# CMB-BNU/PloidyFrost

Measured on AMD Instinct MI355X. Metric: unitigs/s through superbubble+SeqAlign (k=25, z=8), higher is better.
Workload: dtype u64

## Files before the change

ploidyfrost_amd/csrc/pf_bubble.hip:

```cpp
#include <hip/hip_runtime.h>

#include <algorithm>
#include <chrono>
#include <cmath>
#include <cstdio>
#include <cstdlib>
#include <cstring>
#include <string>
#include <vector>

#include "pf_align_dev.hpp"
#include "pf_bubble_launch.hpp"
#include "pf_ctx.hpp"
#include "pf_device_common.hpp"
#include "ploidyfrost_hip.h"

using namespace pf;

#define PF_HIP(call)                                                                         \
    do {                                                                                     \
        hipError_t e_ = (call);                                                              \
        if (e_ != hipSuccess) {                                                              \
            pf::CtxErr{ctx} = std::string(#call) + ": " + hipGetErrorString(e_);                   \
            return PF_ERR_HIP;                                                               \
// ... 534 lines not shown
            const MsaRef M = list[cur][c];
            const char *rows = arena[cur] + M.off;
            uint8_t *ci = M.len <= p.work_bytes ? nw_base : colinfo;
            const Metrics m = classify(rows, M.rows, M.len, ci, snp_pos, indel_pos, indel_len);
            int verdict = 0;
            uint64_t c_indel = 0, c_snp = 0, c_all = 0;
            const int total = m.snp + m.indel, btotal = best_snp + best_indel;
            if (total < btotal) verdict = 1;
            else if (total == btotal) {
                if (m.indel < best_indel) verdict = 1;
                else if (m.indel == best_indel) {
                    c_indel = spread_merged(indel_pos, m.n_indel_pos, nullptr, 0, Lref);
                    if (c_indel > (uint64_t)d_indel) verdict = 1;
                    else if (c_indel == (uint64_t)d_indel) {
                        c_snp = spread_merged(snp_pos, m.n_snp_pos, nullptr, 0, Lref);
                        if (c_snp > (uint64_t)d_snp) verdict = 1;
                        else if (c_snp == (uint64_t)d_snp) {
                            c_all = spread_merged(snp_pos, m.n_snp_pos, indel_pos, m.n_indel_pos, Lref);
                            if (c_all > (uint64_t)d_all) verdict = 1;
                            else if (c_all == (uint64_t)d_all) {
                                if (m.first_site > left || m.last_site > right) verdict = 1;
                                else if (m.first_site == left && m.last_site == right && best >= 0) {
                                    const MsaRef B = list[cur][best];
                                    const char *brows = arena[cur] + B.off;
                                    for (uint32_t r = 0; r < M.rows; ++r)
                                        if (str_greater(rows + (size_t)r * M.len, M.len, brows + (size_t)r * B.len, B.len)) {
                                            verdict = 2;
                                            break;
                                        }
                                    if (verdict == 2) { left = m.first_site; right = m.last_site; }
                                }
                            }
                        }
                    }
                }
            }
            if (verdict == 0) continue;
            if (verdict == 1) {
                const int f = m.any_site ? m.first_site : -1, l = m.any_site ? m.last_site : -1;
                left = left > f ? left : f;
                right = right > l ? right : l;
                c_all = spread_merged(snp_pos, m.n_snp_pos, indel_pos, m.n_indel_pos, Lref);
                c_snp = spread_merged(snp_pos, m.n_snp_pos, nullptr, 0, Lref);
                c_indel = spread_merged(indel_pos, m.n_indel_pos, nullptr, 0, Lref);
            }
            d_all = (int)c_all;
            d_snp = (int)c_snp;
            d_indel = (int)c_indel;
            best_snp = m.snp;
            best_indel = m.indel;
            best = (int)c;
        }
    }

    mark(5);
    pf_bubble_result res;
    memset(&res, 0, sizeof(res));
    if (best < 0) {
        if (lane == 0) o.res[job] = res;
        return 0;
    }
    const MsaRef B = list[cur][best];
    const char *rows = arena[cur] + B.off;
    if (B.len <= p.work_bytes) colinfo = nw_base;
    const Metrics m = classify(rows, B.rows, B.len, colinfo, snp_pos, indel_pos, indel_len);
    uint32_t n_sites = 0;
    for (uint32_t base = 0; base < B.len; base += WAVE) {
        const uint32_t j = base + lane;
        n_sites += (uint32_t)__popcll(__ballot(j < B.len && (colinfo[j] & 16)));
    }
    const unsigned long long t0 = bub_take(o, al, 0, (unsigned long long)B.rows * B.len, 4096);
    const unsigned long long s0 = bub_take(o, al, 1, n_sites, 64);
    const unsigned long long g0 = bub_take(o, al, 2, (unsigned long long)n_sites * B.rows, 256);
    const unsigned long long l0 = bub_take(o, al, 3, m.n_indel_len, 32);
    res.rows_off = t0;
    res.site_off = s0;
    res.group_off = g0;
    res.ilen_off = l0;
    res.n_rows = B.rows;
    res.n_cols = B.len;
    res.n_sites = n_sites;
    res.n_indel_len = m.n_indel_len;
    if (lane == 0) o.res[job] = res;
    if (t0 + (uint64_t)B.rows * B.len > o.text_cap || s0 + n_sites > o.site_cap || g0 + (uint64_t)n_sites * B.rows > o.group_cap ||
        l0 + m.n_indel_len > o.ilen_cap)
        return 0;
    for (uint32_t t = lane; t < B.rows * B.len; t += WAVE) o.text[t0 + t] = rows[t];
    for (uint32_t t = lane; t < m.n_indel_len; t += WAVE) o.ilen[l0 + t] = indel_len[t];
    uint32_t rank_base = 0;
    for (uint32_t base = 0; base < B.len; base += WAVE) {
        const uint32_t j = base + lane;
        const bool is_site = j < B.len && (colinfo[j] & 16);
        const unsigned long long mask = __ballot(is_site);
        if (is_site) {
            const uint32_t rk = rank_base + (uint32_t)__popcll(mask & ((1ull << lane) - 1));
            uint8_t *grp = o.groups + g0 + (uint64_t)rk * B.rows;
            uint8_t next = 0;
            for (uint32_t r = 0; r < B.rows; ++r) {
                const char c = rows[(size_t)r * B.len + j];
                uint32_t e = 0;
                while (e < r && rows[(size_t)e * B.len + j] != c) ++e;
                grp[r] = e < r ? grp[e] : ++next;
            }
            pf_bubble_site sr;
            sr.col = j;
            sr.is_indel = (colinfo[j] & 32) ? 1 : 0;
            sr.maxnum = next;
            sr.pad_ = 0;
            o.sites[s0 + rk] = sr;
        }
        rank_base += (uint32_t)__popcll(mask);
    }
    mark(6);
    return 0;
}

template <bool LDS>
__global__ __launch_bounds__(64, 3) void k_bubble(BubParams p, BubOut o) {
    extern __shared__ __attribute__((aligned(16))) uint8_t smem[];
    uint8_t *nw_base;
    if constexpr (LDS) nw_base = smem;
    else nw_base = p.work + (uint64_t)blockIdx.x * p.work_per_wave;
    uint8_t *scr = p.scratch + (uint64_t)blockIdx.x * p.scratch_per_wave;
    BubAlloc al;
    for (;;) {
        uint32_t q = 0;
        if (lane_id() == 0) q = atomicAdd(p.next, 1u);
        q = read_lane(q, 0);
        if (q >= p.n) break;
        const uint32_t job = p.idx[q];
        const unsigned long long c0 = p.task_clk ? wall_clock64() : 0;
        const int rc = bubble_task<LDS>(p, o, al, job, nw_base, scr);
        if (p.task_clk && lane_id() == 0) p.task_clk[job] = wall_clock64() - c0;
        if (rc != 0 && lane_id() == 0) {
            if (p.final_tier) {
                pf_bubble_result r;
                memset(&r, 0, sizeof(r));
                r.n_rows = 0xFFFFFFFFu;
                o.res[job] = r;
                if (p.bad) atomicAdd(p.bad, 1u);
            } else {
                const unsigned int x = atomicAdd(o.n_retry, 1u);
                o.retry[x] = job;
            }
        }
        aln_sync();
    }
}

}

namespace pf {

unsigned long long *bubble_pool_heads(pf_ctx *ctx, int lane) { return (unsigned long long *)ctx_ws(ctx, bub_ws(WS_BUB_SMALL, lane), 128); }

constexpr int kBubTrains = 3;
static int bubble_streams(pf_ctx *ctx, int lane) {
    if (ctx->bub_streams[lane][0]) return PF_OK;
    for (int c = 0; c < kBubTrains; ++c) {
        PF_HIP(lane_stream_create(&ctx->bub_streams[lane][c], lane));
        PF_HIP(hipEventCreateWithFlags(&ctx->bub_events[lane][c], hipEventDisableTiming));
    }
    PF_HIP(hipEventCreateWithFlags(&ctx->bub_events[lane][kBubLdsClasses], hipEventDisableTiming));
    return PF_OK;
}
static int bubble_func_attr(pf_ctx *ctx) {
    static const hipError_t once = hipFuncSetAttribute(reinterpret_cast<const void *>(&k_bubble<true>), hipFuncAttributeMaxDynamicSharedMemorySize, 64 * 1024);
    PF_HIP(once);
    return PF_OK;
}

int bubble_reserve(pf_ctx *ctx, uint32_t n_tasks, int lane) {
    const BubCaps std_caps{64 * 1024, 8 * 1024, 512, 16 * 1024, 128 * 1024, 256, 8 * 1024};
    const uint64_t per = (bub_scratch_bytes(std_caps) + 255) & ~255ull;
    if (!ctx_ws(ctx, bub_ws(WS_BUB_SMALL, lane), 128) || !ctx_ws(ctx, bub_ws(WS_BUB_RETRY, lane), (size_t)std::max<uint32_t>(n_tasks, 1) * 4) ||
        !ctx_ws(ctx, bub_ws(WS_BUB_SCRATCH, lane), per * (uint64_t)ctx->n_cu * 24))
        return PF_ERR_HIP;
    DevLoadTrace trace;
    { const int e = bubble_streams(ctx, lane); if (e != PF_OK) return e; }
    trace.mark("bubble: class streams");
    { const int e = bubble_func_attr(ctx); if (e != PF_OK) return e; }
    trace.mark("bubble: function attributes");
    uint8_t *small = (uint8_t *)ctx_ws(ctx, bub_ws(WS_BUB_SMALL, lane), 128);
    PF_HIP(hipMemsetAsync(small, 0, 128, ctx->bub_streams[lane][0]));
    PF_HIP(hipStreamSynchronize(ctx->bub_streams[lane][0]));
    BubParams p;
    memset(&p, 0, sizeof(p));
    BubOut o;
    memset(&o, 0, sizeof(o));
    p.next = reinterpret_cast<unsigned int *>(small + 64);
    for (int c = 0; c < kBubLdsClasses; ++c) k_bubble<true><<<1, 64, kBubClassBytes[c], ctx->bub_streams[lane][c % kBubTrains]>>>(p, o);
    PF_HIP(hipGetLastError());
    for (int c = 0; c < kBubTrains; ++c) PF_HIP(hipStreamSynchronize(ctx->bub_streams[lane][c]));
    trace.mark("bubble: an empty launch per class stream");
    return PF_OK;
}

int bubble_launch(pf_ctx *ctx, const BubbleLaunch &L, unsigned long long heads[4]) {
    const int lane = L.lane;
    hipStream_t st = L.stream ? L.stream : ctx->stream;
    size_t tl_at = (size_t)-1;
    auto tbegin = [&](int kernel, hipStream_t s) { (void)ctx_begin_at(ctx, kernel, s, &tl_at); };
    auto tend = [&](hipStream_t s) { ctx_end_at(ctx, tl_at, s); };
    uint8_t *small = (uint8_t *)ctx_ws(ctx, bub_ws(WS_BUB_SMALL, lane), 128);
    uint32_t *d_retry = (uint32_t *)ctx_ws(ctx, bub_ws(WS_BUB_RETRY, lane), (size_t)std::max<uint32_t>(L.n_tasks, 1) * 4);
    if (!small || !d_retry) return PF_ERR_HIP;
    if (L.keep_heads) PF_HIP(hipMemsetAsync(small + 32, 0, 96, st));
    else PF_HIP(hipMemsetAsync(small, 0, 128, st));
    BubOut o;
    o.res = L.out.res; o.text = L.out.otext; o.sites = L.out.osites; o.groups = L.out.ogroups; o.ilen = L.out.oilen;
    o.text_cap = L.out.text_cap; o.site_cap = L.out.site_cap; o.group_cap = L.out.group_cap; o.ilen_cap = L.out.ilen_cap;
    o.heads = reinterpret_cast<unsigned long long *>(small);
    o.n_retry = reinterpret_cast<unsigned int *>(small + 40);
    unsigned int *queue_heads = reinterpret_cast<unsigned int *>(small + 64);
    int n_launch = 0;
    o.retry = d_retry;

    BubParams p;
    memset(&p, 0, sizeof(p));
    p.text = L.text; p.paths = L.paths; p.tasks = L.tasks; p.M = L.match; p.D = L.mismatch; p.G = L.gap;
    p.integral = (L.match == std::floor(L.match) && L.mismatch == std::floor(L.mismatch) && L.gap == std::floor(L.gap) &&
                  std::fabs(L.match) < 1e6 && std::fabs(L.mismatch) < 1e6 && std::fabs(L.gap) < 1e6) ? 1 : 0;
    p.seq = ctx->d_seq; p.off = ctx->d_off; p.len = ctx->d_len; p.n_unitigs = ctx->N;
    const BubCaps std_caps{64 * 1024, 8 * 1024, 512, 16 * 1024, 128 * 1024, 256, 8 * 1024};
    constexpr bool class_streams = true;
    constexpr int kTrains = kBubTrains;
    int grids[kBubLdsClasses];
    int train_of[kBubLdsClasses];
    int order[kBubLdsClasses];
    int n_order = 0;
    const uint64_t wave_budget = (uint64_t)ctx->n_cu * 24;
    const uint64_t train_waves = wave_budget / kTrains;
    {
        double load[kTrains] = {0, 0, 0};
        for (int c = 0; c < kBubLdsClasses; ++c) {
            grids[c] = 0;
            train_of[c] = 0;
            if (L.n_cls[c]) order[n_order++] = c;
        }
        auto work_of = [&](int c) { return (double)L.n_cls[c] * (double)kBubClassBytes[c]; };
        std::sort(order, order + n_order, [&](int x, int y) { return work_of(x) > work_of(y) || (work_of(x) == work_of(y) && x > y); });
        for (int i = 0; i < n_order; ++i) {
            const int c = order[i];
            int tr = 0;
            for (int q = 1; q < kTrains; ++q)
                if (load[q] < load[tr]) tr = q;
            train_of[c] = tr;
            load[tr] += work_of(c);
            grids[c] = (int)std::min<uint64_t>(std::min<uint64_t>(L.n_cls[c], (uint64_t)ctx->n_cu * bubble_class_waves_per_cu(c)), class_streams ? train_waves : wave_budget);
        }
    }
    const uint64_t max_waves = wave_budget;
    p.caps = std_caps;
    p.scratch_per_wave = (bub_scratch_bytes(std_caps) + 255) & ~255ull;
    const bool trace_ws = getenv("PF_TRACE_ALIGN") != nullptr;
    const auto t_ws = std::chrono::steady_clock::now();
    uint8_t *const scratch0 = (uint8_t *)ctx_ws(ctx, bub_ws(WS_BUB_SCRATCH, lane), p.scratch_per_wave * max_waves);
    if (trace_ws)
        fprintf(stderr, "[bubble_launch] scratch for %llu wavefronts x %llu bytes = %.1f MB taken in %.2f ms\n", (unsigned long long)max_waves, (unsigned long long)p.scratch_per_wave,
                (double)(p.scratch_per_wave * max_waves) / 1e6, std::chrono::duration<double>(std::chrono::steady_clock::now() - t_ws).count() * 1e3);
    p.scratch = scratch0;
    if (!p.scratch) return PF_ERR_HIP;
    if (class_streams) { const int e = bubble_streams(ctx, lane); if (e != PF_OK) return e; }

    DevTmp<unsigned long long> clk_;
    unsigned long long *d_clk = nullptr;
    const bool want_clk = getenv("PF_BUBBLE_STATS") != nullptr;
    if (want_clk) {
        PF_HIP(clk_.alloc(((size_t)L.n_tasks + 16) * 8));
        d_clk = clk_.p;
        PF_HIP(hipMemsetAsync(d_clk, 0, ((size_t)L.n_tasks + 16) * 8, st));
        p.task_clk = d_clk;
        p.prof = d_clk + L.n_tasks;
    }
    { const int e = bubble_func_attr(ctx); if (e != PF_OK) return e; }
    uint32_t idx_off = 0;
    for (int c = 0; c < kBubLdsClasses; ++c) idx_off += L.n_cls[c];
    if (class_streams) PF_HIP(hipEventRecord(ctx->bub_events[lane][kBubLdsClasses], st));
    bool train_used[kTrains] = {false, false, false};
    for (int i = 0; i < n_order; ++i) {
        const int c = order[i];
        const uint32_t nc = L.n_cls[c];
        uint32_t first = 0;
        for (int q = 0; q < c; ++q) first += L.n_cls[q];
        p.idx = L.idx + first;
        p.n = nc;
        p.work_bytes = (uint32_t)kBubClassBytes[c];
        const int grid = grids[c];
        p.next = queue_heads + n_launch++;
        hipStream_t cst = st;
        if (class_streams) {
            const int tr = train_of[c];
            cst = ctx->bub_streams[lane][tr];
            if (!train_used[tr]) PF_HIP(hipStreamWaitEvent(cst, ctx->bub_events[lane][kBubLdsClasses], 0));
            train_used[tr] = true;
            p.scratch = scratch0 + (uint64_t)tr * train_waves * p.scratch_per_wave;
        }
        tbegin(PF_K_BUBBLE, cst);
        k_bubble<true><<<grid, 64, kBubClassBytes[c], cst>>>(p, o);
        tend(cst);
        ctx_units(ctx, PF_K_BUBBLE, nc);
    }
    if (class_streams)
        for (int tr = 0; tr < kTrains; ++tr) {
            if (!train_used[tr]) continue;
            PF_HIP(hipEventRecord(ctx->bub_events[lane][tr], ctx->bub_streams[lane][tr]));
            PF_HIP(hipStreamWaitEvent(st, ctx->bub_events[lane][tr], 0));
        }
    p.scratch = scratch0;
    if (L.n_cls[kBubLdsClasses]) {
        const uint32_t nc = L.n_cls[kBubLdsClasses];
        const int grid = (int)std::min<uint32_t>(nc, 256);
        const uint64_t per = (std::min<uint64_t>(L.max_need * 2, 1ull << 31) + 255) & ~255ull;
        uint8_t *work = (uint8_t *)ctx_ws(ctx, bub_ws(WS_BUB_WORK, lane), per * grid);
        if (!work) return PF_ERR_HIP;
        p.idx = L.idx + idx_off;
        p.n = nc;
        p.work = work;
        p.work_per_wave = per;
        p.work_bytes = (uint32_t)std::min<uint64_t>(per, 0xFFFFFFFFu);
        p.next = queue_heads + n_launch++;
        tbegin(PF_K_BUBBLE_BIG, st);
        k_bubble<false><<<grid, 64, 0, st>>>(p, o);
        tend(st);
        ctx_units(ctx, PF_K_BUBBLE_BIG, nc);
    }
    unsigned int n_retry = 0;
    PF_HIP(hipMemcpyAsync(&n_retry, o.n_retry, 4, hipMemcpyDeviceToHost, st));
    PF_HIP(hipStreamSynchronize(st));
    int status = PF_OK;
    DevTmp<uint8_t> big_scratch_, big_work_;
    DevTmp<unsigned int> bad_;
    if (n_retry) {
        const uint64_t need = std::max<uint64_t>(1 << 20, L.retry_need);
        const BubCaps big{2u << 20, 256 * 1024, 16 * 1024, 512 * 1024, 4u << 20, 8192, 256 * 1024};
        const int grid = (int)std::min<uint32_t>(n_retry, 8);
        const uint64_t per_s = (bub_scratch_bytes(big) + 255) & ~255ull;
        const uint64_t per_w = (std::min<uint64_t>(need, 0xFFFFFF00u) + 255) & ~255ull;
        PF_HIP(big_scratch_.alloc(per_s * grid));
        PF_HIP(big_work_.alloc(per_w * grid));
        PF_HIP(bad_.alloc(4));
        PF_HIP(hipMemsetAsync(bad_.p, 0, 4, st));
        uint32_t *d_q = (uint32_t *)ctx_ws(ctx, bub_ws(WS_BUB_IDX2, lane), (size_t)n_retry * 4);
        if (!d_q) return PF_ERR_HIP;
        PF_HIP(hipMemcpyAsync(d_q, d_retry, (size_t)n_retry * 4, hipMemcpyDeviceToDevice, st));
        p.idx = d_q; p.n = n_retry; p.caps = big; p.scratch = big_scratch_.p; p.scratch_per_wave = per_s;
        p.work = big_work_.p; p.work_per_wave = per_w; p.work_bytes = (uint32_t)per_w; p.final_tier = 1;
        p.bad = bad_.p;
        p.next = queue_heads + n_launch++;
        tbegin(PF_K_BUBBLE_BIG, st);
        k_bubble<false><<<grid, 64, 0, st>>>(p, o);
        tend(st);
        unsigned int bad = 0;
        PF_HIP(hipMemcpyAsync(&bad, bad_.p, 4, hipMemcpyDeviceToHost, st));
        PF_HIP(hipStreamSynchronize(st));
        if (bad) {
            pf::CtxErr{ctx} = "pf_align_bubbles: a bubble exceeds the largest scratch tier";
            status = PF_ERR_OVERFLOW;
        }
    }
    if (want_clk) {
        const uint32_t n_tasks = L.n_tasks;
        std::vector<unsigned long long> clk(n_tasks + 16);
        PF_HIP(hipMemcpy(clk.data(), d_clk, ((size_t)n_tasks + 16) * 8, hipMemcpyDeviceToHost));
        fprintf(stderr, "[pf_align_bubbles] traceback: %llu jobs on the one-path fast road, %llu through the depth-first walk: %llu steps, %llu complete paths (%llu ticks in their analysis and copy), %llu kept\n",
                clk[n_tasks + 13], clk[n_tasks + 12], clk[n_tasks + 8], clk[n_tasks + 9], clk[n_tasks + 11], clk[n_tasks + 10]);
        fprintf(stderr, "[pf_align_bubbles] ticks by phase: fill %llu traceback %llu | decode %llu round0(incl. NW) %llu rounds %llu choose %llu publish %llu\n",
                clk[n_tasks], clk[n_tasks + 1], clk[n_tasks + 2], clk[n_tasks + 3], clk[n_tasks + 4], clk[n_tasks + 5], clk[n_tasks + 6]);
        clk.resize(n_tasks);
        {
            uint32_t tot_q = 0;
            for (int c = 0; c <= kBubLdsClasses; ++c) tot_q += L.n_cls[c];
            std::vector<uint32_t> hq(tot_q);
            if (tot_q) PF_HIP(hipMemcpy(hq.data(), L.idx, (size_t)tot_q * 4, hipMemcpyDeviceToHost));
            uint32_t at = 0;
            for (int c = 0; c <= kBubLdsClasses; ++c) {
                unsigned long long sum = 0, mx = 0;
                for (uint32_t q = 0; q < L.n_cls[c]; ++q) { const unsigned long long t = hq[at + q] < n_tasks ? clk[hq[at + q]] : 0; sum += t; mx = std::max(mx, t); }
                at += L.n_cls[c];
                if (L.n_cls[c])
                    fprintf(stderr, "   class %d (%s): %u bubbles on %d wavefronts, %llu ticks (%.2f ms if spread evenly), longest %llu ticks\n", c,
                            c == kBubLdsClasses ? "global" : "LDS", L.n_cls[c], c < kBubLdsClasses ? grids[c] : 0, sum,
                            c < kBubLdsClasses && grids[c] ? (double)sum / grids[c] * 1e-5 : 0.0, mx);
            }
        }
        std::vector<unsigned long long> srt(clk);
        std::sort(srt.begin(), srt.end());
        unsigned long long tot = 0;
        for (auto c : srt) tot += c;
        fprintf(stderr, "[pf_align_bubbles] %u tasks: ticks(10ns) sum %llu  median %llu  p90 %llu  p99 %llu  p99.9 %llu  max %llu\n", n_tasks, tot,
                srt[n_tasks / 2], srt[(size_t)(n_tasks * 0.9)], srt[(size_t)(n_tasks * 0.99)], srt[(size_t)(n_tasks * 0.999)], srt[n_tasks - 1]);
        {
            std::vector<pf_bubble_task> ht(n_tasks);
            PF_HIP(hipMemcpy(ht.data(), L.tasks, (size_t)n_tasks * sizeof(pf_bubble_task), hipMemcpyDeviceToHost));
            unsigned long long tk[2][4] = {{0, 0, 0, 0}, {0, 0, 0, 0}}, nk[2][4] = {{0, 0, 0, 0}, {0, 0, 0, 0}};
            for (uint32_t t = 0; t < n_tasks; ++t) {
                if (!clk[t] || ht[t].n_paths < 2) continue;
                pf_bubble_path p0;
                if (hipMemcpy(&p0, L.paths + ht[t].path_first, sizeof(p0), hipMemcpyDeviceToHost) != hipSuccess) break;
                const int a = p0.ov == PF_NONE ? 1 : 0, b = ht[t].n_paths >= 5 ? 3 : (int)ht[t].n_paths - 2;
                tk[a][b] += clk[t];
                nk[a][b]++;
                if (t > 60000) break;
            }
            for (int a = 0; a < 2; ++a)
                fprintf(stderr, "   %s: 2 paths %llu tasks %llu ticks | 3: %llu / %llu | 4: %llu / %llu | 5+: %llu / %llu\n", a ? "branching" : "strict   ",
                        nk[a][0], tk[a][0], nk[a][1], tk[a][1], nk[a][2], tk[a][2], nk[a][3], tk[a][3]);
        }
        unsigned long long over[4] = {0, 0, 0, 0};
        for (auto c : srt) { over[0] += c > 10000; over[1] += c > 30000; over[2] += c > 100000; if (c > 30000) over[3] += c; }
        fprintf(stderr, "   tasks over 0.1 ms: %llu, over 0.3 ms: %llu (their sum %llu ticks), over 1 ms: %llu\n", over[0], over[1], over[3], over[2]);
        for (int top = 0; top < 8 && top < (int)n_tasks; ++top) {
            const uint32_t t = (uint32_t)(std::max_element(clk.begin(), clk.end()) - clk.begin());
            pf_bubble_task tk;
            PF_HIP(hipMemcpy(&tk, L.tasks + t, sizeof(tk), hipMemcpyDeviceToHost));
            std::vector<pf_bubble_path> pp(std::min<uint32_t>(tk.n_paths, 12));
            if (!pp.empty()) PF_HIP(hipMemcpy(pp.data(), L.paths + tk.path_first, pp.size() * sizeof(pf_bubble_path), hipMemcpyDeviceToHost));
            pf_bubble_result rr;
            PF_HIP(hipMemcpy(&rr, L.out.res + t, sizeof(rr), hipMemcpyDeviceToHost));
            fprintf(stderr, "   slowest: task %u ticks %llu paths %u -> rows %u cols %u sites %u; lens", t, clk[t], tk.n_paths, rr.n_rows, rr.n_cols, rr.n_sites);
            for (auto &x : pp) fprintf(stderr, " %u", x.len);
            fprintf(stderr, "\n");
            clk[t] = 0;
        }
    }
    PF_HIP(hipMemcpy(heads, o.heads, 32, hipMemcpyDeviceToHost));
    if (status == PF_OK && (heads[0] > L.out.text_cap || heads[1] > L.out.site_cap || heads[2] > L.out.group_cap || heads[3] > L.out.ilen_cap)) {
        pf::CtxErr{ctx} = "pf_align_bubbles: output pools too small";
        status = PF_ERR_OVERFLOW;
    }
    return status;
}

}

extern "C" int pf_align_bubbles(pf_ctx *ctx, const char *text, uint64_t text_len, const pf_bubble_path *paths, uint64_t n_paths,
                                const pf_bubble_task *tasks, uint32_t n_tasks, double match, double mismatch, double gap,
                                pf_bubble_result *results, char *out_text, uint64_t text_cap, pf_bubble_site *out_sites,
                                uint64_t site_cap, uint8_t *out_groups, uint64_t group_cap, uint32_t *out_ilen,
                                uint64_t ilen_cap, uint64_t used[4]) {
    if (!ctx || !used || (n_tasks && (!paths || !tasks || !results || !out_text || !out_sites || !out_groups || !out_ilen)))
        return PF_ERR_ARG;
    used[0] = used[1] = used[2] = used[3] = 0;
    if (n_tasks == 0) return PF_OK;
    if (!ctx->d_seq) { pf::CtxErr{ctx} = "pf_align_bubbles: no graph uploaded"; return PF_ERR_ARG; }
    PF_HIP(hipSetDevice(ctx->device));
    hipStream_t st = ctx->stream;
    auto is_dev = [](const void *p) {
        hipPointerAttribute_t at;
        bool d = p && hipPointerGetAttributes(&at, p) == hipSuccess && at.type == hipMemoryTypeDevice;
        (void)hipGetLastError();
        return d;
    };
    std::vector<pf_bubble_task> ht_own;
    std::vector<pf_bubble_path> hp_own;
    const pf_bubble_task *ht = tasks;
    const pf_bubble_path *hp = paths;
    if (is_dev(tasks)) {
        ht_own.resize(n_tasks);
        PF_HIP(hipMemcpy(ht_own.data(), tasks, (size_t)n_tasks * sizeof(pf_bubble_task), hipMemcpyDeviceToHost));
        ht = ht_own.data();
    }
    if (n_paths && is_dev(paths)) {
        hp_own.resize(n_paths);
        PF_HIP(hipMemcpy(hp_own.data(), paths, (size_t)n_paths * sizeof(pf_bubble_path), hipMemcpyDeviceToHost));
        hp = hp_own.data();
    }
    const std::vector<uint32_t> &hlen = ctx->h_len;
    std::vector<uint32_t> cls[kBubLdsClasses + 1];
    std::vector<char> heavy;
    heavy.reserve(n_tasks);
    uint64_t max_need = 0, retry_need = 0;
    for (uint32_t t = 0; t < n_tasks; ++t) {
        const pf_bubble_task &tk = ht[t];
        if (tk.n_paths < 2 || tk.n_paths > 65535 || tk.path_first + tk.n_paths > n_paths) {
            pf::CtxErr{ctx} = "pf_align_bubbles: a bubble needs 2..65535 paths inside the path array";
            return PF_ERR_ARG;
        }
        uint32_t l0 = 0, lmax = 0;
        uint64_t sum = 0;
        for (uint32_t i = 0; i < tk.n_paths; ++i) {
            const pf_bubble_path &pp = hp[tk.path_first + i];
            if (pp.ov != PF_NONE) {
                if ((pp.ov >> 1) >= ctx->N) { pf::CtxErr{ctx} = "pf_align_bubbles: path unitig out of range"; return PF_ERR_ARG; }
                if (pp.len != hlen[pp.ov >> 1]) { pf::CtxErr{ctx} = "pf_align_bubbles: path length differs from the unitig's"; return PF_ERR_ARG; }
            } else if (pp.text_off + pp.len > text_len) {
                pf::CtxErr{ctx} = "pf_align_bubbles: path outside the text buffer";
                return PF_ERR_ARG;
            }
            if (pp.len == 0 || pp.len > 60000) { pf::CtxErr{ctx} = "pf_align_bubbles: empty path or longer than 60000"; return PF_ERR_ARG; }
            if (i == 0) l0 = pp.len;
            lmax = std::max(lmax, pp.len);
            sum += pp.len;
        }
        const int c = bubble_class(l0, lmax);
        cls[c].push_back(t);
        heavy.push_back(tk.n_paths > 2 || lmax > 64);
        if (c == kBubLdsClasses) max_need = std::max(max_need, bubble_need(l0, lmax));
        retry_need = std::max(retry_need, job_bytes((uint32_t)std::min<uint64_t>(sum, 60000), lmax));
    }
    for (auto &v : cls)
        std::stable_partition(v.begin(), v.end(), [&](uint32_t t) { return heavy[t]; });
    const char *d_text = text;
    if (text_len && !is_dev(text)) {
        char *b = (char *)ctx_ws(ctx, WS_BUB_TEXT, text_len + 1);
        if (!b) return PF_ERR_HIP;
        PF_HIP(hipMemcpyAsync(b, text, text_len, hipMemcpyHostToDevice, st));
        d_text = b;
    }
    pf_bubble_path *d_paths = (pf_bubble_path *)ctx_ws(ctx, WS_BUB_PATHS, std::max<uint64_t>(n_paths, 1) * sizeof(pf_bubble_path));
    pf_bubble_task *d_tasks = (pf_bubble_task *)ctx_ws(ctx, WS_BUB_TASKS, (size_t)n_tasks * sizeof(pf_bubble_task));
    uint32_t *d_idx = (uint32_t *)ctx_ws(ctx, WS_BUB_IDX, (size_t)n_tasks * 4);
    if (!d_paths || !d_tasks || !d_idx) return PF_ERR_HIP;
    PF_HIP(hipMemcpyAsync(d_paths, hp, (size_t)n_paths * sizeof(pf_bubble_path), hipMemcpyHostToDevice, st));
    PF_HIP(hipMemcpyAsync(d_tasks, ht, (size_t)n_tasks * sizeof(pf_bubble_task), hipMemcpyHostToDevice, st));
    const bool dev_out = is_dev(results);
    BubbleLaunch L;
    if (dev_out) {
        L.out.res = results; L.out.otext = out_text; L.out.osites = out_sites; L.out.ogroups = out_groups; L.out.oilen = out_ilen;
    } else {
        L.out.res = (pf_bubble_result *)ctx_ws(ctx, WS_BUB_RES, (size_t)n_tasks * sizeof(pf_bubble_result));
        L.out.otext = (char *)ctx_ws(ctx, WS_BUB_OTEXT, std::max<uint64_t>(text_cap, 1));
        L.out.osites = (pf_bubble_site *)ctx_ws(ctx, WS_BUB_OSITES, std::max<uint64_t>(site_cap, 1) * sizeof(pf_bubble_site));
        L.out.ogroups = (uint8_t *)ctx_ws(ctx, WS_BUB_OGROUPS, std::max<uint64_t>(group_cap, 1));
        L.out.oilen = (uint32_t *)ctx_ws(ctx, WS_BUB_OILEN, std::max<uint64_t>(ilen_cap, 1) * 4);
        if (!L.out.res || !L.out.otext || !L.out.osites || !L.out.ogroups || !L.out.oilen) return PF_ERR_HIP;
    }
    L.out.text_cap = text_cap; L.out.site_cap = site_cap; L.out.group_cap = group_cap; L.out.ilen_cap = ilen_cap;
    L.text = d_text; L.paths = d_paths; L.tasks = d_tasks; L.n_tasks = n_tasks;
    L.match = match; L.mismatch = mismatch; L.gap = gap;
    uint32_t idx_off = 0;
    for (int c = 0; c <= kBubLdsClasses; ++c) {
        L.n_cls[c] = (uint32_t)cls[c].size();
        if (cls[c].empty()) continue;
        PF_HIP(hipMemcpyAsync(d_idx + idx_off, cls[c].data(), cls[c].size() * 4, hipMemcpyHostToDevice, st));
        idx_off += (uint32_t)cls[c].size();
    }
    L.idx = d_idx;
    L.max_need = max_need;
    L.retry_need = retry_need;
    unsigned long long heads[4] = {0, 0, 0, 0};
    int status = bubble_launch(ctx, L, heads);
    for (int x = 0; x < 4; ++x) used[x] = heads[x];
    if (!dev_out && status == PF_OK) {
        PF_HIP(hipMemcpyAsync(results, L.out.res, (size_t)n_tasks * sizeof(pf_bubble_result), hipMemcpyDeviceToHost, st));
        PF_HIP(hipMemcpyAsync(out_text, L.out.otext, (size_t)heads[0], hipMemcpyDeviceToHost, st));
        PF_HIP(hipMemcpyAsync(out_sites, L.out.osites, (size_t)heads[1] * sizeof(pf_bubble_site), hipMemcpyDeviceToHost, st));
        PF_HIP(hipMemcpyAsync(out_groups, L.out.ogroups, (size_t)heads[2], hipMemcpyDeviceToHost, st));
        PF_HIP(hipMemcpyAsync(out_ilen, L.out.oilen, (size_t)heads[3] * 4, hipMemcpyDeviceToHost, st));
        PF_HIP(hipStreamSynchronize(st));
    }
    return status;
}
```

ploidyfrost_amd/csrc/pf_bubble_launch.hpp:

```cpp
#pragma once
#include <hip/hip_runtime.h>
#include <stdint.h>

#include "pf_align_dev.hpp"
#include "ploidyfrost_hip.h"

struct pf_ctx;

namespace pf {

constexpr int kBubLdsClasses = 9;
constexpr uint64_t kBubClassBytes[kBubLdsClasses] = {3072, 4608, 6 * 1024, 8 * 1024, 10 * 1024, 12 * 1024, 20 * 1024, 32 * 1024, 64 * 1024};
constexpr int kBubMaxClasses = 12;
__host__ __device__ inline int bubble_class_waves_per_cu(int c) {
    const int fit = (int)((160 * 1024) / kBubClassBytes[c]);
    return fit > 24 ? 24 : fit;
}

__host__ __device__ inline uint64_t bubble_need(uint32_t l0, uint32_t lmax) {
    return job_bytes((l0 > lmax ? l0 : lmax) + 32, lmax);
}
__host__ __device__ inline int bubble_class(uint32_t l0, uint32_t lmax) {
    const uint64_t need = bubble_need(l0, lmax);
    for (int x = 0; x < kBubLdsClasses; ++x)
        if (need <= kBubClassBytes[x]) return x;
    return kBubLdsClasses;
}

struct RowPools {
    pf_bubble_result *res = nullptr;
    char *otext = nullptr;
    uint64_t text_cap = 0;
    pf_bubble_site *osites = nullptr;
    uint64_t site_cap = 0;
    uint8_t *ogroups = nullptr;
    uint64_t group_cap = 0;
    uint32_t *oilen = nullptr;
    uint64_t ilen_cap = 0;
    unsigned long long *heads = nullptr;
};

struct BubbleLaunch {
    const char *text = nullptr;
    const pf_bubble_path *paths = nullptr;
    const pf_bubble_task *tasks = nullptr;
    uint32_t n_tasks = 0;
    const uint32_t *idx = nullptr;
    uint32_t n_cls[kBubLdsClasses + 1] = {};
    uint64_t max_need = 0;
    uint64_t retry_need = 0;
    double match = 2, mismatch = -1, gap = -3;
    RowPools out;
    bool keep_heads = false;
    int lane = 0;
    hipStream_t stream = nullptr;
};

unsigned long long *bubble_pool_heads(pf_ctx *ctx, int lane = 0);

inline bool snp_shortcut_scores(double M, double D, double G) {
    if (!(M < 1e6 && M > -1e6 && D < 1e6 && D > -1e6 && G < 1e6 && G > -1e6)) return false;
    const bool integral = M == (double)(long long)M && D == (double)(long long)D && G == (double)(long long)G;
    return integral && M >= D && M + 1 >= 2 * (G + 1) && D - 2 * G - 2 > 0;
}

int bubble_launch(pf_ctx *ctx, const BubbleLaunch &L, unsigned long long heads[4]);
int bubble_reserve(pf_ctx *ctx, uint32_t n_tasks, int lane = 0);

}
```

ploidyfrost_amd/csrc/pf_call.hip:

```cpp
#include "pf_call_kernels.hpp"
#include "pf_scan.hpp"

using namespace pf;

#define PF_HIP(call)                                                                         \
    do {                                                                                     \
        hipError_t e_ = (call);                                                              \
        if (e_ != hipSuccess) {                                                              \
            pf::CtxErr{ctx} = std::string(#call) + ": " + hipGetErrorString(e_);                   \
            return PF_ERR_HIP;                                                               \
        }                                                                                    \
    } while (0)

#define PF_TRY(call) do { const int s_ = (call); if (s_ != PF_OK) return s_; } while (0)

using namespace pf_call;

struct Need { DevBuf *buf; size_t bytes; };
static int need(pf_ctx *ctx, const char *who, std::initializer_list<Need> list) {
    for (const Need &n : list)
        if (!n.buf->ensure(n.bytes)) { pf::CtxErr{ctx} = std::string(who) + ": out of device memory"; return PF_ERR_HIP; }
    return PF_OK;
}

// ... 214 lines not shown
        return PF_OK;
    }
    if (!ctx || !ctx->d_seq || !ctx->d_tab) { if (ctx) pf::CtxErr{ctx} = "pf_call_coverage: graph and count table first"; return PF_ERR_ARG; }
    PF_HIP(hipSetDevice(ctx->device));
    CallState *S = state_of(ctx);
    const size_t N = ctx->N;
    const int slots = ctx->tab_exact ? 2 : 1;
    if (!S->cov_sum.ensure(N * slots * 8) || !S->cov_min.ensure(N * slots * 4) || !S->cov_miss.ensure(N * slots)) {
        pf::CtxErr{ctx} = "pf_call_coverage: out of device memory";
        return PF_ERR_HIP;
    }
    int st;
    if (!ctx->tab_exact) {
        st = pf_unitig_cov(ctx, 0, (uint32_t)N, S->cov_sum.as<uint64_t>(), S->cov_min.as<uint32_t>(), S->cov_miss.as<uint8_t>());
    } else {
        st = pf_unitig_cov_exact(ctx, 0, (uint32_t)N, 0, S->cov_sum.as<uint64_t>(), S->cov_min.as<uint32_t>(), S->cov_miss.as<uint8_t>());
        if (st == PF_OK || st == PF_ERR_MISSING_KMER)
            st = pf_unitig_cov_exact(ctx, 0, (uint32_t)N, 1, S->cov_sum.as<uint64_t>() + N, S->cov_min.as<uint32_t>() + N, S->cov_miss.as<uint8_t>() + N);
    }
    if (st != PF_OK && st != PF_ERR_MISSING_KMER) return st;
    S->per_strand = ctx->tab_exact;
    S->have_cov = true;
    return PF_OK;
}

int pf_call_scan(pf_ctx *ctx, uint32_t lower, uint32_t upper, uint64_t *n_sides) {
    if (!ctx || !n_sides) return PF_ERR_ARG;
    CallState *S = ctx->call;
    if (!S || !S->have_state || !S->have_cov) { pf::CtxErr{ctx} = "pf_call_scan: pf_call_set_state and pf_call_coverage first"; return PF_ERR_ARG; }
    PF_HIP(hipSetDevice(ctx->device));
    hipStream_t st = ctx->stream;
    const uint32_t N = ctx->N;
    if (!S->side_cnt.ensure(((size_t)N + 1) * 4) || !S->side_base.ensure(((size_t)N + 1) * 4)) { pf::CtxErr{ctx} = "pf_call_scan: out of device memory"; return PF_ERR_HIP; }
    k_call_count_sides<<<(N + 1 + 255) / 256, 256, 0, st>>>(S->flags.as<uint8_t>(), N, S->side_cnt.as<uint32_t>());
    if (!S->scan_tmp.ensure(scan_scratch_bytes((uint64_t)N + 1))) { pf::CtxErr{ctx} = "pf_call_scan: out of device memory"; return PF_ERR_HIP; }
    PF_HIP(scan_exclusive_u32(S->side_cnt.as<uint32_t>(), S->side_base.as<uint32_t>(), (uint64_t)N + 1, S->scan_tmp.p, st));
    uint32_t total = 0;
    PF_HIP(hipMemcpyAsync(&total, S->side_base.as<uint32_t>() + N, 4, hipMemcpyDeviceToHost, st));
    PF_HIP(hipStreamSynchronize(st));
    S->n_sides = total;
    S->n_tasks = 0;
    S->low = lower;
    S->up = upper;
    *n_sides = total;
    if (total == 0) return PF_OK;
    if (!S->sides.ensure((size_t)total * sizeof(pf_call_side)) || !S->ctask.ensure((size_t)total * sizeof(CallTask)) ||
        !S->target.ensure((size_t)total * 4)) {
        pf::CtxErr{ctx} = "pf_call_scan: out of device memory";
        return PF_ERR_HIP;
    }
    ScanArgs a;
    a.flags = S->flags.as<uint8_t>(); a.plus = S->plus.as<uint32_t>(); a.minus = S->minus.as<uint32_t>();
    a.succ = ctx->d_succ; a.pred = ctx->d_pred; a.seq = ctx->d_seq; a.off = ctx->d_off; a.len = ctx->d_len; a.N = N; a.k = ctx->k;
    a.cov_sum = S->cov_sum.as<uint64_t>(); a.cov_min = S->cov_min.as<uint32_t>(); a.cov_miss = S->cov_miss.as<uint8_t>();
    a.per_strand = S->per_strand; a.low = lower; a.up = upper;
    a.side_base = S->side_base.as<uint32_t>(); a.sides = S->sides.as<pf_call_side>(); a.tasks = S->ctask.as<CallTask>();
    a.target = S->target.as<uint32_t>();
    a.n_colors = S->n_colors;
    a.ccov_sum = S->ccov_sum.as<uint64_t>(); a.ccov_min = S->ccov_min.as<uint32_t>(); a.ccov_max = S->ccov_max.as<uint32_t>(); a.ccov_miss = S->ccov_miss.as<uint8_t>();
    a.clow = S->col_low.as<uint32_t>(); a.cup = S->col_up.as<uint32_t>(); a.full = S->col_full.as<uint64_t>(); a.cwords = S->col_words; a.size_total = S->col_size.as<uint64_t>();
    ctx_begin(ctx, PF_K_CALL_SCAN);
    if (S->n_colors) k_call_sides<true><<<(N + 255) / 256, 256, 0, st>>>(a);
    else k_call_sides<false><<<(N + 255) / 256, 256, 0, st>>>(a);
    ctx_end(ctx);
    ctx_units(ctx, PF_K_CALL_SCAN, N);
    PF_HIP(hipGetLastError());
    return PF_OK;
}

int pf_call_resolve(pf_ctx *ctx, uint64_t *n_bubbles, uint32_t *err, uint32_t *err_unitig) {
    if (!ctx || !ctx->call || !n_bubbles || !err || !err_unitig) return PF_ERR_ARG;
    CallState *S = ctx->call;
    *n_bubbles = 0;
    *err = 0;
    *err_unitig = 0;
    S->n_tasks = 0;
    const uint64_t n = S->n_sides;
    if (n == 0) return PF_OK;
    PF_HIP(hipSetDevice(ctx->device));
    hipStream_t st = ctx->stream;
    if (!S->pending.ensure(n * 4) || !S->killed.ensure(n) || !S->rstate.ensure(n) || !S->rflag.ensure(n * 4) || !S->rsmall.ensure(64) ||
        !S->kept.ensure(n * 4)) {
        pf::CtxErr{ctx} = "pf_call_resolve: out of device memory";
        return PF_ERR_HIP;
    }
    PF_HIP(hipMemsetAsync(S->pending.p, 0, n * 4, st));
    PF_HIP(hipMemsetAsync(S->killed.p, 0, n, st));
    PF_HIP(hipMemsetAsync(S->rstate.p, 0, n, st));
    unsigned int *small = S->rsmall.as<unsigned int>();
    ResolveArgs a;
    a.sides = S->sides.as<pf_call_side>(); a.target = S->target.as<uint32_t>(); a.n = (uint32_t)n; a.pending = S->pending.as<int>();
    a.killed = S->killed.as<uint8_t>(); a.state = S->rstate.as<uint8_t>(); a.flag = S->rflag.as<uint32_t>();
    a.undecided = small; a.first_err = small + 1;
    const unsigned int init[3] = {0, 0xFFFFFFFFu, 0};
    PF_HIP(hipMemcpyAsync(small, init, 12, hipMemcpyHostToDevice, st));
    const unsigned grid = (unsigned)((n + 255) / 256);
    k_call_pending<<<grid, 256, 0, st>>>(a);
    for (uint64_t round = 0;; ++round) {
        if (round > n + 2) { pf::CtxErr{ctx} = "pf_call_resolve: the driver pass does not settle"; return PF_ERR_ARG; }
        k_call_resolve<<<grid, 256, 0, st>>>(a);
        PF_HIP(hipMemsetAsync(small, 0, 4, st));
        k_call_resolve<<<grid, 256, 0, st>>>(a);
        unsigned int h[2];
        PF_HIP(hipMemcpyAsync(h, small, 8, hipMemcpyDeviceToHost, st));
        PF_HIP(hipStreamSynchronize(st));
        if (h[1] != 0xFFFFFFFFu && h[0] == 0) {
            pf_call_side bad;
            PF_HIP(hipMemcpy(&bad, S->sides.as<pf_call_side>() + h[1], sizeof(bad), hipMemcpyDeviceToHost));
            *err = bad.err;
            *err_unitig = bad.err_unitig;
            return PF_OK;
        }
        if (h[0] == 0) break;
    }
    if (!S->scan_tmp.ensure(scan_scratch_bytes(n))) { pf::CtxErr{ctx} = "pf_call_resolve: out of device memory"; return PF_ERR_HIP; }
    PF_HIP(select_flagged_u32(S->rflag.as<uint32_t>(), S->kept.as<uint32_t>(), small + 2, nullptr, n, S->scan_tmp.p, st));
    unsigned int sel = 0;
    PF_HIP(hipMemcpyAsync(&sel, small + 2, 4, hipMemcpyDeviceToHost, st));
    PF_HIP(hipStreamSynchronize(st));
    S->n_tasks = sel;
    *n_bubbles = sel;
    return PF_OK;
}

int pf_call_sides(pf_ctx *ctx, pf_call_side *out, uint64_t cap) {
    if (!ctx || !ctx->call) return PF_ERR_ARG;
    CallState *S = ctx->call;
    if (cap < S->n_sides || (S->n_sides && !out)) return PF_ERR_OVERFLOW;
    if (S->n_sides == 0) return PF_OK;
    PF_HIP(hipSetDevice(ctx->device));
    PF_HIP(hipMemcpyAsync(out, S->sides.p, (size_t)S->n_sides * sizeof(pf_call_side), hipMemcpyDefault, ctx->stream));
    PF_HIP(hipStreamSynchronize(ctx->stream));
    return PF_OK;
}

int pf_call_select(pf_ctx *ctx, const uint32_t *side_index, uint64_t n_tasks) {
    if (!ctx || !ctx->call || (n_tasks && !side_index)) return PF_ERR_ARG;
    CallState *S = ctx->call;
    if (n_tasks > S->n_sides) { pf::CtxErr{ctx} = "pf_call_select: more bubbles than open sides"; return PF_ERR_ARG; }
    PF_HIP(hipSetDevice(ctx->device));
    if (!S->kept.ensure(std::max<size_t>(n_tasks, 1) * 4)) { pf::CtxErr{ctx} = "pf_call_select: out of device memory"; return PF_ERR_HIP; }
    if (n_tasks) PF_HIP(hipMemcpyAsync(S->kept.p, side_index, (size_t)n_tasks * 4, hipMemcpyDefault, ctx->stream));
    PF_HIP(hipStreamSynchronize(ctx->stream));
    S->n_tasks = n_tasks;
    return PF_OK;
}

}

namespace {

int ensure_batch_buffers(pf_ctx *ctx, const char *who, CallState::AlignWork &W, CallState::AlignOut &O, uint32_t nb) {
    const size_t list = (size_t)nb * 4;
    return need(ctx, who, {{&W.counters, sizeof(CallCounters)}, {&W.btask, (size_t)nb * sizeof(pf_bubble_task)}, {&W.queues, (size_t)NQ * list},
                           {&W.blist, list}, {&W.slist, list}, {&W.plist, list}, {&W.plist2, list}, {&W.klist, list}, {&W.klist_b, list}, {&W.has, list},
                           {&O.res, (size_t)nb * sizeof(pf_bubble_result)}, {&O.sv_off, (size_t)nb * 8}, {&O.vc, list}});
}

int ensure_wave_scratch(pf_ctx *ctx, const char *who, CallState::AlignWork &W, const CallGrids &g, uint32_t depth, bool stack_tier, bool pair_tier) {
    PF_TRY(need(ctx, who, {{&W.paths_scr, paths_per_wave(depth) * g.paths}}));
    if (stack_tier) PF_TRY(need(ctx, who, {{&W.stack_scr, stack_scratch_bytes() * g.stack}}));
    if (pair_tier) PF_TRY(need(ctx, who, {{&W.pair_scr, PairGeom<PAIR_MAX>::scratch_bytes * g.pair}}));
    return PF_OK;
}

int ensure_pools(pf_ctx *ctx, const char *who, CallState::AlignWork &W, CallState::AlignOut &O, uint32_t nb, const BatchPools &p) {
    PF_TRY(need(ctx, who, {{&W.bpath, p.path_entries(nb) * sizeof(pf_bubble_path)}, {&W.ptext, p.path_text}, {&O.otext, p.row_text},
                           {&O.osites, p.sites * sizeof(pf_bubble_site)}, {&O.ogroups, p.groups}, {&O.oilen, p.ilen * 4}}));
    if (p.walk) PF_TRY(need(ctx, who, {{&W.walk_pool, p.walk * 4}, {&W.walk_off, (size_t)nb * 8}}));
    return PF_OK;
}

int ensure_lane_streams(pf_ctx *ctx, CallState::AlignWork &W, int lane) {
    if (lane != 0 && !W.stream) { PF_HIP(lane_stream_create(&W.stream, lane)); W.own_stream = true; }
    if (!W.side_stream) {
        PF_HIP(lane_stream_create(&W.side_stream, lane));
        PF_HIP(hipEventCreateWithFlags(&W.ev_prep, hipEventDisableTiming));
        PF_HIP(hipEventCreateWithFlags(&W.ev_paths, hipEventDisableTiming));
    }
    return PF_OK;
}

int stats_begin(pf_ctx *ctx, DevTmp<unsigned long long> &prof, size_t words, hipStream_t st, unsigned long long **arg) {
    PF_HIP(prof.alloc(words * 8));
    PF_HIP(hipMemsetAsync(prof.p, 0, words * 8, st));
    *arg = prof.p;
    return PF_OK;
}
int print_pair_stats(pf_ctx *ctx, const DevTmp<unsigned long long> &prof) {
    unsigned long long h[8];
    PF_HIP(hipMemcpy(h, prof.p, 64, hipMemcpyDeviceToHost));
    fprintf(stderr, "[k_call_pair] %llu wavefront rounds; lane-0 ticks (10 ns): decode %llu fill %llu traceback %llu classify %llu publish %llu\n", h[5],
            h[0], h[1], h[2], h[3], h[4]);
    return PF_OK;
}
int print_sites_stats(pf_ctx *ctx, const DevTmp<unsigned long long> &prof, int grid, hipStream_t st) {
    PF_HIP(hipStreamSynchronize(st));
    std::vector<unsigned long long> h((size_t)grid * 6);
    PF_HIP(hipMemcpy(h.data(), prof.p, h.size() * 8, hipMemcpyDeviceToHost));
    unsigned long long sum[6] = {0, 0, 0, 0, 0, 0}, mx = 0;
    for (int w = 0; w < grid; ++w) {
        for (int x = 0; x < 6; ++x) sum[x] += h[(size_t)w * 6 + x];
        mx = std::max(mx, h[(size_t)w * 6]);
    }
    fprintf(stderr, "[k_call_sites] %d wavefronts, %llu bubbles; ticks (10 ns) per wavefront: total %.0f (max %llu) = pop + load %.0f, strings %.0f, ranks + probes %.0f, groups %.0f\n",
            grid, sum[5], (double)sum[0] / grid, mx, (double)sum[1] / grid, (double)sum[2] / grid, (double)sum[3] / grid, (double)sum[4] / grid);
    return PF_OK;
}

int env_int(const char *name, int otherwise) { const char *e = getenv(name); return e ? atoi(e) : otherwise; }

struct AlignTrace {
    const bool on = getenv("PF_TRACE_ALIGN") != nullptr;
    const std::chrono::steady_clock::time_point t_enter = std::chrono::steady_clock::now();
    void stage(const char *what) const {
        if (on) fprintf(stderr, "[pf_call_align]   %-34s %.2f ms\n", what, std::chrono::duration<double>(std::chrono::steady_clock::now() - t_enter).count() * 1e3);
    }
};

struct AlignCall {
    static constexpr const char *who = "pf_call_run";
    pf_ctx *const ctx; CallState *const S;
    CallState::AlignWork &W; CallState::AlignOut &O;
    const int lane; const uint64_t t0; const uint32_t nb;
    const double match, mismatch, gap;
    const AlignTrace trace;
    const bool snp_ok = snp_shortcut_scores(match, mismatch, gap);
    const bool pair_tier = std::fabs(match) < 1e5 && std::fabs(mismatch) < 1e5 && std::fabs(gap) < 1e5;
    const bool pair_integral = match == std::floor(match) && mismatch == std::floor(mismatch) && gap == std::floor(gap);
    const bool stack_tier = stack_scores(match, mismatch, gap);
    const int stack_ok = stack_tier ? std::max(1, std::min(3, env_int("PF_STACK_LEVEL", 1))) : 0;
    const int paths_force_scratch = env_int("PF_PATHS_SCRATCH", 0) ? 1 : 0;
    const CallGrids grids = call_grids(ctx->n_cu);
    const uint32_t depth;
    hipStream_t st = nullptr;
    CallCounters *d_cnt = nullptr;
    BatchRef batch = {};
    GraphSeq graph = {};
    CallLists lists = {};
    RowPools pools;
    BatchPools cap = {};
    PathArgs ph = {};
    PairArgs pr = {};
    int attempt = 0;
    CallCounters hc = {};
    unsigned long long heads[4] = {0, 0, 0, 0};
    uint64_t n_jobs = 0;
    uint32_t n_called = 0;
    size_t tl_at = (size_t)-1;

    AlignCall(pf_ctx *c, int lane_, uint64_t t0_, uint32_t nb_, uint32_t complex_size, double m, double d, double g)
        : ctx(c), S(c->call), W(c->call->work[lane_]), O(c->call->lane[lane_]), lane(lane_), t0(t0_), nb(nb_), match(m), mismatch(d), gap(g), depth(depth_cap(complex_size)) {}

    void tbegin(int kernel, hipStream_t s) { (void)ctx_begin_at(ctx, kernel, s, &tl_at); }
    void tend(hipStream_t s) { ctx_end_at(ctx, tl_at, s); }

    int prepare() {
        PF_TRY(ensure_lane_streams(ctx, W, lane));
        st = lane == 0 ? ctx->stream : W.stream;
        for (hipEvent_t e : O.read_ev) if (e) PF_HIP(hipStreamWaitEvent(st, e, 0));
        PF_TRY(ensure_batch_buffers(ctx, who, W, O, nb));
        PF_TRY(ensure_wave_scratch(ctx, who, W, grids, depth, stack_tier, pair_tier));
        if (W.mlist_cap < MANY_LIST_MIN) W.mlist_cap = MANY_LIST_MIN;
        PF_TRY(need(ctx, who, {{&W.mlist, (size_t)W.mlist_cap * 4}}));
        d_cnt = W.counters.as<CallCounters>();
        batch = BatchRef{S->ctask.as<CallTask>(), S->kept.as<uint32_t>(), t0, nb};
        graph = GraphSeq{ctx->d_seq, ctx->d_off, ctx->d_len};
        lists = CallLists{W.queues.as<uint32_t>(), W.blist.as<uint32_t>(), W.slist.as<uint32_t>(), W.plist.as<uint32_t>(), W.plist2.as<uint32_t>(), W.klist.as<uint32_t>(), W.klist_b.as<uint32_t>(), nb};
        trace.stage("lists and scratch");
        return PF_OK;
    }

    int size_pools() {
        LearntPools l;
        l.path_pool = S->path_pool; l.path_text = S->text_pool; l.row_text = S->otext_cap; l.sites = S->osites_cap; l.groups = S->ogroups_cap; l.ilen = S->oilen_cap;
        l.walk = W.walk_cap;
        cap = batch_pools(nb, grids, l, S->n_colors != 0);
        PF_TRY(ensure_pools(ctx, who, W, O, nb, cap));
        unsigned long long *d_heads = bubble_pool_heads(ctx, lane);
        if (!d_heads) return PF_ERR_HIP;
        pools = RowPools{O.res.as<pf_bubble_result>(), O.otext.as<char>(), cap.row_text, O.osites.as<pf_bubble_site>(), cap.sites, O.ogroups.as<uint8_t>(), cap.groups,
                         O.oilen.as<uint32_t>(), cap.ilen, d_heads};
        PF_HIP(hipMemsetAsync(d_cnt, 0, sizeof(CallCounters), st));
        PF_HIP(hipMemsetAsync(d_heads, 0, 32, st));
        return PF_OK;
    }

    int launch_tiers() {
        PrepArgs pa;
        pa.batch = batch; pa.len = graph.len; pa.btask = W.btask.as<pf_bubble_task>(); pa.bpath = W.bpath.as<pf_bubble_path>(); pa.res = pools.res;
        pa.lists = lists; pa.snp_ok = snp_ok ? 1 : 0; pa.pair_ok = pair_tier ? 1 : 0; pa.stack_ok = stack_ok; pa.cnt = d_cnt;
        tbegin(PF_K_CALL_PREP, st);
        k_call_prep<<<(nb + 255) / 256, 256, 0, st>>>(pa);
        tend(st);
        hipStream_t pst = W.side_stream;
        PF_HIP(hipEventRecord(W.ev_prep, st));
        PF_HIP(hipStreamWaitEvent(pst, W.ev_prep, 0));
        ph = PathArgs{};
        ph.batch = batch; ph.blist = lists.blist; ph.succ = ctx->d_succ; ph.graph = graph; ph.k = ctx->k; ph.depth_cap = depth;
        ph.scratch = W.paths_scr.as<uint8_t>(); ph.scratch_per_wave = paths_per_wave(depth); ph.force_scratch = paths_force_scratch;
        ph.max_paths = MAX_PATHS; ph.n_list = &d_cnt->n_branching; ph.mlist = W.mlist.as<uint32_t>(); ph.mlist_cap = W.mlist_cap;
        ph.walk_pool = S->n_colors ? W.walk_pool.as<uint32_t>() : nullptr; ph.walk_off = W.walk_off.as<uint64_t>(); ph.walk_cap = cap.walk;
        ph.btask = pa.btask; ph.bpath = pa.bpath; ph.path_cap = cap.path_pool; ph.text = W.ptext.as<char>(); ph.text_cap = cap.path_text;
        ph.queues = lists.queues; ph.klist = lists.klist_b; ph.stack_ok = stack_ok; ph.cnt = d_cnt;
        tbegin(PF_K_CALL_PATHS, pst);
        k_call_paths<false><<<grids.paths, 64, 0, pst>>>(ph);
        tend(pst);
        PF_HIP(hipEventRecord(W.ev_paths, pst));
        if (snp_ok) {
            SnpArgs sn;
            sn.batch = batch; sn.slist = lists.slist; sn.graph = graph; sn.out = pools; sn.lists = lists; sn.pair_ok = pa.pair_ok; sn.stack_ok = stack_ok; sn.cnt = d_cnt;
            tbegin(PF_K_CALL_SNP, st);
            k_call_snp<<<(nb + 255) / 256, 256, 0, st>>>(sn);
            tend(st);
        }
        StackArgs sk;
        if (stack_tier) {
            sk.list = lists.klist; sk.n_list = &d_cnt->n_stack; sk.scratch = W.stack_scr.as<uint8_t>(); sk.pair_ok = pa.pair_ok;
            sk.btask = pa.btask; sk.bpath = pa.bpath; sk.ptext = W.ptext.as<char>(); sk.graph = graph;
            sk.M = (int)match; sk.D = (int)mismatch; sk.G = (int)gap;
            sk.out = pools; sk.lists = lists; sk.cnt = d_cnt;
            tbegin(PF_K_CALL_STACK, st);
            k_call_stack<<<grids.stack, 64, 0, st>>>(sk);
            tend(st);
        }
        if (pair_tier) {
            pr = PairArgs{};
            pr.batch = batch; pr.graph = graph; pr.M = match; pr.D = mismatch; pr.G = gap; pr.Mi = (int)match; pr.Di = (int)mismatch; pr.Gi = (int)gap;
            pr.list = lists.plist; pr.n_list = &d_cnt->n_pair; pr.n_done = &d_cnt->n_pair_done;
            pr.scratch = W.pair_scr.as<uint8_t>(); pr.out = pools; pr.lists = lists; pr.cnt = d_cnt;
            static const bool pair_stats = getenv("PF_PAIR_STATS") != nullptr;
            DevTmp<unsigned long long> prof;
            if (pair_stats) PF_TRY(stats_begin(ctx, prof, 8, st, &pr.prof));
            tbegin(PF_K_CALL_PAIR, st);
            if (pair_integral) k_call_pair<PAIR_MAX, true><<<grids.pair, 64, 0, st>>>(pr);
            else k_call_pair<PAIR_MAX, false><<<grids.pair, 64, 0, st>>>(pr);
            tend(st);
            if (pair_stats) PF_TRY(print_pair_stats(ctx, prof));
            pr.prof = nullptr;
        }
        PF_HIP(hipStreamWaitEvent(st, W.ev_paths, 0));
        if (stack_tier) {
            sk.list = lists.klist_b; sk.n_list = &d_cnt->n_stack_b; sk.pair_ok = 0;
            tbegin(PF_K_CALL_STACK, st);
            k_call_stack<<<grids.stack, 64, 0, st>>>(sk);
            tend(st);
        }
        return PF_OK;
    }

    int read_counters() {
        PF_HIP(hipGetLastError());
        PF_HIP(hipMemcpyAsync(&hc, d_cnt, sizeof(hc), hipMemcpyDeviceToHost, st));
        PF_HIP(hipStreamSynchronize(st));
        return PF_OK;
    }

    int launch_pair_tier2() {
        if (!pair_tier || !hc.n_pair2) return PF_OK;
        PairArgs p2 = pr;
        p2.list = lists.plist2; p2.n_list = &d_cnt->n_pair2; p2.n_done = &d_cnt->n_pair2_done;
        const uint32_t tier2_min = (uint32_t)env_int("PF_PAIR2_MIN", 0);
        if (hc.n_pair2 < (tier2_min ? tier2_min : pair2_min(ctx->n_cu))) {
            k_call_pair2_reroute<<<(hc.n_pair2 + 255) / 256, 256, 0, st>>>(p2);
        } else {
            const int g2 = call_pair2_grid(hc.n_pair2, grids);
            PF_TRY(need(ctx, who, {{&W.pair_scr2, PairGeom<PAIR_MAX2>::scratch_bytes * g2}}));
            p2.scratch = W.pair_scr2.as<uint8_t>();
            tbegin(PF_K_CALL_PAIR, st);
            if (pair_integral) k_call_pair<PAIR_MAX2, true><<<g2, 64, 0, st>>>(p2);
            else k_call_pair<PAIR_MAX2, false><<<g2, 64, 0, st>>>(p2);
            tend(st);
        }
        return read_counters();
    }

    void note_units() const {
        ctx_units(ctx, PF_K_CALL_PREP, nb);
        if (snp_ok) ctx_units(ctx, PF_K_CALL_SNP, hc.n_snp);
        if (pair_tier) ctx_units(ctx, PF_K_CALL_PAIR, hc.n_pair + hc.n_pair2);
        if (stack_tier) ctx_units(ctx, PF_K_CALL_STACK, hc.n_stack + hc.n_stack_b);
        ctx_units(ctx, PF_K_CALL_PATHS, hc.n_branching);
        if (trace.on) fprintf(stderr, "[pf_call_align] bubbles of more than 255 walks: %u, err %u\n", hc.n_many, hc.err);
    }

    int launch_paths_big(bool *retry) {
        if (!hc.n_many || (hc.err & ERR_WALK)) return PF_OK;
        if (hc.n_many > W.mlist_cap) {
            W.mlist_cap = grown_many(hc.n_many);
            *retry = true;
            return need(ctx, who, {{&W.mlist, (size_t)W.mlist_cap * 4}});
        }
        const int big_grid = paths_big_grid(hc.n_many);
        const uint64_t big_per_wave = paths_big_per_wave(depth, PATHS_BIG);
        PF_TRY(need(ctx, who, {{&W.paths_big_scr, big_per_wave * big_grid}}));
        PathArgs pb = ph;
        pb.blist = W.mlist.as<uint32_t>(); pb.n_list = &d_cnt->n_many; pb.max_paths = PATHS_BIG; pb.mlist = nullptr; pb.mlist_cap = 0;
        pb.scratch = W.paths_big_scr.as<uint8_t>(); pb.scratch_per_wave = big_per_wave;
        tbegin(PF_K_CALL_PATHS, st);
        k_call_paths<true><<<big_grid, 64, 0, st>>>(pb);
        tend(st);
        return read_counters();
    }

    int accept_walks(bool *retry) {
        if (hc.err & ERR_WALK) {
            char where[96];
            snprintf(where, sizeof where, " (superbubble from unitig %u%c to unitig %u%c)", (hc.err_entrance >> 1) + 1, (hc.err_entrance & 1) ? '-' : '+',
                     (hc.err_exit >> 1) + 1, (hc.err_exit & 1) ? '-' : '+');
            pf::CtxErr{ctx} = std::string(hc.err & ERR_MANY_PATHS ? "pf_call_run: a bubble has more than 65535 paths" : "pf_call_run: a bubble is deeper than the complex size allows") + where;
            return PF_ERR_ARG;
        }
        amax(S->otext_cap, cap.row_text); amax(S->osites_cap, cap.sites);
        amax(S->ogroups_cap, cap.groups); amax(S->oilen_cap, cap.ilen);
        amax(S->path_pool, cap.path_pool);
        amax(S->text_pool, cap.path_text);
        const uint64_t rows_need = row_text_need(hc.text_head, hc.n_branching, nb);
        if (trace.on)
            fprintf(stderr, "[pf_call_align] attempt %d: %u bubbles, path pool %llu of %llu, path text %llu of %llu, rows text cap %llu (needs %llu)\n", attempt, nb,
                    (unsigned long long)hc.path_head, (unsigned long long)cap.path_pool, (unsigned long long)hc.text_head, (unsigned long long)cap.path_text,
                    (unsigned long long)cap.row_text, (unsigned long long)rows_need);
        if (hc.path_head > cap.path_pool || hc.text_head > cap.path_text || hc.walk_head > cap.walk) {
            amax(S->path_pool, grown(hc.path_head, 1024));
            amax(S->text_pool, grown(hc.text_head, 4096));
            if (S->n_colors) W.walk_cap = std::max<uint64_t>(W.walk_cap, grown(hc.walk_head, 1024));
            *retry = true;
            return PF_OK;
        }
        if (S->n_colors) W.walk_cap = std::max(W.walk_cap, cap.walk);
        if (cap.row_text < rows_need) {
            amax(S->otext_cap, rows_need + rows_need / 16 + 4096);
            *retry = true;
        }
        return PF_OK;
    }

    int run_bubble(bool *retry) {
        n_jobs = 0;
        for (int x = 0; x < NQ; ++x) n_jobs += hc.q_n[x];
        PF_TRY(need(ctx, who, {{&W.scan_tmp2, std::max<size_t>((size_t)n_jobs, 1) * 4}}));
        uint32_t *d_idx = W.scan_tmp2.as<uint32_t>();
        size_t at = 0;
        for (int x = 0; x < NQ; ++x) {
            if (!hc.q_n[x]) continue;
            PF_HIP(hipMemcpyAsync(d_idx + at, W.queues.as<uint32_t>() + (size_t)x * nb, (size_t)hc.q_n[x] * 4, hipMemcpyDeviceToDevice, st));
            at += hc.q_n[x];
        }
        BubbleLaunch BL;
        BL.text = W.ptext.as<char>(); BL.paths = W.bpath.as<pf_bubble_path>(); BL.tasks = W.btask.as<pf_bubble_task>();
        BL.n_tasks = nb; BL.idx = d_idx;
        for (int c = 0; c <= kBubLdsClasses; ++c) BL.n_cls[c] = hc.q_n[2 * c] + hc.q_n[2 * c + 1];
        BL.max_need = hc.max_need; BL.retry_need = hc.retry_need;
        BL.match = match; BL.mismatch = mismatch; BL.gap = gap;
        BL.out = pools;
        BL.keep_heads = true;
        BL.lane = lane; BL.stream = st;
        trace.stage("K-BUBBLE launching");
        const int bst = bubble_launch(ctx, BL, heads);
        trace.stage("K-BUBBLE done");
        if (trace.on)
            fprintf(stderr, "[pf_call_align] attempt %d: K-BUBBLE status %d, pools text %llu of %llu, sites %llu of %llu, groups %llu of %llu, indel lengths %llu of %llu\n", attempt, bst,
                    heads[0], (unsigned long long)cap.row_text, heads[1], (unsigned long long)cap.sites, heads[2], (unsigned long long)cap.groups, heads[3], (unsigned long long)cap.ilen);
        if (bst == PF_ERR_OVERFLOW && (heads[0] > cap.row_text || heads[1] > cap.sites || heads[2] > cap.groups || heads[3] > cap.ilen)) {
            amax(S->otext_cap, heads[0] + heads[0] / 8);
            amax(S->osites_cap, heads[1] + heads[1] / 8);
            amax(S->ogroups_cap, heads[2] + heads[2] / 8);
            amax(S->oilen_cap, heads[3] + heads[3] / 8);
            *retry = true;
            return PF_OK;
        }
        return bst;
    }

    int number_called() {
        k_call_has<<<(nb + 255) / 256, 256, 0, st>>>(O.res.as<pf_bubble_result>(), nb, W.has.as<uint32_t>());
        PF_TRY(need(ctx, who, {{&W.scan_tmp, scan_scratch_bytes(nb)}}));
        PF_HIP(scan_inclusive_u32(W.has.as<uint32_t>(), O.vc.as<uint32_t>(), nb, W.scan_tmp.p, st));
        PF_HIP(hipMemcpyAsync(&n_called, O.vc.as<uint32_t>() + (nb - 1), 4, hipMemcpyDeviceToHost, st));
        return PF_OK;
    }

    SiteArgs site_args(uint32_t ks, uint64_t rows_cap, uint64_t per_wave, uint64_t sv_cap) const {
        SiteArgs sa;
        sa.batch = batch; sa.blist = lists.blist; sa.res = pools.res; sa.otext = pools.otext; sa.osites = pools.osites; sa.ogroups = pools.ogroups;
        sa.k = ctx->k; sa.tab = ctx->d_tab; sa.mask = ctx->tab_cap - 1; sa.one_strand = ctx->tab_one_strand; sa.tab_exact = ctx->tab_exact;
        sa.low = S->low; sa.up = S->up; sa.ks = ks; sa.rows_cap = (uint32_t)rows_cap;
        sa.scratch = W.sites_scr.as<uint8_t>(); sa.scratch_per_wave = per_wave; sa.sv_off = O.sv_off.as<uint64_t>();
        sa.sv = O.sv.as<double>(); sa.sv_cap = sv_cap; sa.cnt = d_cnt; sa.prof = nullptr;
        sa.n_colors = S->n_colors;
        sa.ctab = CTab{ctx->d_ctab, ctx->ctab_cap - 1, ctx->ctab_line_bytes}; sa.c_one_strand = ctx->ctab_one_strand; sa.unread = ctx->d_unread;
        sa.clow = S->col_low.as<uint32_t>(); sa.cup = S->col_up.as<uint32_t>(); sa.full = S->col_full.as<uint64_t>(); sa.cwords = S->col_words;
        sa.part_first = S->part_first.as<uint32_t>(); sa.part_colour = S->part_colour.as<uint32_t>(); sa.part_word = S->part_word.as<uint64_t>();
        sa.part_bits = S->part_bits.as<uint64_t>(); sa.walk_pool = W.walk_pool.as<uint32_t>(); sa.walk_off = W.walk_off.as<uint64_t>();
        sa.graph = graph;
        return sa;
    }

    int launch_sites(SiteArgs &sa, int grid) {
        static const bool sites_stats = getenv("PF_SITES_STATS") != nullptr;
        DevTmp<unsigned long long> prof;
        if (sites_stats) PF_TRY(stats_begin(ctx, prof, (size_t)grid * 6, st, &sa.prof));
        PF_HIP(hipMemsetAsync(&d_cnt->sites_next, 0, 4, st));
        PF_HIP(hipMemsetAsync(&d_cnt->sv_head, 0, 8, st));
        PF_HIP(hipMemsetAsync(&d_cnt->site_strings, 0, 8, st));
        tbegin(PF_K_CALL_SITES, st);
        if (sa.n_colors) k_call_sites<true><<<grid, 64, 0, st>>>(sa);
        else k_call_sites<false><<<grid, 64, 0, st>>>(sa);
        tend(st);
        ctx_units(ctx, PF_K_CALL_SITES, hc.n_branching);
        if (sites_stats) { PF_HIP(hipGetLastError()); PF_TRY(print_sites_stats(ctx, prof, grid, st)); }
        return read_counters();
    }

    int run_sites() {
        uint32_t KS = std::max<uint32_t>(first_site_string(ctx->k), S->sites_ks.load());
        const uint32_t C = S->n_colors;
        const uint64_t rows_cap = sites_rows_cap(hc.max_rows);
        for (int sv_attempt = 0, ks_attempt = 0;;) {
            const uint64_t per_wave = sites_per_wave(rows_cap, KS, C, S->col_words);
            const int grid = call_sites_grid(hc.n_branching, grids, per_wave);
            const uint64_t sv_cap = site_values_cap(C, hc.n_branching, grid, S->sv_pool);
            PF_TRY(need(ctx, who, {{&W.sites_scr, per_wave * grid}, {&O.sv, sv_cap * 8}}));
            SiteArgs sa = site_args(KS, rows_cap, per_wave, sv_cap);
            PF_TRY(launch_sites(sa, grid));
            if (hc.err & ERR_SITE_LONG) {
                if (++ks_attempt > 3 || hc.ks_need <= KS) { pf::CtxErr{ctx} = "pf_call_run: the room for a site string does not converge"; return PF_ERR_OVERFLOW; }
                KS = grown_site_string(hc.ks_need);
                amax(S->sites_ks, KS);
                hc.err = 0; hc.ks_need = 0;
                PF_HIP(hipMemsetAsync(&d_cnt->err, 0, 4, st));
                PF_HIP(hipMemsetAsync(&d_cnt->ks_need, 0, 4, st));
                continue;
            }
            if (hc.err & ERR_MISSING_KMER) { pf::CtxErr{ctx} = "CDBG::readCov(): a kmer of a site string can not found ."; return PF_ERR_MISSING_KMER; }
            if (hc.err & ERR_SITE_ROW) { pf::CtxErr{ctx} = "CDBG::PloidyEstimation(): a site string runs past the end of an aligned row (the reference terminates here: std::out_of_range from substr, src/CDBG.cpp:1478-1590)"; return PF_ERR_ARG; }
            if (hc.err & ERR_SITE_UNITIG) { pf::CtxErr{ctx} = "CCDBG::PloidyEstimation(): a site string does not start on a unitig of its bubble"; return PF_ERR_ARG; }
            if (hc.sv_head > sv_cap) {
                if (sv_attempt++ >= 2) { pf::CtxErr{ctx} = "pf_call_run: site value pool does not converge"; return PF_ERR_OVERFLOW; }
                amax(S->sv_pool, grown(hc.sv_head, 1024));
                continue;
            }
            amax(S->sv_pool, sv_cap);
            return PF_OK;
        }
    }
};

}

extern "C" {

int pf_call_align_lane(pf_ctx *ctx, int lane, uint64_t t0, uint64_t t1, uint32_t complex_size, double match, double mismatch, double gap,
                       pf_call_result *out) {
    if (!ctx || !out || lane < 0 || lane >= PF_CALL_LANES) return PF_ERR_ARG;
    CallState *S = ctx->call;
    if (!S || t0 > t1 || t1 > S->n_tasks) { pf::CtxErr{ctx} = "pf_call_align: range outside the selection"; return PF_ERR_ARG; }
    memset(out, 0, sizeof(*out));
    CallState::AlignOut &O = S->lane[lane];
    O.nb = 0;
    O.t0 = t0;
    O.cur = pf_call_result{};
    if (t1 == t0) return PF_OK;
    if (t1 - t0 > (1u << 24)) { pf::CtxErr{ctx} = "pf_call_align: at most 2^24 bubbles per batch"; return PF_ERR_ARG; }
    PF_HIP(hipSetDevice(ctx->device));
    AlignCall A(ctx, lane, t0, (uint32_t)(t1 - t0), complex_size, match, mismatch, gap);
    PF_TRY(A.prepare());
    for (A.attempt = 0;; ++A.attempt) {
        if (A.attempt > 5) { pf::CtxErr{ctx} = "pf_call_align: pools do not converge"; return PF_ERR_OVERFLOW; }
        bool retry = false;
        PF_TRY(A.size_pools());
        PF_TRY(A.launch_tiers());
        PF_TRY(A.read_counters());
        A.trace.stage("K-PREP .. K-STACK done");
        PF_TRY(A.launch_pair_tier2());
        A.note_units();
        PF_TRY(A.launch_paths_big(&retry));
        if (!retry) PF_TRY(A.accept_walks(&retry));
        if (!retry) PF_TRY(A.run_bubble(&retry));
        if (!retry) break;
    }
    const CallCounters &hc = A.hc;
    out->n_branching = hc.n_branching;
    out->align_jobs = A.n_jobs + hc.n_snp_done + hc.n_pair_done + hc.n_pair2_done + hc.n_stack_done;
    out->snp_jobs = hc.n_snp_done; out->pair_jobs = hc.n_pair_done + hc.n_pair2_done; out->wave_jobs = A.n_jobs; out->stack_jobs = hc.n_stack_done;
    PF_TRY(A.number_called());
    if (hc.n_branching) {
        PF_TRY(A.run_sites());
    } else {
        PF_TRY(need(ctx, A.who, {{&O.sv, 16}}));
        PF_HIP(hipStreamSynchronize(A.st));
    }
    out->site_strings = hc.site_strings;
    A.trace.stage("K-SITES done");
    out->n_called = A.n_called;
    O.nb = A.nb;
    O.cur = *out;
    for (int x = 0; x < 4; ++x) O.used[x] = A.heads[x];
    O.used[4] = hc.n_branching ? hc.sv_head : 0;
    return PF_OK;
}

int pf_call_peek(pf_ctx *ctx, int lane, pf_call_bubble *bubbles, pf_bubble_result *results, uint64_t *sv_off, uint64_t bubble_cap, char *text,
                 pf_bubble_site *sites, uint8_t *groups, uint32_t *ilen, double *sv, const uint64_t cap[5], uint64_t used[6]) {
    if (!ctx || lane < 0 || lane >= PF_CALL_LANES || !used) return PF_ERR_ARG;
    CallState *S = ctx->call;
    if (!S) { pf::CtxErr{ctx} = "pf_call_peek: pf_call_align first"; return PF_ERR_ARG; }
    if (S->n_colors) { pf::CtxErr{ctx} = "pf_call_peek: the single-sample path's view (a colored site holds one value per colour and group)"; return PF_ERR_ARG; }
    const CallState::AlignOut &O = S->lane[lane];
    used[0] = O.nb;
    for (int x = 0; x < 5; ++x) used[x + 1] = O.used[x];
    if (!O.nb) return PF_OK;
    if (!bubbles && !results && !text && !sites && !groups && !ilen && !sv && !sv_off) return PF_OK;
    if (bubble_cap < O.nb || !cap) return PF_ERR_ARG;
    for (int x = 0; x < 5; ++x)
        if (cap[x] < O.used[x]) return PF_ERR_ARG;
    PF_HIP(hipSetDevice(ctx->device));
    if (bubbles) {
        std::vector<uint32_t> kept(O.nb);
        PF_HIP(hipMemcpy(kept.data(), S->kept.as<uint32_t>() + O.t0, (size_t)O.nb * 4, hipMemcpyDeviceToHost));
        std::vector<CallTask> ct(S->n_sides);
        if (S->n_sides) PF_HIP(hipMemcpy(ct.data(), S->ctask.p, (size_t)S->n_sides * sizeof(CallTask), hipMemcpyDeviceToHost));
        for (uint32_t j = 0; j < O.nb; ++j) {
            const CallTask &t = ct[kept[j]];
            pf_call_bubble &b = bubbles[j];
            b.entrance_ov = t.entrance_ov; b.exit_ov = t.exit_ov; b.strict = t.strict; b.n_inner = t.n_inner;
            for (int x = 0; x < 4; ++x) { b.inner[x] = t.inner[x]; b.cov[x] = t.cov[x]; }
            b.core_mean = t.core_mean; b.cov_sum = t.cov_sum;
        }
    }
    if (results) PF_HIP(hipMemcpy(results, O.res.p, (size_t)O.nb * sizeof(pf_bubble_result), hipMemcpyDeviceToHost));
    if (sv_off) PF_HIP(hipMemcpy(sv_off, O.sv_off.p, (size_t)O.nb * 8, hipMemcpyDeviceToHost));
    if (text && O.used[0]) PF_HIP(hipMemcpy(text, O.otext.p, O.used[0], hipMemcpyDeviceToHost));
    if (sites && O.used[1]) PF_HIP(hipMemcpy(sites, O.osites.p, O.used[1] * sizeof(pf_bubble_site), hipMemcpyDeviceToHost));
    if (groups && O.used[2]) PF_HIP(hipMemcpy(groups, O.ogroups.p, O.used[2], hipMemcpyDeviceToHost));
    if (ilen && O.used[3]) PF_HIP(hipMemcpy(ilen, O.oilen.p, O.used[3] * 4, hipMemcpyDeviceToHost));
    if (sv && O.used[4]) PF_HIP(hipMemcpy(sv, O.sv.p, O.used[4] * 8, hipMemcpyDeviceToHost));
    return PF_OK;
}

int pf_call_reserve_lanes(pf_ctx *ctx, uint64_t nb64, uint32_t complex_size, int n_lanes) {
    if (!ctx || nb64 == 0 || n_lanes < 1 || n_lanes > PF_CALL_LANES) return PF_ERR_ARG;
    CallState *S = state_of(ctx);
    PF_HIP(hipSetDevice(ctx->device));
    const uint32_t nb = (uint32_t)std::min<uint64_t>(nb64, 1u << 24);
    const char *who = "pf_call_reserve";
    const CallGrids grids = call_grids(ctx->n_cu);
    DevLoadTrace trace;
    for (int lane = 0; lane < n_lanes; ++lane) {
        CallState::AlignWork &W = S->work[lane];
        CallState::AlignOut &O = S->lane[lane];
        PF_TRY(ensure_batch_buffers(ctx, who, W, O, nb));
        PF_TRY(ensure_wave_scratch(ctx, who, W, grids, depth_cap(complex_size), true, true));
        PF_TRY(ensure_pools(ctx, who, W, O, nb, batch_pools(nb, grids, LearntPools{}, false)));
        PF_TRY(need(ctx, who, {{&W.scan_tmp2, reserve_job_index_bytes(nb)}, {&W.sites_scr, sites_per_wave(256, first_site_string(31), 0, 1) * grids.sites},
                               {&O.sv, reserve_site_values(nb, grids) * 8}}));
        trace.mark("reserve: a lane's buffers");
        PF_TRY(ensure_lane_streams(ctx, W, lane));
        trace.mark("reserve: a lane's streams and events");
        PF_TRY(bubble_reserve(ctx, nb, lane));
        trace.mark("reserve: K-BUBBLE's workspaces and first launches");
    }
    return PF_OK;
}

int pf_call_reserve(pf_ctx *ctx, uint64_t nb64, uint32_t complex_size) { return pf_call_reserve_lanes(ctx, nb64, complex_size, 2); }

int pf_call_align(pf_ctx *ctx, uint64_t t0, uint64_t t1, uint32_t complex_size, double match, double mismatch, double gap,
                  pf_call_result *out) {
    return pf_call_align_lane(ctx, 0, t0, t1, complex_size, match, mismatch, gap, out);
}

static int text_work_of(pf_ctx *ctx, pf::CallState *S, int which, uint32_t nb) {
    pf::CallState::TextWork &T = S->text[which];
    if (!T.stream) {
        int least = 0, greatest = 0;
        PF_HIP(hipDeviceGetStreamPriorityRange(&least, &greatest));
        PF_HIP(hipStreamCreateWithPriority(&T.stream, hipStreamNonBlocking, greatest));
    }
    return need(ctx, "pf_call_text", {{&T.sizes, (size_t)N_INT * (nb + 1) * 4}, {&T.offs, ((size_t)N_INT * (nb + 1) + 1) * 8}, {&T.totals, 16 * 8},
                                      {&T.tcounters, sizeof(CallCounters)}, {&T.tscan, scan_scratch_bytes((uint64_t)N_INT * (nb + 1))}});
}

int pf_call_reserve_text(pf_ctx *ctx, uint64_t piece_bubbles) {
    if (!ctx || piece_bubbles == 0) return PF_ERR_ARG;
    pf::CallState *S = state_of(ctx);
    PF_HIP(hipSetDevice(ctx->device));
    const uint32_t nb = (uint32_t)std::min<uint64_t>(piece_bubbles, 1u << 24);
    for (int which = 0; which < 2; ++which) { const int ts = text_work_of(ctx, S, which, nb); if (ts != PF_OK) return ts; }
    for (int slab = 0; slab < PF_CALL_SLABS; ++slab) PF_TRY(need(ctx, "pf_call_text", {{&S->out[slab], (11ull * 31 + 40) * nb}}));
    for (int which = 0; which < 2; ++which) {
        pf::CallState::TextWork &T = S->text[which];
        FmtArgs fa;
        memset(&fa, 0, sizeof(fa));
        fa.sizes = T.sizes.as<uint32_t>(); fa.offs = T.offs.as<uint64_t>(); fa.cnt = T.tcounters.as<CallCounters>();
        if (S->n_colors) { k_call_format<false, true><<<1, FMT_BLOCK, 0, T.stream>>>(fa); k_call_format<true, true><<<1, FMT_BLOCK, 0, T.stream>>>(fa); }
        else { k_call_format<false, false><<<1, FMT_BLOCK, 0, T.stream>>>(fa); k_call_format<true, false><<<1, FMT_BLOCK, 0, T.stream>>>(fa); }
        PF_HIP(hipGetLastError());
        PF_HIP(hipStreamSynchronize(T.stream));
    }
    return PF_OK;
}

static int call_text_impl(pf_ctx *ctx, int lane, int slab, uint64_t first, uint64_t count, uint64_t var_count_base, pf_call_result *out, bool sizes_only) {
    if (!ctx || !out || slab < 0 || slab >= PF_CALL_SLABS || lane < 0 || lane >= PF_CALL_LANES) return PF_ERR_ARG;
    CallState *S = ctx->call;
    if (!S) return PF_ERR_ARG;
    CallState::AlignOut &O = S->lane[lane];
    if (first + count > O.nb) { pf::CtxErr{ctx} = "pf_call_text_range: range outside the aligned batch"; return PF_ERR_ARG; }
    if (S->n_colors && S->mt_format) { pf::CtxErr{ctx} = "pf_call_text_range: the -t > 1 format is the single-sample path's"; return PF_ERR_ARG; }
    if (!sizes_only)
        for (int s = 0; s < N_STREAMS; ++s) S->out_len[slab][s] = 0;
    *out = O.cur;
    out->n_called = 0;
    if (count == 0) return PF_OK;
    PF_HIP(hipSetDevice(ctx->device));
    const bool trace_stages = getenv("PF_TRACE_ALIGN") != nullptr;
    const auto t_enter = std::chrono::steady_clock::now();
    auto ta = [&](const char *what) {
        if (trace_stages) fprintf(stderr, "[pf_call_text]    %-34s %.2f ms\n", what, std::chrono::duration<double>(std::chrono::steady_clock::now() - t_enter).count() * 1e3);
    };
    const uint32_t nb = (uint32_t)count;
    const int which = sizes_only ? 0 : (slab & 1);
    { const int ts = text_work_of(ctx, S, which, nb); if (ts != PF_OK) return ts; }
    CallState::TextWork &T = S->text[which];
    hipStream_t st = T.stream;
    const uint64_t t0 = O.t0;
    uint32_t vc_edge[2] = {0, 0};
    PF_HIP(hipMemcpyAsync(&vc_edge[1], O.vc.as<uint32_t>() + (first + count - 1), 4, hipMemcpyDeviceToHost, st));
    if (first) PF_HIP(hipMemcpyAsync(&vc_edge[0], O.vc.as<uint32_t>() + (first - 1), 4, hipMemcpyDeviceToHost, st));
    CallCounters *d_cnt = T.tcounters.as<CallCounters>();
    CallCounters hc;
    const size_t n_sizes = (size_t)N_INT * (nb + 1);
    ta("stream and size tables");
    PF_HIP(hipMemsetAsync(&d_cnt->allele[0], 0, 6 * 8, st));
    FmtArgs fa;
    fa.ct = S->ctask.as<CallTask>(); fa.kept = S->kept.as<uint32_t>(); fa.t0 = t0; fa.j0 = (uint32_t)first; fa.nb = nb;
    fa.res = O.res.as<pf_bubble_result>();
    fa.otext = O.otext.as<char>(); fa.osites = O.osites.as<pf_bubble_site>(); fa.ogroups = O.ogroups.as<uint8_t>();
    fa.oilen = O.oilen.as<uint32_t>(); fa.sv_off = O.sv_off.as<uint64_t>(); fa.sv = O.sv.as<double>(); fa.vc = O.vc.as<uint32_t>();
    fa.vc_base = var_count_base; fa.mt = S->mt_format ? 1 : 0; fa.len = ctx->d_len; fa.sizes = T.sizes.as<uint32_t>(); fa.offs = T.offs.as<uint64_t>(); fa.cnt = d_cnt;
    for (int s = 0; s < N_INT; ++s) fa.out[s] = nullptr;
    fa.packed = S->pack_alignseq ? 1 : 0;
    size_t at = 0;
    ctx_begin_at(ctx, PF_K_CALL_FORMAT, st, &at);
    fa.n_colors = S->n_colors; fa.N = ctx->N; fa.k = ctx->k; fa.full = S->col_full.as<uint64_t>(); fa.cwords = S->col_words; fa.ccov_sum = S->ccov_sum.as<uint64_t>();
    if (S->n_colors) k_call_format<false, true><<<(nb + 1 + FMT_BLOCK - 1) / FMT_BLOCK, FMT_BLOCK, 0, st>>>(fa);
    else k_call_format<false, false><<<(nb + 1 + FMT_BLOCK - 1) / FMT_BLOCK, FMT_BLOCK, 0, st>>>(fa);
    ctx_end_at(ctx, at, st);
    PF_HIP(scan_exclusive_u32_u64(T.sizes.as<uint32_t>(), T.offs.as<uint64_t>(), n_sizes, T.tscan.p, st));
    k_call_totals<<<1, 64, 0, st>>>(T.offs.as<uint64_t>(), T.sizes.as<uint32_t>(), nb, T.totals.as<uint64_t>());
    uint64_t totals[N_INT + 1] = {};
    PF_HIP(hipMemcpyAsync(totals, T.totals.p, N_INT * 8, hipMemcpyDeviceToHost, st));
    PF_HIP(hipMemcpyAsync(&hc, d_cnt, sizeof(hc), hipMemcpyDeviceToHost, st));
    PF_HIP(hipStreamSynchronize(st));
    out->n_called = vc_edge[1] - vc_edge[0];
    const uint64_t packed_len = (fa.packed && totals[PF_OUT_ALIGNSEQ]) ? alnpack_index_bytes(nb) + totals[S_PACK] : 0;
    auto slab_len = [&](int s) { return (s == PF_OUT_ALIGNSEQ && fa.packed) ? packed_len : totals[s]; };
    out->alignseq_packed_len = packed_len;
    uint64_t all = 0;
    for (int s = 0; s < N_STREAMS; ++s) all += slab_len(s);
    if (sizes_only) {
        for (int s = 0; s < N_STREAMS; ++s) out->text_len[s] = totals[s];
        for (int x = 0; x < 4; ++x) out->allele[x] = hc.allele[x];
        out->core_cov = hc.core_cov;
        out->core_num = hc.core_num;
        return PF_OK;
    }
    ta("sizes counted");
    PF_TRY(need(ctx, "pf_call_text", {{&S->out[slab], std::max<uint64_t>(all, 16)}}));
    ta("slab taken");
    all = 0;
    for (int s = 0; s < N_STREAMS; ++s) {
        fa.out[s] = S->out[slab].as<char>() + all;
        S->out_off[slab][s] = all;
        S->out_len[slab][s] = slab_len(s);
        out->text_len[s] = totals[s];
        all += slab_len(s);
    }
    if (fa.packed) { fa.out[S_PACK] = fa.out[PF_OUT_ALIGNSEQ]; fa.out[PF_OUT_ALIGNSEQ] = nullptr; }
    if (S->model.read_ev[slab]) PF_HIP(hipStreamWaitEvent(st, S->model.read_ev[slab], 0));
    ctx_begin_at(ctx, PF_K_CALL_FORMAT, st, &at);
    if (S->n_colors) k_call_format<true, true><<<(nb + FMT_BLOCK - 1) / FMT_BLOCK, FMT_BLOCK, 0, st>>>(fa);
    else k_call_format<true, false><<<(nb + FMT_BLOCK - 1) / FMT_BLOCK, FMT_BLOCK, 0, st>>>(fa);
    ctx_end_at(ctx, at, st);
    ctx_units(ctx, PF_K_CALL_FORMAT, nb);
    PF_HIP(hipGetLastError());
    S->fetch_base[slab] = S->out[slab].as<char>();
    S->nib[slab] = false;
    out->numeric_packed = 0;
    for (int s = 0; s < N_STREAMS; ++s) { S->txt_off[slab][s] = S->out_off[slab][s]; S->txt_len[slab][s] = S->out_len[slab][s]; }
    if (S->pack_numeric) {
        uint64_t foff[N_STREAMS], flen[N_STREAMS], fall = 0;
        for (int s = 0; s < N_STREAMS; ++s) {
            flen[s] = s == PF_OUT_ALIGNSEQ ? ((slab_len(s) + 15) & ~15ull) : PF_NUMERIC_PACKED_LEN(totals[s]);
            foff[s] = fall;
            fall += flen[s];
        }
        PF_TRY(need(ctx, "pf_call_text", {{&S->outp[slab], fall + 16}}));
        char *pb = S->outp[slab].as<char>();
        PF_HIP(hipMemsetAsync(pb + fall, 0, 16, st));
        if (slab_len(PF_OUT_ALIGNSEQ))
            PF_HIP(hipMemcpyAsync(pb + foff[PF_OUT_ALIGNSEQ], S->out[slab].as<char>() + S->txt_off[slab][PF_OUT_ALIGNSEQ], (size_t)slab_len(PF_OUT_ALIGNSEQ), hipMemcpyDeviceToDevice, st));
        NibArgs na;
        int x = 0;
        uint64_t units = 0;
        for (int s = 0; s < N_STREAMS; ++s) {
            if (s == PF_OUT_ALIGNSEQ) continue;
// ... 154 lines not shown
```

ploidyfrost_amd/csrc/pf_call_kernels.hpp:

```cpp
#pragma once

#include <hip/hip_runtime.h>

#include <algorithm>
#include <atomic>
#include <chrono>
#include <cmath>
#include <cstddef>
#include <cstdio>
#include <cstdlib>
#include <cstring>
#include <string>
#include <vector>

#include "pf_bubble_launch.hpp"
#include "pf_alnpack.hpp"
#include "pf_call_dev.hpp"
#include "pf_call_plan.hpp"
#include "pf_colored_dev.hpp"
#include "pf_cov_stream.hpp"
#include "pf_ctx.hpp"
#include "pf_device_common.hpp"
#include "pf_filter_rows.hpp"
#include "pf_format_dev.hpp"
#include "pf_pair_dev.hpp"
#include "pf_stack_dev.hpp"
#include "ploidyfrost_hip.h"

using namespace pf;

namespace pf_call {

constexpr uint8_t B_PLUS = 0x01, B_MINUS = 0x02, B_STRICT_M = 0x08, B_STRICT_P = 0x10, B_COMPLEX_M = 0x20, B_COMPLEX_P = 0x40;
constexpr int N_STREAMS = PF_CALL_STREAMS;
constexpr int N_INT = N_STREAMS + 1;
constexpr int S_PACK = N_STREAMS;
constexpr int NQ = 2 * (kBubLdsClasses + 1);
constexpr int KEY_BRANCHING = NQ, KEY_SNP = NQ + 1, KEY_PAIR = NQ + 2, KEY_PAIR2 = NQ + 3, KEY_STACK = NQ + 4, KEY_NONE = NQ + 5;

struct DevBuf {
    void *p = nullptr;
    size_t cap = 0;
    template <typename T>
    T *as() const { return reinterpret_cast<T *>(p); }
    bool ensure(size_t bytes) {
        if (bytes <= cap && p) return true;
        if (p) (void)hipFree(p);
        p = nullptr;
        cap = 0;
        const size_t want = bytes + bytes / 4 + 256;
        if (hipMalloc(&p, want) != hipSuccess) { (void)hipGetLastError(); p = nullptr; return false; }
        cap = want;
        return true;
    }
    void release() {
        if (p) (void)hipFree(p);
        p = nullptr;
        cap = 0;
    }
};

template <typename T, typename V>
inline void amax(std::atomic<T> &a, V v) {
    T cur = a.load(std::memory_order_relaxed);
    while (cur < (T)v && !a.compare_exchange_weak(cur, (T)v, std::memory_order_relaxed)) {}
}

enum CallErr : unsigned int {
    ERR_MANY_PATHS = 1u,
    ERR_MISSING_KMER = 2u,
    ERR_SITE_ROW = 4u,
    ERR_PATH_POOL = 8u,
    ERR_SITE_LONG = 16u,
    ERR_TOO_DEEP = 32u,
    ERR_SITE_UNITIG = 64u,
    ERR_WALK = ERR_MANY_PATHS | ERR_TOO_DEEP,
};

struct CallCounters {
    unsigned int q_n[NQ];
    unsigned int n_branching;
    unsigned int n_snp, n_snp_done;
    unsigned int n_pair, n_pair_done;
    unsigned int n_pair2, n_pair2_done;
    unsigned int n_stack, n_stack_b, n_stack_done;
    unsigned int paths_next, sites_next;
    unsigned int n_many, max_rows;
    unsigned int ks_need;
    unsigned int err;
    unsigned int err_entrance, err_exit;
    unsigned long long path_head, text_head, sv_head, walk_head;
    unsigned long long max_need, retry_need;
    unsigned long long allele[4], core_cov, core_num, n_called, site_strings;
};

static_assert(offsetof(CallCounters, core_cov) == offsetof(CallCounters, allele) + 32 && offsetof(CallCounters, core_num) == offsetof(CallCounters, allele) + 40, "allele[4], core_cov, core_num are contiguous");

}

namespace pf {
using namespace pf_call;

struct CallState {
    DevBuf flags, plus, minus;
    bool have_state = false;
    DevBuf cov_sum, cov_min, cov_miss;
    bool have_cov = false, per_strand = false;
    uint32_t n_colors = 0, col_words = 1;
    DevBuf col_low, col_up, col_full, col_size, part_first, part_colour, part_word, part_bits;
    DevBuf ccov_sum, ccov_min, ccov_max, ccov_miss;
    std::atomic<uint32_t> sites_ks{0};
    bool pack_alignseq = false;
    bool pack_numeric = false;
    DevBuf side_cnt, side_base, sides, ctask, scan_tmp, target, pending, killed, rstate, rflag, rsmall;
    uint64_t n_sides = 0;
    uint32_t low = 0, up = 0;
    DevBuf kept;
    DevBuf sb_cnt, sb_base, sb_sizes, sb_offs, sb_out;
    uint64_t sb_len = 0;
    uint64_t n_tasks = 0;
    struct AlignOut {
        DevBuf res, otext, osites, ogroups, oilen, sv_off, sv, vc;
        uint64_t t0 = 0;
        uint32_t nb = 0;
        pf_call_result cur = {};
        uint64_t used[5] = {};
        hipEvent_t read_ev[2] = {nullptr, nullptr};
    } lane[PF_CALL_LANES];
    struct AlignWork {
        DevBuf counters, btask, bpath, ptext, queues, blist, slist, plist, plist2, klist, klist_b, stack_scr, pair_scr, pair_scr2, has, scan_tmp, scan_tmp2, paths_scr, sites_scr;
        DevBuf mlist, paths_big_scr;
        uint32_t mlist_cap = 0;
        DevBuf walk_off, walk_pool;
        uint64_t walk_cap = 0;
        hipStream_t stream = nullptr;
        bool own_stream = false;
        hipStream_t side_stream = nullptr;
        hipEvent_t ev_prep = nullptr, ev_paths = nullptr;
    } work[PF_CALL_LANES];
    struct TextWork {
        DevBuf sizes, offs, totals, tcounters, tscan;
        hipStream_t stream = nullptr;
    } text[2];
    std::atomic<uint64_t> path_pool{0}, text_pool{0}, sv_pool{0};
    std::atomic<uint64_t> otext_cap{0}, osites_cap{0}, ogroups_cap{0}, oilen_cap{0};
    DevBuf out[PF_CALL_SLABS];
    uint64_t out_len[PF_CALL_SLABS][N_STREAMS] = {}, out_off[PF_CALL_SLABS][N_STREAMS] = {};
    DevBuf outp[PF_CALL_SLABS];
    const char *fetch_base[PF_CALL_SLABS] = {};
    bool nib[PF_CALL_SLABS] = {};
    uint64_t txt_len[PF_CALL_SLABS][N_STREAMS] = {}, txt_off[PF_CALL_SLABS][N_STREAMS] = {};
    hipStream_t copy_stream = nullptr;
    hipEvent_t fetch_ev[2] = {nullptr, nullptr};
    hipEvent_t text_ev[PF_CALL_SLABS] = {};
    bool mt_format = false;
    std::atomic<uint64_t> fetched_bytes{0};
    struct ModelWork {
        bool active = false;
        int source = 0;
        double q = 0;
        hipStream_t stream = nullptr;
        DevBuf state, flags, ends, nvals, voff, n_rows, scan;
        DevBuf vals[14];
        uint64_t bound[14] = {};
        bool filter = false, taken = false;
        pf::FilterRule rule = {};
        DevBuf cflag, coff, upload, tokens;
        bool each = false, each_done = false;
        DevBuf keys[14], tkeys, ctok;
        uint64_t pooled_n = 0;
        uint32_t color_count = 0;
        uint8_t color_kept[1024] = {};
        hipEvent_t read_ev[PF_CALL_SLABS] = {};
    } model;
    void release_all() {
        for (DevBuf *b : {&model.state, &model.flags, &model.ends, &model.nvals, &model.voff, &model.n_rows, &model.scan, &model.cflag, &model.coff, &model.upload, &model.tokens, &model.tkeys, &model.ctok}) b->release();
        for (DevBuf &b : model.vals) b.release();
        for (DevBuf &b : model.keys) b.release();
        model.each_done = false;
        if (model.stream) { (void)hipStreamDestroy(model.stream); model.stream = nullptr; }
        for (hipEvent_t &e : model.read_ev)
            if (e) { (void)hipEventDestroy(e); e = nullptr; }
        model.active = false;
        DevBuf *all[] = {&col_low, &col_up, &col_full, &col_size, &part_first, &part_colour, &part_word, &part_bits, &ccov_sum, &ccov_min, &ccov_max, &ccov_miss,
                         &flags, &plus, &minus, &cov_sum, &cov_min, &cov_miss, &side_cnt, &side_base, &sides, &ctask, &scan_tmp, &target, &pending, &killed, &rstate, &rflag, &rsmall, &kept, &sb_cnt, &sb_base, &sb_sizes, &sb_offs, &sb_out,
                         };
        for (DevBuf *b : all) b->release();
        for (TextWork &t : text) {
            for (DevBuf *b : {&t.sizes, &t.offs, &t.totals, &t.tcounters, &t.tscan}) b->release();
            if (t.stream) { (void)hipStreamDestroy(t.stream); t.stream = nullptr; }
        }
        for (AlignOut &o : lane) {
            for (DevBuf *b : {&o.res, &o.otext, &o.osites, &o.ogroups, &o.oilen, &o.sv_off, &o.sv, &o.vc}) b->release();
            for (hipEvent_t &e : o.read_ev) if (e) { (void)hipEventDestroy(e); e = nullptr; }
        }
        for (AlignWork &w : work) {
            for (DevBuf *b : {&w.counters, &w.btask, &w.bpath, &w.ptext, &w.queues, &w.blist, &w.slist, &w.plist, &w.plist2, &w.klist, &w.klist_b, &w.stack_scr,
                              &w.pair_scr, &w.pair_scr2, &w.has, &w.scan_tmp, &w.scan_tmp2, &w.paths_scr, &w.sites_scr, &w.mlist, &w.paths_big_scr, &w.walk_off, &w.walk_pool})
                b->release();
            if (w.own_stream && w.stream) (void)hipStreamDestroy(w.stream);
            w.stream = nullptr; w.own_stream = false;
            if (w.side_stream) { (void)hipStreamDestroy(w.side_stream); w.side_stream = nullptr; }
            if (w.ev_prep) { (void)hipEventDestroy(w.ev_prep); w.ev_prep = nullptr; }
            if (w.ev_paths) { (void)hipEventDestroy(w.ev_paths); w.ev_paths = nullptr; }
        }
        for (DevBuf &b : out) b.release();
        for (DevBuf &b : outp) b.release();
        if (copy_stream) { (void)hipStreamDestroy(copy_stream); copy_stream = nullptr; }
        for (hipEvent_t &e : fetch_ev)
            if (e) { (void)hipEventDestroy(e); e = nullptr; }
        for (hipEvent_t &e : text_ev)
            if (e) { (void)hipEventDestroy(e); e = nullptr; }
    }
};
}

namespace pf_call {

__device__ inline bool colour_in(const uint64_t *__restrict__ full, uint32_t words, uint32_t u, uint32_t c) {
    return (full[(size_t)u * words + (c >> 6)] >> (c & 63)) & 1;
}

inline CallState *state_of(pf_ctx *ctx) {
    if (!ctx->call) {
        ctx->call = new CallState();
        if (hipStreamCreateWithFlags(&ctx->call->copy_stream, hipStreamNonBlocking) != hipSuccess) { (void)hipGetLastError(); ctx->call->copy_stream = nullptr; }
    }
    return ctx->call;
}

struct ScanArgs {
    const uint8_t *flags;
    const uint32_t *plus, *minus, *succ, *pred;
    const uint64_t *seq, *off;
    const uint32_t *len;
    uint32_t N;
    int k;
    const uint64_t *cov_sum;
    const uint32_t *cov_min;
    const uint8_t *cov_miss;
    int per_strand;
    uint32_t low, up;
    const uint32_t *side_base;
    pf_call_side *sides;
    CallTask *tasks;
    uint32_t *target;
    uint32_t n_colors;
    const uint64_t *ccov_sum;
    const uint32_t *ccov_min, *ccov_max;
    const uint8_t *ccov_miss;
    const uint32_t *clow, *cup;
    const uint64_t *full, *size_total;
    uint32_t cwords;
};

struct ResolveArgs {
    const pf_call_side *sides;
    const uint32_t *target;
    uint32_t n;
    int *pending;
    uint8_t *killed;
    uint8_t *state;
    uint32_t *flag;
    unsigned int *undecided;
    unsigned int *first_err;
};

struct CallLists {
    uint32_t *queues;
    uint32_t *blist, *slist, *plist, *plist2, *klist, *klist_b;
    uint32_t nb;
};
__device__ inline void wave_append(int key, uint32_t val, const CallLists &L, CallCounters *cnt) {
    unsigned long long todo = __ballot(key != KEY_NONE);
    while (todo) {
        const int x = __shfl(key, __ffsll((long long)todo) - 1, WAVE);
        const unsigned long long m = __ballot(key == x);
        todo &= ~m;
        const int leader = __ffsll((long long)m) - 1;
        uint32_t base = 0;
        uint32_t c_off = (uint32_t)offsetof(CallCounters, n_stack);
        c_off = x == KEY_PAIR2 ? (uint32_t)offsetof(CallCounters, n_pair2) : c_off;
        c_off = x == KEY_PAIR ? (uint32_t)offsetof(CallCounters, n_pair) : c_off;
        c_off = x == KEY_SNP ? (uint32_t)offsetof(CallCounters, n_snp) : c_off;
        c_off = x == KEY_BRANCHING ? (uint32_t)offsetof(CallCounters, n_branching) : c_off;
        c_off = x < NQ ? (uint32_t)offsetof(CallCounters, q_n) + 4u * (uint32_t)x : c_off;
        if (lane_id() == leader)
            base = atomicAdd(reinterpret_cast<unsigned int *>(reinterpret_cast<char *>(cnt) + c_off), (unsigned int)__popcll(m));
        base = __shfl(base, leader, WAVE);
        if (key == x) {
            const uint32_t at = base + (uint32_t)__popcll(m & ((1ull << lane_id()) - 1));
            if (x < NQ) L.queues[(size_t)x * L.nb + at] = val;
            else if (x == KEY_BRANCHING) L.blist[at] = val;
            else if (x == KEY_SNP) L.slist[at] = val;
            else if (x == KEY_PAIR) L.plist[at] = val;
            else if (x == KEY_PAIR2) L.plist2[at] = val;
            else L.klist[at] = val;
        }
    }
}

constexpr int N_KEYS = NQ + 5;
__device__ inline void block_append(int key, uint32_t val, const CallLists &L, CallCounters *cnt) {
    __shared__ uint32_t s_n[4][N_KEYS];
    __shared__ uint32_t s_base[N_KEYS];
    const int lane = lane_id(), wv = (int)(threadIdx.x >> 6);
    if (lane < N_KEYS) s_n[wv][lane] = 0;
    __builtin_amdgcn_fence(__ATOMIC_SEQ_CST, "workgroup");
    __builtin_amdgcn_wave_barrier();
    uint32_t rank = 0;
    unsigned long long todo = __ballot(key != KEY_NONE);
    while (todo) {
        const int x = __shfl(key, __ffsll((long long)todo) - 1, WAVE);
        const unsigned long long m = __ballot(key == x);
        todo &= ~m;
        if (key == x) rank = (uint32_t)__popcll(m & ((1ull << lane) - 1));
        if (lane == __ffsll((long long)m) - 1) s_n[wv][x] = (uint32_t)__popcll(m);
    }
    __syncthreads();
    if (threadIdx.x < (unsigned)N_KEYS) {
        const int x = (int)threadIdx.x;
        const uint32_t total = s_n[0][x] + s_n[1][x] + s_n[2][x] + s_n[3][x];
        uint32_t base = 0;
        if (total) {
            uint32_t c_off = (uint32_t)offsetof(CallCounters, n_stack);
            c_off = x == KEY_PAIR2 ? (uint32_t)offsetof(CallCounters, n_pair2) : c_off;
            c_off = x == KEY_PAIR ? (uint32_t)offsetof(CallCounters, n_pair) : c_off;
            c_off = x == KEY_SNP ? (uint32_t)offsetof(CallCounters, n_snp) : c_off;
            c_off = x == KEY_BRANCHING ? (uint32_t)offsetof(CallCounters, n_branching) : c_off;
            c_off = x < NQ ? (uint32_t)offsetof(CallCounters, q_n) + 4u * (uint32_t)x : c_off;
            base = atomicAdd(reinterpret_cast<unsigned int *>(reinterpret_cast<char *>(cnt) + c_off), total);
        }
        s_base[x] = base;
    }
    __syncthreads();
    if (key != KEY_NONE) {
        uint32_t at = s_base[key] + rank;
        for (int w = 0; w < wv; ++w) at += s_n[w][key];
        if (key < NQ) L.queues[(size_t)key * L.nb + at] = val;
        else if (key == KEY_BRANCHING) L.blist[at] = val;
        else if (key == KEY_SNP) L.slist[at] = val;
        else if (key == KEY_PAIR) L.plist[at] = val;
        else if (key == KEY_PAIR2) L.plist2[at] = val;
        else L.klist[at] = val;
    }
    __syncthreads();
}

struct BatchRef { const CallTask *ct; const uint32_t *kept; uint64_t t0; uint32_t nb; };
struct GraphSeq { const uint64_t *seq, *off; const uint32_t *len; };

struct PrepArgs {
    BatchRef batch;
    const uint32_t *len;
    pf_bubble_task *btask;
    pf_bubble_path *bpath;
    pf_bubble_result *res;
// ... 188 lines not shown
```

ploidyfrost_amd/csrc/pf_ctx.hpp:

```cpp
#pragma once
#include <hip/hip_runtime.h>
#include <stdint.h>

#include <mutex>
#include <string>
#include <vector>

#include "pf_device_common.hpp"
#include "ploidyfrost_hip.h"

namespace pf {
template <typename T>
struct DevTmp {
    T *p = nullptr;
    DevTmp() = default;
    DevTmp(const DevTmp &) = delete;
    DevTmp &operator=(const DevTmp &) = delete;
    ~DevTmp() { if (p) (void)hipFree(p); }
    hipError_t alloc(size_t bytes) { return hipMalloc(reinterpret_cast<void **>(&p), bytes ? bytes : 1); }
};

struct TimedLaunch {
    int kernel;
    hipEvent_t a, b;
    bool closed;
};
struct CallState;

inline bool is_device_ptr(const void *p) {
    hipPointerAttribute_t at;
    const bool dev = p && hipPointerGetAttributes(&at, p) == hipSuccess && at.type == hipMemoryTypeDevice;
    (void)hipGetLastError();
    return dev;
}
}

struct pf_ctx {
    int device = 0;
    int n_cu = 256;
    std::string name;
    std::string err;
    hipStream_t own_stream = nullptr, stream = nullptr;

    uint64_t *d_seq = nullptr;
    uint64_t *d_off = nullptr;
    uint32_t *d_len = nullptr;
    uint32_t N = 0;
    int k = 0;
    uint64_t n_words = 0, n_kmers = 0;
    uint64_t *d_kpre = nullptr;
    uint32_t *d_kwin = nullptr;
    uint64_t n_kwin = 0;
    uint32_t *d_succ = nullptr, *d_pred = nullptr;
    uint32_t *d_pred16 = nullptr;
    bool has_adj = false;
    uint32_t *d_cand = nullptr;
    std::vector<uint32_t> h_cand;
    std::vector<uint32_t> h_len;

    pf::CountLine *d_tab = nullptr;
    uint64_t tab_cap = 0, tab_n = 0;
    hipStream_t join_stream = nullptr;
    hipEvent_t join_done = nullptr;
    bool join_inflight = false;
    hipEvent_t join_c_done = nullptr;
    bool join_c_inflight = false;
    int tab_k = 0;
    bool tab_one_strand = false;
    bool tab_exact = false;
    uint64_t tab_max_count = 0;

    uint32_t *d_gcov = nullptr;
    uint64_t *d_khead = nullptr;
    uint32_t *d_krow = nullptr;
    uint64_t n_krow = 0;
    bool gcov_valid = false;

    uint8_t *d_ctab = nullptr;
    uint64_t ctab_cap = 0;
    uint32_t ctab_line_bytes = 128, n_colors = 0;
    bool ctab_one_strand = false;
    uint64_t ctab_unread = 0;
    uint8_t *d_unread = nullptr;
    uint64_t ctab_max_count = 0;
    uint32_t *d_gcov_c = nullptr;
    uint64_t gcov_c_stride = 0;
    bool gcov_c_valid = false;

    uint64_t *d_cov_sum = nullptr;
    uint32_t *d_cov_min = nullptr;
    uint8_t *d_cov_miss = nullptr;
    uint32_t cov_cap = 0;

    uint64_t gmm_n = 0;
    bool gmm_loaded = false;

    pf::CallState *call = nullptr;
    hipStream_t bub_streams[PF_CALL_LANES][12] = {};
    hipEvent_t bub_events[PF_CALL_LANES][13] = {};

    void *cc = nullptr;
    void *gfa = nullptr;
    void *count = nullptr;
    void *comm = nullptr;
    const void *cc_rec = nullptr;
    const uint32_t *cc_pool = nullptr;
    const pf_bfs_record *bfs_last_rec = nullptr;
    const uint32_t *bfs_last_pool = nullptr;
    uint64_t bfs_last_n = 0, bfs_last_pool_len = 0;
    uint64_t bfs_call_id = 0;
    uint64_t bfs_res_pool_cap = 0;
    hipStream_t copy_stream = nullptr;
    struct {
        bool active = false;
        pf_bfs_record *records = nullptr;
        uint64_t c0 = 0;
        std::vector<uint32_t> deferred;
    } bfs_pending;

    unsigned int bfs_live_n = 0;
    unsigned long long *h_live = nullptr;
    uint64_t live_cap = 0;

    std::vector<std::pair<void *, size_t>> ws;

    bool timing = false;
    uint64_t timing_mask = ~0ull;
    std::vector<hipEvent_t> event_pool;
    std::vector<pf::TimedLaunch> launches;
    size_t side_launch = (size_t)-1;
    size_t main_launch = (size_t)-1;
    std::mutex launch_mu;
    uint64_t units[PF_K_COUNT_] = {};
};

namespace pf {
struct CtxErr {
    pf_ctx *c;
    void operator=(std::string s) const {
        std::lock_guard<std::mutex> lk(c->launch_mu);
        c->err = std::move(s);
    }
};
struct Kc4Args;
int launch_cov_stream(pf_ctx *ctx, Kc4Args a, uint32_t n_colors, bool wide, bool colored);
int ctx_begin(pf_ctx *ctx, int kernel);
void ctx_end(pf_ctx *ctx);
int ctx_begin_on(pf_ctx *ctx, int kernel, hipStream_t stream);
void ctx_end_on(pf_ctx *ctx, hipStream_t stream);
int ctx_begin_at(pf_ctx *ctx, int kernel, hipStream_t stream, size_t *at);
void ctx_end_at(pf_ctx *ctx, size_t at, hipStream_t stream);
inline void ctx_units(pf_ctx *ctx, int kernel, uint64_t n) { if (ctx->timing) __atomic_fetch_add(&ctx->units[kernel], n, __ATOMIC_RELAXED); }
int ctx_grid(const pf_ctx *ctx, uint64_t work_items, int block, int per_cu);
int join_graph_counts(pf_ctx *ctx);
int join_graph_counts_begin(pf_ctx *ctx);
int join_finish(pf_ctx *ctx);
int join_graph_counts_colored_begin(pf_ctx *ctx);
int join_colored_finish(pf_ctx *ctx);
hipStream_t join_stream(pf_ctx *ctx);
int join_graph_counts_colored(pf_ctx *ctx);
void *ctx_ws(pf_ctx *ctx, int slot, size_t bytes);
hipError_t lane_stream_create(hipStream_t *s, int lane);
struct DevLoadTrace {
    bool on = getenv("PF_TRACE_LOAD") != nullptr;
    std::chrono::steady_clock::time_point t = std::chrono::steady_clock::now();
    void mark(const char *what) {
        if (!on) return;
        const auto now = std::chrono::steady_clock::now();
        fprintf(stderr, "[load]   . %-42s %.3fs\n", what, std::chrono::duration<double>(now - t).count());
        t = now;
    }
};
void call_state_create(pf_ctx *ctx);
void call_destroy(pf_ctx *ctx);
void cc_destroy(pf_ctx *ctx);
void gfa_destroy(pf_ctx *ctx);
void comm_destroy(pf_ctx *ctx);
void count_destroy(pf_ctx *ctx);
void call_invalidate(pf_ctx *ctx);
int call_state_arrays(pf_ctx *ctx, uint8_t **flags, uint32_t **plus, uint32_t **minus);
void call_state_resident(pf_ctx *ctx);
enum WsSlot {
    WS_ALN_TEXT = 0, WS_ALN_JOBS, WS_ALN_SMALL, WS_ALN_RETRY, WS_ALN_IDX, WS_ALN_OFIRST, WS_ALN_OCOUNT, WS_ALN_OHITS, WS_ALN_OTEXT,
    WS_ALN_OGAPS, WS_ALN_STTEXT, WS_ALN_STGAPS, WS_ALN_STHITS, WS_ALN_WORK, WS_BFS_REC, WS_BFS_POOL, WS_BFS_SMALL, WS_BFS_DEF, WS_BFS_WLIST,
    WS_BFS_RES_REC, WS_BFS_RES_POOL,
    WS_STR_TEXT, WS_STR_OFF, WS_STR_SUM, WS_STR_OK, WS_STR_MISS,
    WS_BUB_TEXT, WS_BUB_PATHS, WS_BUB_TASKS, WS_BUB_SMALL, WS_BUB_RETRY, WS_BUB_IDX, WS_BUB_RES, WS_BUB_OTEXT, WS_BUB_OSITES,
    WS_BUB_OGROUPS, WS_BUB_OILEN, WS_BUB_SCRATCH, WS_BUB_WORK, WS_BUB_IDX2, WS_CCOV_SUM, WS_CCOV_MIN, WS_CCOV_MAX, WS_CCOV_MISS, WS_GMM_X, WS_GMM_STATE, WS_GMM_PART,
    WS_JOIN_REST, WS_JOIN_REST_N,
    WS_DENSITY,
    WS_MASK_TEXT, WS_MASK_OUT, WS_MASK_BITS, WS_MASK_TABLE, WS_MASK_INDEX,
    WS_BUB_LANES,
    WS_COUNT_ = WS_BUB_LANES + 5 * (PF_CALL_LANES - 1)
};
inline int bub_ws(int slot, int lane) {
    if (lane == 0) return slot;
    const int j = slot == WS_BUB_SMALL ? 0 : slot == WS_BUB_RETRY ? 1 : slot == WS_BUB_SCRATCH ? 2 : slot == WS_BUB_WORK ? 3 : 4;
    return WS_BUB_LANES + 5 * (lane - 1) + j;
}
}
```

ploidyfrost_amd/csrc/pf_device.hip:

```cpp
#include <hip/hip_runtime.h>
#include <sys/mman.h>

#include <algorithm>
#include <cstdio>
#include <cstring>
#include <string>
#include <type_traits>
#include <vector>

#include "pf_cov_stream.hpp"
#include "pf_ctx.hpp"
#include "pf_device_common.hpp"
#include "pf_scan.hpp"
#include "ploidyfrost_hip.h"

using namespace pf;

static std::string g_create_err;

#define PF_HIP(call)                                                                         \
    do {                                                                                     \
        hipError_t e_ = (call);                                                              \
        if (e_ != hipSuccess) {                                                              \
            pf::CtxErr{ctx} = std::string(#call) + ": " + hipGetErrorString(e_);                   \
// ... 570 lines not shown
    if (!rest || !rest_n) { pf::CtxErr{ctx} = "no room for K-COV-JOIN's hand-over list"; return PF_ERR_HIP; }
    if (!ctx->join_done) PF_HIP(hipEventCreateWithFlags(&ctx->join_done, hipEventDisableTiming));
    const hipStream_t st = join_stream(ctx);
    size_t at = 0;
    (void)ctx_begin_at(ctx, PF_K_COV_JOIN, st, &at);
#define PF_JOIN_LAUNCH(KK) k_cov_join<KK><<<blocks, 256, 0, st>>>(ctx->d_tab, ctx->tab_cap - 1, ctx->k, ctx->d_seq, ctx->d_off, ctx->d_kpre, ctx->d_khead, \
        ctx->d_krow, ctx->tab_one_strand, ctx->n_kmers, ctx->d_gcov, rest, rest_n, rest_cap, JOIN_ROWS_PER_WAVE)
    if (ctx->k == 25) PF_JOIN_LAUNCH(25);
    else if (ctx->k == 31) PF_JOIN_LAUNCH(31);
    else PF_JOIN_LAUNCH(0);
#undef PF_JOIN_LAUNCH
    ctx_end_at(ctx, at, st);
    (void)ctx_begin_at(ctx, PF_K_COV_JOIN_REST, st, &at);
    k_cov_join_rest<<<blocks, 256, 0, st>>>(ctx->d_tab, ctx->tab_cap - 1, ctx->k, ctx->tab_one_strand, rest, rest_n, rest_cap, ctx->d_gcov, ctx->d_seq, ctx->d_off,
                                            ctx->d_kpre, ctx->d_khead, ctx->d_krow, ctx->n_kmers, JOIN_ROWS_PER_WAVE);
    ctx_end_at(ctx, at, st);
    PF_HIP(hipGetLastError());
    PF_HIP(hipEventRecord(ctx->join_done, st));
    ctx->join_inflight = true;
    return PF_OK;
}

int join_finish(pf_ctx *ctx) {
    if (!ctx->join_inflight) return PF_OK;
    ctx->join_inflight = false;
    PF_HIP(hipSetDevice(ctx->device));
    PF_HIP(hipEventSynchronize(ctx->join_done));
    ctx->gcov_valid = true;
    return PF_OK;
}

int join_graph_counts(pf_ctx *ctx) {
    const int rc = join_graph_counts_begin(ctx);
    return rc ? rc : join_finish(ctx);
}
}

template <typename T>
static int stage_in(pf_ctx *ctx, const T *src, size_t n, T **dev, bool *owned) {
    *owned = false;
    if (n == 0) { *dev = nullptr; return PF_OK; }
    if (is_device_ptr(src)) {
        *dev = const_cast<T *>(src);
        return PF_OK;
    }
    PF_HIP(hipMalloc(dev, n * sizeof(T)));
    *owned = true;
    PF_HIP(hipMemcpyAsync(*dev, src, n * sizeof(T), hipMemcpyDefault, ctx->stream));
    return PF_OK;
}


extern "C" {

const char *pf_kernel_name(int kernel) { return (kernel >= 0 && kernel < PF_K_COUNT_) ? kKernelNames[kernel] : "?"; }

const char *pf_last_error(const pf_ctx *ctx) {
    if (!ctx) return g_create_err.c_str();
    static thread_local std::string mine;
    {
        std::lock_guard<std::mutex> lk(const_cast<pf_ctx *>(ctx)->launch_mu);
        mine = ctx->err;
    }
    return mine.c_str();
}

int pf_warmup(int device) {
    if (hipSetDevice(device) != hipSuccess) { (void)hipGetLastError(); return PF_ERR_NO_DEVICE; }
    if (hipFree(nullptr) != hipSuccess) { (void)hipGetLastError(); return PF_ERR_HIP; }
    return PF_OK;
}

int pf_create(int device, pf_ctx **out) {
    if (!out) return PF_ERR_ARG;
    *out = nullptr;
    int n = 0;
    if (hipGetDeviceCount(&n) != hipSuccess || n <= 0) {
        g_create_err = "no HIP device visible: the PloidyFrost device layer has no CPU fallback";
        return PF_ERR_NO_DEVICE;
    }
    if (device < 0 || device >= n) { g_create_err = "device index out of range"; return PF_ERR_ARG; }
    hipDeviceProp_t prop;
    if (hipSetDevice(device) != hipSuccess || hipGetDeviceProperties(&prop, device) != hipSuccess) {
        g_create_err = "hipSetDevice / hipGetDeviceProperties failed";
        return PF_ERR_HIP;
    }
    if (std::string(prop.gcnArchName).rfind("gfx950", 0) != 0) {
        g_create_err = std::string("device is ") + prop.gcnArchName + ", this library is built for gfx950 only";
        return PF_ERR_NO_DEVICE;
    }
    pf_ctx *ctx = new pf_ctx();
    ctx->device = device;
    ctx->n_cu = prop.multiProcessorCount;
    ctx->name = prop.name;
    if (hipStreamCreateWithFlags(&ctx->own_stream, hipStreamNonBlocking) != hipSuccess) {
        g_create_err = "hipStreamCreate failed";
        delete ctx;
        return PF_ERR_HIP;
    }
    ctx->stream = ctx->own_stream;
    ctx->ws.resize(WS_COUNT_, {nullptr, 0});
    call_state_create(ctx);
    *out = ctx;
    return PF_OK;
}

static void free_graph(pf_ctx *ctx) {
    call_invalidate(ctx);
    hipFree(ctx->d_seq); hipFree(ctx->d_off); hipFree(ctx->d_len); hipFree(ctx->d_succ); hipFree(ctx->d_pred);
    hipFree(ctx->d_cand);
    hipFree(ctx->d_pred16);
    hipFree(ctx->d_kpre);
    hipFree(ctx->d_kwin);
    hipFree(ctx->d_gcov); hipFree(ctx->d_khead); hipFree(ctx->d_krow); hipFree(ctx->d_gcov_c);
    ctx->d_gcov = nullptr;
    ctx->d_gcov_c = nullptr;
    ctx->gcov_c_valid = false;
    ctx->d_khead = nullptr;
    ctx->d_krow = nullptr;
    ctx->gcov_valid = false;
    ctx->d_kpre = nullptr;
    ctx->d_kwin = nullptr;
    ctx->d_pred16 = nullptr;
    ctx->d_seq = ctx->d_off = nullptr;
    ctx->d_len = ctx->d_succ = ctx->d_pred = ctx->d_cand = nullptr;
    ctx->h_cand.clear();
    ctx->has_adj = false;
}

void pf_destroy(pf_ctx *ctx) {
    if (!ctx) return;
    hipSetDevice(ctx->device);
    hipStreamSynchronize(ctx->stream);
    if (ctx->join_stream) { hipStreamSynchronize(ctx->join_stream); hipStreamDestroy(ctx->join_stream); }
    if (ctx->join_done) hipEventDestroy(ctx->join_done);
    if (ctx->join_c_done) hipEventDestroy(ctx->join_c_done);
    for (auto &tl : ctx->launches) { hipEventDestroy(tl.a); hipEventDestroy(tl.b); }
    for (auto &e : ctx->event_pool) hipEventDestroy(e);
    call_destroy(ctx);
    cc_destroy(ctx);
    gfa_destroy(ctx);
    comm_destroy(ctx);
    count_destroy(ctx);
    free_graph(ctx);
    hipFree(ctx->d_tab);
    hipFree(ctx->d_ctab);
    hipFree(ctx->d_unread);
    hipFree(ctx->d_cov_sum); hipFree(ctx->d_cov_min); hipFree(ctx->d_cov_miss);
    for (auto &w : ctx->ws) hipFree(w.first);
    if (ctx->h_live) hipHostFree(ctx->h_live);
    if (ctx->copy_stream) { hipStreamSynchronize(ctx->copy_stream); hipStreamDestroy(ctx->copy_stream); }
    for (auto &lane : ctx->bub_streams) for (auto &s : lane) if (s) hipStreamDestroy(s);
    for (auto &lane : ctx->bub_events) for (auto &e : lane) if (e) hipEventDestroy(e);
    hipStreamDestroy(ctx->own_stream);
    delete ctx;
}

int pf_set_stream(pf_ctx *ctx, void *s) {
    if (!ctx) return PF_ERR_ARG;
    ctx->stream = s ? (hipStream_t)s : ctx->own_stream;
    return PF_OK;
}

int pf_synchronize(pf_ctx *ctx) {
    if (!ctx) return PF_ERR_ARG;
    PF_HIP(hipStreamSynchronize(ctx->stream));
    return PF_OK;
}

int pf_enable_timing(pf_ctx *ctx, int on) {
    if (!ctx) return PF_ERR_ARG;
    ctx->timing = on != 0;
    return PF_OK;
}

int pf_timing_select(pf_ctx *ctx, uint64_t kernel_mask) {
    if (!ctx) return PF_ERR_ARG;
    ctx->timing_mask = kernel_mask;
    return PF_OK;
}

int pf_reset_timing(pf_ctx *ctx) {
    if (!ctx) return PF_ERR_ARG;
    PF_HIP(hipSetDevice(ctx->device));
    PF_HIP(hipDeviceSynchronize());
    std::lock_guard<std::mutex> lk(ctx->launch_mu);
    for (auto &tl : ctx->launches) { ctx->event_pool.push_back(tl.a); ctx->event_pool.push_back(tl.b); }
    ctx->launches.clear();
    memset(ctx->units, 0, sizeof(ctx->units));
    return PF_OK;
}

int pf_kernel_units(pf_ctx *ctx, int kernel, uint64_t *units) {
    if (!ctx || kernel < 0 || kernel >= PF_K_COUNT_ || !units) return PF_ERR_ARG;
    *units = ctx->units[kernel];
    return PF_OK;
}

int pf_kernel_time(pf_ctx *ctx, int kernel, double *total_ms, uint64_t *launches) {
    if (!ctx || kernel < 0 || kernel >= PF_K_COUNT_) return PF_ERR_ARG;
    PF_HIP(hipStreamSynchronize(ctx->stream));
    double tot = 0;
    uint64_t n = 0;
    for (auto &tl : ctx->launches) {
        if (tl.kernel != kernel || !tl.closed) continue;
        float ms = 0;
        PF_HIP(hipEventElapsedTime(&ms, tl.a, tl.b));
        tot += ms;
        n++;
    }
    if (total_ms) *total_ms = tot;
    if (launches) *launches = n;
    return PF_OK;
}

static int busy_union(pf_ctx *ctx, uint64_t kernel_mask, double *busy_ms, double *span_ms) {
    if (!ctx) return PF_ERR_ARG;
    PF_HIP(hipSetDevice(ctx->device));
    PF_HIP(hipDeviceSynchronize());
    std::vector<std::pair<float, float>> iv;
    size_t unread = 0;
    {
        std::lock_guard<std::mutex> lk(ctx->launch_mu);
        iv.reserve(ctx->launches.size());
        for (auto &tl : ctx->launches) {
            float a = 0, b = 0;
            if (!((kernel_mask >> tl.kernel) & 1ull)) continue;
            if (!tl.closed) { ++unread; continue; }
            if (hipEventElapsedTime(&a, ctx->launches[0].a, tl.a) != hipSuccess || hipEventElapsedTime(&b, ctx->launches[0].a, tl.b) != hipSuccess) {
                (void)hipGetLastError();
                ++unread;
                continue;
            }
            if (b > a) iv.emplace_back(a, b);
        }
    }
    std::sort(iv.begin(), iv.end());
    double busy = 0, lo = 0, hi = 0;
    bool open = false;
    for (auto &x : iv) {
        if (!open) { lo = x.first; hi = x.second; open = true; }
        else if (x.first <= hi) hi = std::max<double>(hi, x.second);
        else { busy += hi - lo; lo = x.first; hi = x.second; }
    }
    if (open) busy += hi - lo;
    if (busy_ms) *busy_ms = busy;
    if (span_ms) {
        float mx = 0;
        for (auto &x : iv) mx = std::max(mx, x.second);
        *span_ms = iv.empty() ? 0.0 : (double)mx - (double)iv.front().first;
    }
    if (unread) {
        pf::CtxErr{ctx} = "pf_device_busy: " + std::to_string(unread) + " launch intervals could not be read (busy_ms leaves them out)";
        return PF_ERR_HIP;
    }
    return PF_OK;
}

int pf_device_busy(pf_ctx *ctx, double *busy_ms, double *span_ms) { return busy_union(ctx, ~0ull, busy_ms, span_ms); }
int pf_kernel_busy(pf_ctx *ctx, uint64_t kernel_mask, double *busy_ms) { return busy_union(ctx, kernel_mask, busy_ms, nullptr); }

namespace {
std::mutex g_host_mu;
std::vector<std::pair<void *, size_t>> g_host_maps;
}
int pf_host_alloc(pf_ctx *ctx, size_t bytes, void **out) {
    if (!ctx || !out) return PF_ERR_ARG;
    PF_HIP(hipSetDevice(ctx->device));
    const size_t page = 1u << 21;
    const size_t size = ((bytes ? bytes : 1) + page - 1) & ~(page - 1);
    void *p = mmap(nullptr, size, PROT_READ | PROT_WRITE, MAP_PRIVATE | MAP_ANONYMOUS | MAP_POPULATE, -1, 0);
    if (p != MAP_FAILED) {
        if (hipHostRegister(p, size, hipHostRegisterDefault) == hipSuccess) {
            std::lock_guard<std::mutex> lk(g_host_mu);
            g_host_maps.emplace_back(p, size);
            *out = p;
            return PF_OK;
        }
        (void)hipGetLastError();
        munmap(p, size);
    }
    PF_HIP(hipHostMalloc(out, bytes ? bytes : 1, hipHostMallocNonCoherent));
    return PF_OK;
}

int pf_fetch(pf_ctx *ctx, void *dst_host, const void *src_dev, uint64_t bytes) {
    if (!ctx || (bytes && (!dst_host || !src_dev))) return PF_ERR_ARG;
    PF_HIP(hipSetDevice(ctx->device));
    if (bytes) PF_HIP(hipMemcpy(dst_host, src_dev, bytes, hipMemcpyDeviceToHost));
    return PF_OK;
}

void pf_host_free(pf_ctx *ctx, void *p) {
    (void)ctx;
    if (!p) return;
    size_t size = 0;
    {
        std::lock_guard<std::mutex> lk(g_host_mu);
        for (size_t i = 0; i < g_host_maps.size(); ++i)
            if (g_host_maps[i].first == p) { size = g_host_maps[i].second; g_host_maps.erase(g_host_maps.begin() + (long)i); break; }
    }
    if (size) { (void)hipHostUnregister(p); munmap(p, size); }
    else hipHostFree(p);
}

int pf_device_name(pf_ctx *ctx, char *buf, size_t cap) {
// ... 431 lines not shown
```

Before: 244.7 million.

## Split bubble launch into enqueue/collect and overlap two bubble calls per lane

Splits bubble_launch into bubble_enqueue and bubble_collect so the alignment driver can queue a second bubble batch (slot 1) while the first is still running. It adds per-slot retry, work and index buffers plus pinned host retry counters, so the host does not block on a pageable copy. The global-memory big-bubble kernel now runs on the least-loaded train stream instead of after all trains on the caller stream. The cost is more workspace, more complex error/drain handling, and a risk of contention between overlapped batches.

Result: slower. 237.0 million (-3.2%).

```diff
diff --git a/ploidyfrost_amd/csrc/pf_bubble.hip b/ploidyfrost_amd/csrc/pf_bubble.hip
--- a/ploidyfrost_amd/csrc/pf_bubble.hip
+++ b/ploidyfrost_amd/csrc/pf_bubble.hip
@@ -710,7 +710,8 @@
 
 namespace pf {
 
-unsigned long long *bubble_pool_heads(pf_ctx *ctx, int lane) { return (unsigned long long *)ctx_ws(ctx, bub_ws(WS_BUB_SMALL, lane), 128); }
+constexpr size_t kBubSmallBytes = 256;
+unsigned long long *bubble_pool_heads(pf_ctx *ctx, int lane) { return (unsigned long long *)ctx_ws(ctx, bub_ws(WS_BUB_SMALL, lane), kBubSmallBytes); }
 
 constexpr int kBubTrains = 3;
 static int bubble_streams(pf_ctx *ctx, int lane) {
@@ -720,6 +721,7 @@
         PF_HIP(hipEventCreateWithFlags(&ctx->bub_events[lane][c], hipEventDisableTiming));
     }
     PF_HIP(hipEventCreateWithFlags(&ctx->bub_events[lane][kBubLdsClasses], hipEventDisableTiming));
+    if (!ctx->bub_h_retry[lane]) PF_HIP(hipHostMalloc((void **)&ctx->bub_h_retry[lane], 64, hipHostMallocDefault));
     return PF_OK;
 }
 static int bubble_func_attr(pf_ctx *ctx) {
@@ -731,7 +733,8 @@
 int bubble_reserve(pf_ctx *ctx, uint32_t n_tasks, int lane) {
     const BubCaps std_caps{64 * 1024, 8 * 1024, 512, 16 * 1024, 128 * 1024, 256, 8 * 1024};
     const uint64_t per = (bub_scratch_bytes(std_caps) + 255) & ~255ull;
-    if (!ctx_ws(ctx, bub_ws(WS_BUB_SMALL, lane), 128) || !ctx_ws(ctx, bub_ws(WS_BUB_RETRY, lane), (size_t)std::max<uint32_t>(n_tasks, 1) * 4) ||
+    if (!ctx_ws(ctx, bub_ws(WS_BUB_SMALL, lane), kBubSmallBytes) || !ctx_ws(ctx, bub_ws(WS_BUB_RETRY, lane), (size_t)std::max<uint32_t>(n_tasks, 1) * 4) ||
+        !ctx_ws(ctx, bub_ws(WS_BUB_RETRY, lane, 1), (size_t)std::max<uint32_t>(n_tasks, 1) * 4) ||
         !ctx_ws(ctx, bub_ws(WS_BUB_SCRATCH, lane), per * (uint64_t)ctx->n_cu * 24))
         return PF_ERR_HIP;
     DevLoadTrace trace;
@@ -739,8 +742,8 @@
     trace.mark("bubble: class streams");
     { const int e = bubble_func_attr(ctx); if (e != PF_OK) return e; }
     trace.mark("bubble: function attributes");
-    uint8_t *small = (uint8_t *)ctx_ws(ctx, bub_ws(WS_BUB_SMALL, lane), 128);
-    PF_HIP(hipMemsetAsync(small, 0, 128, ctx->bub_streams[lane][0]));
+    uint8_t *small = (uint8_t *)ctx_ws(ctx, bub_ws(WS_BUB_SMALL, lane), kBubSmallBytes);
+    PF_HIP(hipMemsetAsync(small, 0, kBubSmallBytes, ctx->bub_streams[lane][0]));
     PF_HIP(hipStreamSynchronize(ctx->bub_streams[lane][0]));
     BubParams p;
     memset(&p, 0, sizeof(p));
@@ -754,43 +757,63 @@
     return PF_OK;
 }
 
-int bubble_launch(pf_ctx *ctx, const BubbleLaunch &L, unsigned long long heads[4]) {
+struct BubSetup {
+    BubParams p;
+    BubOut o;
+    uint8_t *tail;
+    unsigned int *queue_heads;
+};
+static const BubCaps kStdCaps{64 * 1024, 8 * 1024, 512, 16 * 1024, 128 * 1024, 256, 8 * 1024};
+
+static int bubble_setup(pf_ctx *ctx, const BubbleLaunch &L, BubSetup &B) {
+    uint8_t *small = (uint8_t *)ctx_ws(ctx, bub_ws(WS_BUB_SMALL, L.lane), kBubSmallBytes);
+    uint32_t *d_retry = (uint32_t *)ctx_ws(ctx, bub_ws(WS_BUB_RETRY, L.lane, L.slot), (size_t)std::max<uint32_t>(L.n_tasks, 1) * 4);
+    if (!small || !d_retry) return PF_ERR_HIP;
+    B.tail = small + 128 * (size_t)L.slot;
+    BubOut &o = B.o;
+    o.res = L.out.res; o.text = L.out.otext; o.sites = L.out.osites; o.groups = L.out.ogroups; o.ilen = L.out.oilen;
+    o.text_cap = L.out.text_cap; o.site_cap = L.out.site_cap; o.group_cap = L.out.group_cap; o.ilen_cap = L.out.ilen_cap;
+    o.heads = reinterpret_cast<unsigned long long *>(small);
+    o.n_retry = reinterpret_cast<unsigned int *>(B.tail + 40);
+    B.queue_heads = reinterpret_cast<unsigned int *>(B.tail + 64);
+    o.retry = d_retry;
+    BubParams &p = B.p;
+    memset(&p, 0, sizeof(p));
+    p.text = L.text; p.paths = L.paths; p.tasks = L.tasks; p.M = L.match; p.D = L.mismatch; p.G = L.gap;
+    p.integral = (L.match == std::floor(L.match) && L.mismatch == std::floor(L.mismatch) && L.gap == std::floor(L.gap) &&
+                  std::fabs(L.match) < 1e6 && std::fabs(L.mismatch) < 1e6 && std::fabs(L.gap) < 1e6) ? 1 : 0;
+    p.seq = ctx->d_seq; p.off = ctx->d_off; p.len = ctx->d_len; p.n_unitigs = ctx->N;
+    p.caps = kStdCaps;
+    p.scratch_per_wave = (bub_scratch_bytes(kStdCaps) + 255) & ~255ull;
+    return PF_OK;
+}
+
+int bubble_enqueue(pf_ctx *ctx, const BubbleLaunch &L, BubblePending &P) {
+    P = BubblePending{};
+    P.L = L;
+    if (L.slot < 0 || L.slot > 1 || (L.slot == 1 && !L.keep_heads)) return PF_ERR_ARG;
     const int lane = L.lane;
     hipStream_t st = L.stream ? L.stream : ctx->stream;
     size_t tl_at = (size_t)-1;
     auto tbegin = [&](int kernel, hipStream_t s) { (void)ctx_begin_at(ctx, kernel, s, &tl_at); };
     auto tend = [&](hipStream_t s) { ctx_end_at(ctx, tl_at, s); };
-    uint8_t *small = (uint8_t *)ctx_ws(ctx, bub_ws(WS_BUB_SMALL, lane), 128);
-    uint32_t *d_retry = (uint32_t *)ctx_ws(ctx, bub_ws(WS_BUB_RETRY, lane), (size_t)std::max<uint32_t>(L.n_tasks, 1) * 4);
-    if (!small || !d_retry) return PF_ERR_HIP;
-    if (L.keep_heads) PF_HIP(hipMemsetAsync(small + 32, 0, 96, st));
-    else PF_HIP(hipMemsetAsync(small, 0, 128, st));
-    BubOut o;
-    o.res = L.out.res; o.text = L.out.otext; o.sites = L.out.osites; o.groups = L.out.ogroups; o.ilen = L.out.oilen;
-    o.text_cap = L.out.text_cap; o.site_cap = L.out.site_cap; o.group_cap = L.out.group_cap; o.ilen_cap = L.out.ilen_cap;
-    o.heads = reinterpret_cast<unsigned long long *>(small);
-    o.n_retry = reinterpret_cast<unsigned int *>(small + 40);
-    unsigned int *queue_heads = reinterpret_cast<unsigned int *>(small + 64);
-    int n_launch = 0;
-    o.retry = d_retry;
-
-    BubParams p;
-    memset(&p, 0, sizeof(p));
-    p.text = L.text; p.paths = L.paths; p.tasks = L.tasks; p.M = L.match; p.D = L.mismatch; p.G = L.gap;
-    p.integral = (L.match == std::floor(L.match) && L.mismatch == std::floor(L.mismatch) && L.gap == std::floor(L.gap) &&
-                  std::fabs(L.match) < 1e6 && std::fabs(L.mismatch) < 1e6 && std::fabs(L.gap) < 1e6) ? 1 : 0;
-    p.seq = ctx->d_seq; p.off = ctx->d_off; p.len = ctx->d_len; p.n_unitigs = ctx->N;
-    const BubCaps std_caps{64 * 1024, 8 * 1024, 512, 16 * 1024, 128 * 1024, 256, 8 * 1024};
-    constexpr bool class_streams = true;
+    BubSetup B;
+    { const int e = bubble_setup(ctx, L, B); if (e != PF_OK) return e; }
+    if (L.slot == 0 && !L.keep_heads) PF_HIP(hipMemsetAsync(B.tail, 0, 128, st));
+    else PF_HIP(hipMemsetAsync(B.tail + 32, 0, 96, st));
+    BubParams &p = B.p;
+    BubOut &o = B.o;
+    unsigned int *queue_heads = B.queue_heads;
+    int &n_launch = P.n_launch;
     constexpr int kTrains = kBubTrains;
-    int grids[kBubLdsClasses];
+    int *grids = P.grids;
     int train_of[kBubLdsClasses];
     int order[kBubLdsClasses];
     int n_order = 0;
     const uint64_t wave_budget = (uint64_t)ctx->n_cu * 24;
     const uint64_t train_waves = wave_budget / kTrains;
+    double load[kTrains] = {0, 0, 0};
     {
-        double load[kTrains] = {0, 0, 0};
         for (int c = 0; c < kBubLdsClasses; ++c) {
             grids[c] = 0;
             train_of[c] = 0;
@@ -805,12 +828,10 @@
                 if (load[q] < load[tr]) tr = q;
             train_of[c] = tr;
             load[tr] += work_of(c);
-            grids[c] = (int)std::min<uint64_t>(std::min<uint64_t>(L.n_cls[c], (uint64_t)ctx->n_cu * bubble_class_waves_per_cu(c)), class_streams ? train_waves : wave_budget);
+            grids[c] = (int)std::min<uint64_t>(std::min<uint64_t>(L.n_cls[c], (uint64_t)ctx->n_cu * bubble_class_waves_per_cu(c)), train_waves);
         }
     }
     const uint64_t max_waves = wave_budget;
-    p.caps = std_caps;
-    p.scratch_per_wave = (bub_scratch_bytes(std_caps) + 255) & ~255ull;
     const bool trace_ws = getenv("PF_TRACE_ALIGN") != nullptr;
     const auto t_ws = std::chrono::steady_clock::now();
     uint8_t *const scratch0 = (uint8_t *)ctx_ws(ctx, bub_ws(WS_BUB_SCRATCH, lane), p.scratch_per_wave * max_waves);
@@ -819,23 +840,26 @@
                 (double)(p.scratch_per_wave * max_waves) / 1e6, std::chrono::duration<double>(std::chrono::steady_clock::now() - t_ws).count() * 1e3);
     p.scratch = scratch0;
     if (!p.scratch) return PF_ERR_HIP;
-    if (class_streams) { const int e = bubble_streams(ctx, lane); if (e != PF_OK) return e; }
-
-    DevTmp<unsigned long long> clk_;
-    unsigned long long *d_clk = nullptr;
+    { const int e = bubble_streams(ctx, lane); if (e != PF_OK) return e; }
+
     const bool want_clk = getenv("PF_BUBBLE_STATS") != nullptr;
     if (want_clk) {
-        PF_HIP(clk_.alloc(((size_t)L.n_tasks + 16) * 8));
-        d_clk = clk_.p;
-        PF_HIP(hipMemsetAsync(d_clk, 0, ((size_t)L.n_tasks + 16) * 8, st));
-        p.task_clk = d_clk;
-        p.prof = d_clk + L.n_tasks;
+        PF_HIP(hipMalloc(&P.d_clk, ((size_t)L.n_tasks + 16) * 8));
+        PF_HIP(hipMemsetAsync(P.d_clk, 0, ((size_t)L.n_tasks + 16) * 8, st));
+        p.task_clk = P.d_clk;
+        p.prof = P.d_clk + L.n_tasks;
     }
     { const int e = bubble_func_attr(ctx); if (e != PF_OK) return e; }
     uint32_t idx_off = 0;
     for (int c = 0; c < kBubLdsClasses; ++c) idx_off += L.n_cls[c];
-    if (class_streams) PF_HIP(hipEventRecord(ctx->bub_events[lane][kBubLdsClasses], st));
+    PF_HIP(hipEventRecord(ctx->bub_events[lane][kBubLdsClasses], st));
     bool train_used[kTrains] = {false, false, false};
+    auto train_stream = [&](int tr) -> hipStream_t {
+        hipStream_t cst = ctx->bub_streams[lane][tr];
+        if (!train_used[tr] && hipStreamWaitEvent(cst, ctx->bub_events[lane][kBubLdsClasses], 0) != hipSuccess) return nullptr;
+        train_used[tr] = true;
+        return cst;
+    };
     for (int i = 0; i < n_order; ++i) {
         const int c = order[i];
         const uint32_t nc = L.n_cls[c];
@@ -846,46 +870,67 @@
         p.work_bytes = (uint32_t)kBubClassBytes[c];
         const int grid = grids[c];
         p.next = queue_heads + n_launch++;
-        hipStream_t cst = st;
-        if (class_streams) {
-            const int tr = train_of[c];
-            cst = ctx->bub_streams[lane][tr];
-            if (!train_used[tr]) PF_HIP(hipStreamWaitEvent(cst, ctx->bub_events[lane][kBubLdsClasses], 0));
-            train_used[tr] = true;
-            p.scratch = scratch0 + (uint64_t)tr * train_waves * p.scratch_per_wave;
-        }
+        const int tr = train_of[c];
+        hipStream_t cst = train_stream(tr);
+        if (!cst) { pf::CtxErr{ctx} = "bubble_enqueue: a train stream could not wait for its caller"; return PF_ERR_HIP; }
+        p.scratch = scratch0 + (uint64_t)tr * train_waves * p.scratch_per_wave;
         tbegin(PF_K_BUBBLE, cst);
         k_bubble<true><<<grid, 64, kBubClassBytes[c], cst>>>(p, o);
         tend(cst);
         ctx_units(ctx, PF_K_BUBBLE, nc);
     }
-    if (class_streams)
-        for (int tr = 0; tr < kTrains; ++tr) {
-            if (!train_used[tr]) continue;
-            PF_HIP(hipEventRecord(ctx->bub_events[lane][tr], ctx->bub_streams[lane][tr]));
-            PF_HIP(hipStreamWaitEvent(st, ctx->bub_events[lane][tr], 0));
-        }
-    p.scratch = scratch0;
     if (L.n_cls[kBubLdsClasses]) {
         const uint32_t nc = L.n_cls[kBubLdsClasses];
-        const int grid = (int)std::min<uint32_t>(nc, 256);
+        const int grid = (int)std::min<uint64_t>(std::min<uint32_t>(nc, 256), std::max<uint64_t>(train_waves, 1));
         const uint64_t per = (std::min<uint64_t>(L.max_need * 2, 1ull << 31) + 255) & ~255ull;
-        uint8_t *work = (uint8_t *)ctx_ws(ctx, bub_ws(WS_BUB_WORK, lane), per * grid);
+        uint8_t *work = (uint8_t *)ctx_ws(ctx, bub_ws(WS_BUB_WORK, lane, L.slot), per * grid);
         if (!work) return PF_ERR_HIP;
+        int tr = 0;
+        for (int q = 1; q < kTrains; ++q)
+            if (load[q] < load[tr]) tr = q;
+        hipStream_t cst = train_stream(tr);
+        if (!cst) { pf::CtxErr{ctx} = "bubble_enqueue: a train stream could not wait for its caller"; return PF_ERR_HIP; }
+        p.scratch = scratch0 + (uint64_t)tr * train_waves * p.scratch_per_wave;
         p.idx = L.idx + idx_off;
         p.n = nc;
         p.work = work;
         p.work_per_wave = per;
         p.work_bytes = (uint32_t)std::min<uint64_t>(per, 0xFFFFFFFFu);
         p.next = queue_heads + n_launch++;
-        tbegin(PF_K_BUBBLE_BIG, st);
-        k_bubble<false><<<grid, 64, 0, st>>>(p, o);
-        tend(st);
+        tbegin(PF_K_BUBBLE_BIG, cst);
+        k_bubble<false><<<grid, 64, 0, cst>>>(p, o);
+        tend(cst);
         ctx_units(ctx, PF_K_BUBBLE_BIG, nc);
     }
-    unsigned int n_retry = 0;
-    PF_HIP(hipMemcpyAsync(&n_retry, o.n_retry, 4, hipMemcpyDeviceToHost, st));
+    for (int tr = 0; tr < kTrains; ++tr) {
+        if (!train_used[tr]) continue;
+        PF_HIP(hipEventRecord(ctx->bub_events[lane][tr], ctx->bub_streams[lane][tr]));
+        PF_HIP(hipStreamWaitEvent(st, ctx->bub_events[lane][tr], 0));
+    }
+    PF_HIP(hipGetLastError());
+    PF_HIP(hipMemcpyAsync(ctx->bub_h_retry[lane] + L.slot, o.n_retry, 4, hipMemcpyDeviceToHost, st));
+    P.enqueued = true;
+    return PF_OK;
+}
+
+int bubble_collect(pf_ctx *ctx, BubblePending &P, unsigned long long heads[4]) {
+    if (!P.enqueued) return PF_ERR_ARG;
+    P.enqueued = false;
+    const BubbleLaunch &L = P.L;
+    const int lane = L.lane;
+    hipStream_t st = L.stream ? L.stream : ctx->stream;
+    size_t tl_at = (size_t)-1;
+    auto tbegin = [&](int kernel, hipStream_t s) { (void)ctx_begin_at(ctx, kernel, s, &tl_at); };
+    auto tend = [&](hipStream_t s) { ctx_end_at(ctx, tl_at, s); };
+    BubSetup B;
+    { const int e = bubble_setup(ctx, L, B); if (e != PF_OK) return e; }
+    BubParams &p = B.p;
+    BubOut &o = B.o;
+    unsigned long long *const d_clk = P.d_clk;
+    struct ClkFree { unsigned long long *&q; ~ClkFree() { if (q) { (void)hipFree(q); q = nullptr; } } } clk_free{P.d_clk};
+    if (d_clk) { p.task_clk = d_clk; p.prof = d_clk + L.n_tasks; }
     PF_HIP(hipStreamSynchronize(st));
+    const unsigned int n_retry = P.n_retry = ctx->bub_h_retry[lane][L.slot];
     int status = PF_OK;
     DevTmp<uint8_t> big_scratch_, big_work_;
     DevTmp<unsigned int> bad_;
@@ -899,13 +944,13 @@
         PF_HIP(big_work_.alloc(per_w * grid));
         PF_HIP(bad_.alloc(4));
         PF_HIP(hipMemsetAsync(bad_.p, 0, 4, st));
-        uint32_t *d_q = (uint32_t *)ctx_ws(ctx, bub_ws(WS_BUB_IDX2, lane), (size_t)n_retry * 4);
+        uint32_t *d_q = (uint32_t *)ctx_ws(ctx, bub_ws(WS_BUB_IDX2, lane, L.slot), (size_t)n_retry * 4);
         if (!d_q) return PF_ERR_HIP;
-        PF_HIP(hipMemcpyAsync(d_q, d_retry, (size_t)n_retry * 4, hipMemcpyDeviceToDevice, st));
+        PF_HIP(hipMemcpyAsync(d_q, o.retry, (size_t)n_retry * 4, hipMemcpyDeviceToDevice, st));
         p.idx = d_q; p.n = n_retry; p.caps = big; p.scratch = big_scratch_.p; p.scratch_per_wave = per_s;
         p.work = big_work_.p; p.work_per_wave = per_w; p.work_bytes = (uint32_t)per_w; p.final_tier = 1;
         p.bad = bad_.p;
-        p.next = queue_heads + n_launch++;
+        p.next = B.queue_heads + P.n_launch++;
         tbegin(PF_K_BUBBLE_BIG, st);
         k_bubble<false><<<grid, 64, 0, st>>>(p, o);
         tend(st);
@@ -917,7 +962,7 @@
             status = PF_ERR_OVERFLOW;
         }
     }
-    if (want_clk) {
+    if (d_clk) {
         const uint32_t n_tasks = L.n_tasks;
         std::vector<unsigned long long> clk(n_tasks + 16);
         PF_HIP(hipMemcpy(clk.data(), d_clk, ((size_t)n_tasks + 16) * 8, hipMemcpyDeviceToHost));
@@ -938,8 +983,8 @@
                 at += L.n_cls[c];
                 if (L.n_cls[c])
                     fprintf(stderr, "   class %d (%s): %u bubbles on %d wavefronts, %llu ticks (%.2f ms if spread evenly), longest %llu ticks\n", c,
-                            c == kBubLdsClasses ? "global" : "LDS", L.n_cls[c], c < kBubLdsClasses ? grids[c] : 0, sum,
-                            c < kBubLdsClasses && grids[c] ? (double)sum / grids[c] * 1e-5 : 0.0, mx);
+                            c == kBubLdsClasses ? "global" : "LDS", L.n_cls[c], c < kBubLdsClasses ? P.grids[c] : 0, sum,
+                            c < kBubLdsClasses && P.grids[c] ? (double)sum / P.grids[c] * 1e-5 : 0.0, mx);
             }
         }
         std::vector<unsigned long long> srt(clk);
@@ -982,12 +1027,29 @@
             clk[t] = 0;
         }
     }
-    PF_HIP(hipMemcpy(heads, o.heads, 32, hipMemcpyDeviceToHost));
+    PF_HIP(hipMemcpyAsync(heads, o.heads, 32, hipMemcpyDeviceToHost, st));
+    PF_HIP(hipStreamSynchronize(st));
     if (status == PF_OK && (heads[0] > L.out.text_cap || heads[1] > L.out.site_cap || heads[2] > L.out.group_cap || heads[3] > L.out.ilen_cap)) {
         pf::CtxErr{ctx} = "pf_align_bubbles: output pools too small";
         status = PF_ERR_OVERFLOW;
     }
     return status;
+}
+
+int bubble_launch(pf_ctx *ctx, const BubbleLaunch &L, unsigned long long heads[4]) {
+    BubblePending P;
+    const int e = bubble_enqueue(ctx, L, P);
+    if (e != PF_OK) {
+        if (P.d_clk) { (void)hipFree(P.d_clk); P.d_clk = nullptr; }
+        return e;
+    }
+    return bubble_collect(ctx, P, heads);
+}
+
+int bubble_drain(pf_ctx *ctx, int lane) {
+    for (int c = 0; c < kBubTrains; ++c)
+        if (ctx->bub_streams[lane][c]) PF_HIP(hipStreamSynchronize(ctx->bub_streams[lane][c]));
+    return PF_OK;
 }
 
 }
diff --git a/ploidyfrost_amd/csrc/pf_bubble_launch.hpp b/ploidyfrost_amd/csrc/pf_bubble_launch.hpp
--- a/ploidyfrost_amd/csrc/pf_bubble_launch.hpp
+++ b/ploidyfrost_amd/csrc/pf_bubble_launch.hpp
@@ -54,6 +54,16 @@
     bool keep_heads = false;
     int lane = 0;
     hipStream_t stream = nullptr;
+    int slot = 0;
+};
+
+struct BubblePending {
+    BubbleLaunch L;
+    int n_launch = 0;
+    int grids[kBubLdsClasses] = {};
+    unsigned long long *d_clk = nullptr;
+    unsigned int n_retry = 0;
+    bool enqueued = false;
 };
 
 unsigned long long *bubble_pool_heads(pf_ctx *ctx, int lane = 0);
@@ -64,7 +74,10 @@
     return integral && M >= D && M + 1 >= 2 * (G + 1) && D - 2 * G - 2 > 0;
 }
 
+int bubble_enqueue(pf_ctx *ctx, const BubbleLaunch &L, BubblePending &P);
+int bubble_collect(pf_ctx *ctx, BubblePending &P, unsigned long long heads[4]);
 int bubble_launch(pf_ctx *ctx, const BubbleLaunch &L, unsigned long long heads[4]);
+int bubble_drain(pf_ctx *ctx, int lane);
 int bubble_reserve(pf_ctx *ctx, uint32_t n_tasks, int lane = 0);
 
 }
diff --git a/ploidyfrost_amd/csrc/pf_call.hip b/ploidyfrost_amd/csrc/pf_call.hip
--- a/ploidyfrost_amd/csrc/pf_call.hip
+++ b/ploidyfrost_amd/csrc/pf_call.hip
@@ -390,14 +390,14 @@
 
 int ensure_batch_buffers(pf_ctx *ctx, const char *who, CallState::AlignWork &W, CallState::AlignOut &O, uint32_t nb) {
     const size_t list = (size_t)nb * 4;
-    return need(ctx, who, {{&W.counters, sizeof(CallCounters)}, {&W.btask, (size_t)nb * sizeof(pf_bubble_task)}, {&W.queues, (size_t)NQ * list},
+    return need(ctx, who, {{&W.counters, 2 * sizeof(CallCounters)}, {&W.btask, (size_t)nb * sizeof(pf_bubble_task)}, {&W.queues, 2 * (size_t)NQ * list},
                            {&W.blist, list}, {&W.slist, list}, {&W.plist, list}, {&W.plist2, list}, {&W.klist, list}, {&W.klist_b, list}, {&W.has, list},
                            {&O.res, (size_t)nb * sizeof(pf_bubble_result)}, {&O.sv_off, (size_t)nb * 8}, {&O.vc, list}});
 }
 
 int ensure_wave_scratch(pf_ctx *ctx, const char *who, CallState::AlignWork &W, const CallGrids &g, uint32_t depth, bool stack_tier, bool pair_tier) {
     PF_TRY(need(ctx, who, {{&W.paths_scr, paths_per_wave(depth) * g.paths}}));
-    if (stack_tier) PF_TRY(need(ctx, who, {{&W.stack_scr, stack_scratch_bytes() * g.stack}}));
+    if (stack_tier) PF_TRY(need(ctx, who, {{&W.stack_scr, stack_scratch_bytes() * g.stack}, {&W.stack_scr_b, stack_scratch_bytes() * g.stack}}));
     if (pair_tier) PF_TRY(need(ctx, who, {{&W.pair_scr, PairGeom<PAIR_MAX>::scratch_bytes * g.pair}}));
     return PF_OK;
 }
@@ -415,6 +415,7 @@
         PF_HIP(lane_stream_create(&W.side_stream, lane));
         PF_HIP(hipEventCreateWithFlags(&W.ev_prep, hipEventDisableTiming));
         PF_HIP(hipEventCreateWithFlags(&W.ev_paths, hipEventDisableTiming));
+        PF_HIP(hipEventCreateWithFlags(&W.ev_snp, hipEventDisableTiming));
     }
     return PF_OK;
 }
@@ -469,10 +470,15 @@
     const bool stack_tier = stack_scores(match, mismatch, gap);
     const int stack_ok = stack_tier ? std::max(1, std::min(3, env_int("PF_STACK_LEVEL", 1))) : 0;
     const int paths_force_scratch = env_int("PF_PATHS_SCRATCH", 0) ? 1 : 0;
+    const bool split = chains_split();
+    const uint32_t pools_divide = (uint32_t)std::max(1, env_int("PF_FIRST_POOLS_DIVIDE", 1));
     const CallGrids grids = call_grids(ctx->n_cu);
     const uint32_t depth;
     hipStream_t st = nullptr;
+    hipStream_t pst = nullptr;
     CallCounters *d_cnt = nullptr;
+    CallCounters *d_cnt_b = nullptr;
+    uint32_t *queues_b = nullptr;
     BatchRef batch = {};
     GraphSeq graph = {};
     CallLists lists = {};
@@ -482,14 +488,19 @@
     PairArgs pr = {};
     int attempt = 0;
     CallCounters hc = {};
+    CallCounters hb = {};
     unsigned long long heads[4] = {0, 0, 0, 0};
     uint64_t n_jobs = 0;
+    BubblePending pend_strict, pend_branch;
+    struct SitePlan { uint32_t ks = 0; uint64_t rows_cap = 0, per_wave = 0, sv_cap = 0; int grid = 0; } site_plan;
+    bool sites_enqueued = false;
     uint32_t n_called = 0;
     size_t tl_at = (size_t)-1;
 
     AlignCall(pf_ctx *c, int lane_, uint64_t t0_, uint32_t nb_, uint32_t complex_size, double m, double d, double g)
         : ctx(c), S(c->call), W(c->call->work[lane_]), O(c->call->lane[lane_]), lane(lane_), t0(t0_), nb(nb_), match(m), mismatch(d), gap(g), depth(depth_cap(complex_size)) {}
 
+    static bool chains_split() { const char *e = getenv("PF_CALL_CHAINS"); return e && strcmp(e, "split") == 0; }
     void tbegin(int kernel, hipStream_t s) { (void)ctx_begin_at(ctx, kernel, s, &tl_at); }
     void tend(hipStream_t s) { ctx_end_at(ctx, tl_at, s); }
 
@@ -502,6 +513,10 @@
         if (W.mlist_cap < MANY_LIST_MIN) W.mlist_cap = MANY_LIST_MIN;
         PF_TRY(need(ctx, who, {{&W.mlist, (size_t)W.mlist_cap * 4}}));
         d_cnt = W.counters.as<CallCounters>();
+        d_cnt_b = split ? d_cnt + 1 : d_cnt;
+        queues_b = W.queues.as<uint32_t>() + (split ? (size_t)NQ * nb : 0);
+        pst = W.side_stream;
+        if (split) PF_TRY(need(ctx, who, {{&W.scan_tmp2, (size_t)nb * 4}}));
         batch = BatchRef{S->ctask.as<CallTask>(), S->kept.as<uint32_t>(), t0, nb};
         graph = GraphSeq{ctx->d_seq, ctx->d_off, ctx->d_len};
         lists = CallLists{W.queues.as<uint32_t>(), W.blist.as<uint32_t>(), W.slist.as<uint32_t>(), W.plist.as<uint32_t>(), W.plist2.as<uint32_t>(), W.klist.as<uint32_t>(), W.klist_b.as<uint32_t>(), nb};
@@ -514,12 +529,20 @@
         l.path_pool = S->path_pool; l.path_text = S->text_pool; l.row_text = S->otext_cap; l.sites = S->osites_cap; l.groups = S->ogroups_cap; l.ilen = S->oilen_cap;
         l.walk = W.walk_cap;
         cap = batch_pools(nb, grids, l, S->n_colors != 0);
+        if (pools_divide > 1) {
+            cap.path_text = std::max<uint64_t>(l.path_text, cap.path_text / pools_divide);
+            cap.row_text = std::max<uint64_t>(l.row_text, cap.row_text / pools_divide);
+            cap.sites = std::max<uint64_t>(l.sites, cap.sites / pools_divide);
+            cap.groups = std::max<uint64_t>(l.groups, cap.groups / pools_divide);
+            cap.ilen = std::max<uint64_t>(l.ilen, cap.ilen / pools_divide);
+        }
         PF_TRY(ensure_pools(ctx, who, W, O, nb, cap));
         unsigned long long *d_heads = bubble_pool_heads(ctx, lane);
         if (!d_heads) return PF_ERR_HIP;
         pools = RowPools{O.res.as<pf_bubble_result>(), O.otext.as<char>(), cap.row_text, O.osites.as<pf_bubble_site>(), cap.sites, O.ogroups.as<uint8_t>(), cap.groups,
                          O.oilen.as<uint32_t>(), cap.ilen, d_heads};
-        PF_HIP(hipMemsetAsync(d_cnt, 0, sizeof(CallCounters), st));
+        PF_HIP(hipMemsetAsync(d_cnt, 0, 2 * sizeof(CallCounters), st));
+        sites_enqueued = false;
         PF_HIP(hipMemsetAsync(d_heads, 0, 32, st));
         return PF_OK;
     }
@@ -531,7 +554,6 @@
         tbegin(PF_K_CALL_PREP, st);
         k_call_prep<<<(nb + 255) / 256, 256, 0, st>>>(pa);
         tend(st);
-        hipStream_t pst = W.side_stream;
         PF_HIP(hipEventRecord(W.ev_prep, st));
         PF_HIP(hipStreamWaitEvent(pst, W.ev_prep, 0));
         ph = PathArgs{};
@@ -540,17 +562,35 @@
         ph.max_paths = MAX_PATHS; ph.n_list = &d_cnt->n_branching; ph.mlist = W.mlist.as<uint32_t>(); ph.mlist_cap = W.mlist_cap;
         ph.walk_pool = S->n_colors ? W.walk_pool.as<uint32_t>() : nullptr; ph.walk_off = W.walk_off.as<uint64_t>(); ph.walk_cap = cap.walk;
         ph.btask = pa.btask; ph.bpath = pa.bpath; ph.path_cap = cap.path_pool; ph.text = W.ptext.as<char>(); ph.text_cap = cap.path_text;
-        ph.queues = lists.queues; ph.klist = lists.klist_b; ph.stack_ok = stack_ok; ph.cnt = d_cnt;
+        ph.queues = queues_b; ph.klist = lists.klist_b; ph.stack_ok = stack_ok; ph.cnt = d_cnt_b;
         tbegin(PF_K_CALL_PATHS, pst);
         k_call_paths<false><<<grids.paths, 64, 0, pst>>>(ph);
         tend(pst);
-        PF_HIP(hipEventRecord(W.ev_paths, pst));
+        StackArgs skb;
+        if (stack_tier) {
+            skb.list = lists.klist_b; skb.n_list = &d_cnt_b->n_stack_b; skb.scratch = W.stack_scr_b.as<uint8_t>(); skb.pair_ok = 0;
+            skb.btask = pa.btask; skb.bpath = pa.bpath; skb.ptext = W.ptext.as<char>(); skb.graph = graph;
+            skb.M = (int)match; skb.D = (int)mismatch; skb.G = (int)gap;
+            skb.out = pools; skb.lists = lists; skb.lists.queues = queues_b; skb.cnt = d_cnt_b;
+        }
+        if (!split) PF_HIP(hipEventRecord(W.ev_paths, pst));
         if (snp_ok) {
             SnpArgs sn;
             sn.batch = batch; sn.slist = lists.slist; sn.graph = graph; sn.out = pools; sn.lists = lists; sn.pair_ok = pa.pair_ok; sn.stack_ok = stack_ok; sn.cnt = d_cnt;
             tbegin(PF_K_CALL_SNP, st);
             k_call_snp<<<(nb + 255) / 256, 256, 0, st>>>(sn);
             tend(st);
+        }
+        if (split) {
+            if (snp_ok) {
+                PF_HIP(hipEventRecord(W.ev_snp, st));
+                PF_HIP(hipStreamWaitEvent(pst, W.ev_snp, 0));
+            }
+            if (stack_tier) {
+                tbegin(PF_K_CALL_STACK, pst);
+                k_call_stack<<<grids.stack, 64, 0, pst>>>(skb);
+                tend(pst);
+            }
         }
         StackArgs sk;
         if (stack_tier) {
@@ -577,11 +617,11 @@
             if (pair_stats) PF_TRY(print_pair_stats(ctx, prof));
             pr.prof = nullptr;
         }
+        if (split) return PF_OK;
         PF_HIP(hipStreamWaitEvent(st, W.ev_paths, 0));
         if (stack_tier) {
-            sk.list = lists.klist_b; sk.n_list = &d_cnt->n_stack_b; sk.pair_ok = 0;
             tbegin(PF_K_CALL_STACK, st);
-            k_call_stack<<<grids.stack, 64, 0, st>>>(sk);
+            k_call_stack<<<grids.stack, 64, 0, st>>>(skb);
             tend(st);
         }
         return PF_OK;
@@ -591,7 +631,25 @@
         PF_HIP(hipGetLastError());
         PF_HIP(hipMemcpyAsync(&hc, d_cnt, sizeof(hc), hipMemcpyDeviceToHost, st));
         PF_HIP(hipStreamSynchronize(st));
+        if (!split) hb = hc;
         return PF_OK;
+    }
+    int read_branch_counters() {
+        PF_HIP(hipGetLastError());
+        unsigned int n_branching = 0;
+        PF_HIP(hipMemcpyAsync(&hb, d_cnt_b, sizeof(hb), hipMemcpyDeviceToHost, pst));
+        PF_HIP(hipMemcpyAsync(&n_branching, &d_cnt->n_branching, 4, hipMemcpyDeviceToHost, pst));
+        PF_HIP(hipStreamSynchronize(pst));
+        hb.n_branching = n_branching;
+        return PF_OK;
+    }
+    void drain() {
+        (void)hipStreamSynchronize(st);
+        (void)hipStreamSynchronize(pst);
+        (void)bubble_drain(ctx, lane);
+        if (pend_strict.d_clk) { (void)hipFree(pend_strict.d_clk); pend_strict.d_clk = nullptr; }
+        if (pend_branch.d_clk) { (void)hipFree(pend_branch.d_clk); pend_branch.d_clk = nullptr; }
+        pend_strict.enqueued = pend_branch.enqueued = false;
     }
 
     int launch_pair_tier2() {
@@ -617,51 +675,52 @@
         ctx_units(ctx, PF_K_CALL_PREP, nb);
         if (snp_ok) ctx_units(ctx, PF_K_CALL_SNP, hc.n_snp);
         if (pair_tier) ctx_units(ctx, PF_K_CALL_PAIR, hc.n_pair + hc.n_pair2);
-        if (stack_tier) ctx_units(ctx, PF_K_CALL_STACK, hc.n_stack + hc.n_stack_b);
-        ctx_units(ctx, PF_K_CALL_PATHS, hc.n_branching);
-        if (trace.on) fprintf(stderr, "[pf_call_align] bubbles of more than 255 walks: %u, err %u\n", hc.n_many, hc.err);
+        if (stack_tier) ctx_units(ctx, PF_K_CALL_STACK, hc.n_stack + hb.n_stack_b);
+        ctx_units(ctx, PF_K_CALL_PATHS, hb.n_branching);
+        if (trace.on) fprintf(stderr, "[pf_call_align] bubbles of more than 255 walks: %u, err %u\n", hb.n_many, hb.err);
     }
 
     int launch_paths_big(bool *retry) {
-        if (!hc.n_many || (hc.err & ERR_WALK)) return PF_OK;
-        if (hc.n_many > W.mlist_cap) {
-            W.mlist_cap = grown_many(hc.n_many);
+        if (!hb.n_many || (hb.err & ERR_WALK)) return PF_OK;
+        if (hb.n_many > W.mlist_cap) {
+            W.mlist_cap = grown_many(hb.n_many);
             *retry = true;
             return need(ctx, who, {{&W.mlist, (size_t)W.mlist_cap * 4}});
         }
-        const int big_grid = paths_big_grid(hc.n_many);
+        const int big_grid = paths_big_grid(hb.n_many);
         const uint64_t big_per_wave = paths_big_per_wave(depth, PATHS_BIG);
         PF_TRY(need(ctx, who, {{&W.paths_big_scr, big_per_wave * big_grid}}));
         PathArgs pb = ph;
-        pb.blist = W.mlist.as<uint32_t>(); pb.n_list = &d_cnt->n_many; pb.max_paths = PATHS_BIG; pb.mlist = nullptr; pb.mlist_cap = 0;
+        pb.blist = W.mlist.as<uint32_t>(); pb.n_list = &d_cnt_b->n_many; pb.max_paths = PATHS_BIG; pb.mlist = nullptr; pb.mlist_cap = 0;
         pb.scratch = W.paths_big_scr.as<uint8_t>(); pb.scratch_per_wave = big_per_wave;
-        tbegin(PF_K_CALL_PATHS, st);
-        k_call_paths<true><<<big_grid, 64, 0, st>>>(pb);
-        tend(st);
-        return read_counters();
+        hipStream_t bst = split ? pst : st;
+        tbegin(PF_K_CALL_PATHS, bst);
+        k_call_paths<true><<<big_grid, 64, 0, bst>>>(pb);
+        tend(bst);
+        return split ? read_branch_counters() : read_counters();
     }
 
     int accept_walks(bool *retry) {
-        if (hc.err & ERR_WALK) {
+        if (hb.err & ERR_WALK) {
             char where[96];
-            snprintf(where, sizeof where, " (superbubble from unitig %u%c to unitig %u%c)", (hc.err_entrance >> 1) + 1, (hc.err_entrance & 1) ? '-' : '+',
-                     (hc.err_exit >> 1) + 1, (hc.err_exit & 1) ? '-' : '+');
-            pf::CtxErr{ctx} = std::string(hc.err & ERR_MANY_PATHS ? "pf_call_run: a bubble has more than 65535 paths" : "pf_call_run: a bubble is deeper than the complex size allows") + where;
+            snprintf(where, sizeof where, " (superbubble from unitig %u%c to unitig %u%c)", (hb.err_entrance >> 1) + 1, (hb.err_entrance & 1) ? '-' : '+',
+                     (hb.err_exit >> 1) + 1, (hb.err_exit & 1) ? '-' : '+');
+            pf::CtxErr{ctx} = std::string(hb.err & ERR_MANY_PATHS ? "pf_call_run: a bubble has more than 65535 paths" : "pf_call_run: a bubble is deeper than the complex size allows") + where;
             return PF_ERR_ARG;
         }
         amax(S->otext_cap, cap.row_text); amax(S->osites_cap, cap.sites);
         amax(S->ogroups_cap, cap.groups); amax(S->oilen_cap, cap.ilen);
         amax(S->path_pool, cap.path_pool);
         amax(S->text_pool, cap.path_text);
-        const uint64_t rows_need = row_text_need(hc.text_head, hc.n_branching, nb);
+        const uint64_t rows_need = row_text_need(hb.text_head, hb.n_branching, nb);
         if (trace.on)
             fprintf(stderr, "[pf_call_align] attempt %d: %u bubbles, path pool %llu of %llu, path text %llu of %llu, rows text cap %llu (needs %llu)\n", attempt, nb,
-                    (unsigned long long)hc.path_head, (unsigned long long)cap.path_pool, (unsigned long long)hc.text_head, (unsigned long long)cap.path_text,
+                    (unsigned long long)hb.path_head, (unsigned long long)cap.path_pool, (unsigned long long)hb.text_head, (unsigned long long)cap.path_text,
                     (unsigned long long)cap.row_text, (unsigned long long)rows_need);
-        if (hc.path_head > cap.path_pool || hc.text_head > cap.path_text || hc.walk_head > cap.walk) {
-            amax(S->path_pool, grown(hc.path_head, 1024));
-            amax(S->text_pool, grown(hc.text_head, 4096));
-            if (S->n_colors) W.walk_cap = std::max<uint64_t>(W.walk_cap, grown(hc.walk_head, 1024));
+        if (hb.path_head > cap.path_pool || hb.text_head > cap.path_text || hb.walk_head > cap.walk) {
+            amax(S->path_pool, grown(hb.path_head, 1024));
+            amax(S->text_pool, grown(hb.text_head, 4096));
+            if (S->n_colors) W.walk_cap = std::max<uint64_t>(W.walk_cap, grown(hb.walk_head, 1024));
             *retry = true;
             return PF_OK;
         }
@@ -673,29 +732,30 @@
         return PF_OK;
     }
 
-    int run_bubble(bool *retry) {
-        n_jobs = 0;
-        for (int x = 0; x < NQ; ++x) n_jobs += hc.q_n[x];
-        PF_TRY(need(ctx, who, {{&W.scan_tmp2, std::max<size_t>((size_t)n_jobs, 1) * 4}}));
-        uint32_t *d_idx = W.scan_tmp2.as<uint32_t>();
+    int enqueue_bubble(BubblePending &P, int slot, hipStream_t on, const CallCounters &c, const uint32_t *queues, uint32_t *d_idx, uint64_t *jobs) {
+        uint64_t n = 0;
+        for (int x = 0; x < NQ; ++x) n += c.q_n[x];
+        *jobs = n;
+        if (split && n == 0) return PF_OK;
         size_t at = 0;
         for (int x = 0; x < NQ; ++x) {
-            if (!hc.q_n[x]) continue;
-            PF_HIP(hipMemcpyAsync(d_idx + at, W.queues.as<uint32_t>() + (size_t)x * nb, (size_t)hc.q_n[x] * 4, hipMemcpyDeviceToDevice, st));
-            at += hc.q_n[x];
+            if (!c.q_n[x]) continue;
+            PF_HIP(hipMemcpyAsync(d_idx + at, queues + (size_t)x * nb, (size_t)c.q_n[x] * 4, hipMemcpyDeviceToDevice, on));
+            at += c.q_n[x];
         }
         BubbleLaunch BL;
         BL.text = W.ptext.as<char>(); BL.paths = W.bpath.as<pf_bubble_path>(); BL.tasks = W.btask.as<pf_bubble_task>();
         BL.n_tasks = nb; BL.idx = d_idx;
-        for (int c = 0; c <= kBubLdsClasses; ++c) BL.n_cls[c] = hc.q_n[2 * c] + hc.q_n[2 * c + 1];
-        BL.max_need = hc.max_need; BL.retry_need = hc.retry_need;
+        for (int k = 0; k <= kBubLdsClasses; ++k) BL.n_cls[k] = c.q_n[2 * k] + c.q_n[2 * k + 1];
+        BL.max_need = c.max_need; BL.retry_need = c.retry_need;
         BL.match = match; BL.mismatch = mismatch; BL.gap = gap;
         BL.out = pools;
         BL.keep_heads = true;
-        BL.lane = lane; BL.stream = st;
-        trace.stage("K-BUBBLE launching");
-        const int bst = bubble_launch(ctx, BL, heads);
-        trace.stage("K-BUBBLE done");
+        BL.lane = lane; BL.stream = on; BL.slot = slot;
+        return bubble_enqueue(ctx, BL, P);
+    }
+
+    int judge_bubble(int bst, bool *retry) {
         if (trace.on)
             fprintf(stderr, "[pf_call_align] attempt %d: K-BUBBLE status %d, pools text %llu of %llu, sites %llu of %llu, groups %llu of %llu, indel lengths %llu of %llu\n", attempt, bst,
                     heads[0], (unsigned long long)cap.row_text, heads[1], (unsigned long long)cap.sites, heads[2], (unsigned long long)cap.groups, heads[3], (unsigned long long)cap.ilen);
@@ -709,6 +769,59 @@
         }
         return bst;
     }
+    bool heads_fit() const { return heads[0] <= cap.row_text && heads[1] <= cap.sites && heads[2] <= cap.groups && heads[3] <= cap.ilen; }
+
+    int run_bubble(bool *retry) {
+        PF_TRY(need(ctx, who, {{&W.scan_tmp2, std::max<size_t>((size_t)jobs_s_of(hc), 1) * 4}}));
+        trace.stage("K-BUBBLE launching");
+        int bst = enqueue_bubble(pend_strict, 0, st, hc, W.queues.as<uint32_t>(), W.scan_tmp2.as<uint32_t>(), &n_jobs);
+        if (bst == PF_OK) bst = bubble_collect(ctx, pend_strict, heads);
+        trace.stage("K-BUBBLE done");
+        return judge_bubble(bst, retry);
+    }
+
+    int attempt_joined(bool *retry) {
+        PF_TRY(read_counters());
+        trace.stage("K-PREP .. K-STACK done");
+        PF_TRY(launch_pair_tier2());
+        note_units();
+        PF_TRY(launch_paths_big(retry));
+        if (!*retry) PF_TRY(accept_walks(retry));
+        if (!*retry) PF_TRY(run_bubble(retry));
+        return PF_OK;
+    }
+
+    int attempt_split(bool *retry) {
+        PF_TRY(read_branch_counters());
+        trace.stage("K-PATHS, K-STACK (branching) done");
+        PF_TRY(launch_paths_big(retry));
+        if (!*retry) PF_TRY(accept_walks(retry));
+        if (*retry) return PF_OK;
+        uint32_t *d_idx = W.scan_tmp2.as<uint32_t>();
+        uint64_t jobs_b = 0, jobs_s = 0;
+        PF_TRY(enqueue_bubble(pend_branch, 1, pst, hb, queues_b, d_idx, &jobs_b));
+        trace.stage("K-BUBBLE (branching) enqueued");
+        PF_TRY(read_counters());
+        trace.stage("K-PREP .. K-PAIR done");
+        PF_TRY(launch_pair_tier2());
+        note_units();
+        PF_TRY(enqueue_bubble(pend_strict, 0, st, hc, W.queues.as<uint32_t>(), d_idx + (nb - jobs_s_of(hc)), &jobs_s));
+        trace.stage("K-BUBBLE (strict) enqueued");
+        n_jobs = jobs_b + jobs_s;
+        int bst = PF_OK;
+        if (pend_branch.enqueued) bst = bubble_collect(ctx, pend_branch, heads);
+        else { PF_HIP(hipMemcpyAsync(heads, pools.heads, 32, hipMemcpyDeviceToHost, pst)); PF_HIP(hipStreamSynchronize(pst)); }
+        if (bst != PF_OK && bst != PF_ERR_OVERFLOW) return bst;
+        if (bst == PF_OK && hb.n_branching && heads_fit()) PF_TRY(enqueue_sites());
+        int sst = PF_OK;
+        if (pend_strict.enqueued) sst = bubble_collect(ctx, pend_strict, heads);
+        else { PF_HIP(hipMemcpyAsync(heads, pools.heads, 32, hipMemcpyDeviceToHost, st)); PF_HIP(hipStreamSynchronize(st)); }
+        trace.stage("K-BUBBLE done");
+        if (bst == PF_OK) bst = sst;
+        if (bst == PF_OK && !heads_fit()) bst = PF_ERR_OVERFLOW;
+        return judge_bubble(bst, retry);
+    }
+    static uint64_t jobs_s_of(const CallCounters &c) { uint64_t n = 0; for (int x = 0; x < NQ; ++x) n += c.q_n[x]; return n; }
 
     int number_called() {
         k_call_has<<<(nb + 255) / 256, 256, 0, st>>>(O.res.as<pf_bubble_result>(), nb, W.has.as<uint32_t>());
@@ -734,33 +847,60 @@
         return sa;
     }
 
-    int launch_sites(SiteArgs &sa, int grid) {
+    int launch_sites(SiteArgs &sa, int grid, hipStream_t on) {
         static const bool sites_stats = getenv("PF_SITES_STATS") != nullptr;
         DevTmp<unsigned long long> prof;
-        if (sites_stats) PF_TRY(stats_begin(ctx, prof, (size_t)grid * 6, st, &sa.prof));
-        PF_HIP(hipMemsetAsync(&d_cnt->sites_next, 0, 4, st));
-        PF_HIP(hipMemsetAsync(&d_cnt->sv_head, 0, 8, st));
-        PF_HIP(hipMemsetAsync(&d_cnt->site_strings, 0, 8, st));
-        tbegin(PF_K_CALL_SITES, st);
-        if (sa.n_colors) k_call_sites<true><<<grid, 64, 0, st>>>(sa);
-        else k_call_sites<false><<<grid, 64, 0, st>>>(sa);
-        tend(st);
-        ctx_units(ctx, PF_K_CALL_SITES, hc.n_branching);
-        if (sites_stats) { PF_HIP(hipGetLastError()); PF_TRY(print_sites_stats(ctx, prof, grid, st)); }
-        return read_counters();
+        if (sites_stats) PF_TRY(stats_begin(ctx, prof, (size_t)grid * 6, on, &sa.prof));
+        PF_HIP(hipMemsetAsync(&d_cnt->sites_next, 0, 4, on));
+        PF_HIP(hipMemsetAsync(&d_cnt->sv_head, 0, 8, on));
+        PF_HIP(hipMemsetAsync(&d_cnt->site_strings, 0, 8, on));
+        tbegin(PF_K_CALL_SITES, on);
+        if (sa.n_colors) k_call_sites<true><<<grid, 64, 0, on>>>(sa);
+        else k_call_sites<false><<<grid, 64, 0, on>>>(sa);
+        tend(on);
+        ctx_units(ctx, PF_K_CALL_SITES, hb.n_branching);
+        if (sites_stats) { PF_HIP(hipGetLastError()); PF_TRY(print_sites_stats(ctx, prof, grid, on)); }
+        return PF_OK;
+    }
+
+    int plan_sites(uint32_t ks) {
+        site_plan.ks = ks;
+        site_plan.rows_cap = sites_rows_cap(hb.max_rows);
+        site_plan.per_wave = sites_per_wave(site_plan.rows_cap, ks, S->n_colors, S->col_words);
+        site_plan.grid = call_sites_grid(hb.n_branching, grids, site_plan.per_wave);
+        site_plan.sv_cap = site_values_cap(S->n_colors, hb.n_branching, site_plan.grid, S->sv_pool);
+        return need(ctx, who, {{&W.sites_scr, site_plan.per_wave * site_plan.grid}, {&O.sv, site_plan.sv_cap * 8}});
+    }
+
+    int enqueue_sites() {
+        PF_TRY(plan_sites(std::max<uint32_t>(first_site_string(ctx->k), S->sites_ks.load())));
+        SiteArgs sa = site_args(site_plan.ks, site_plan.rows_cap, site_plan.per_wave, site_plan.sv_cap);
+        PF_TRY(launch_sites(sa, site_plan.grid, pst));
+        sites_enqueued = true;
+        trace.stage("K-SITES enqueued");
+        return PF_OK;
+    }
+
+    int join_chains() {
+        if (!split) return PF_OK;
+        PF_HIP(hipEventRecord(W.ev_paths, pst));
+        PF_HIP(hipStreamWaitEvent(st, W.ev_paths, 0));
+        return PF_OK;
     }
 
     int run_sites() {
         uint32_t KS = std::max<uint32_t>(first_site_string(ctx->k), S->sites_ks.load());
-        const uint32_t C = S->n_colors;
-        const uint64_t rows_cap = sites_rows_cap(hc.max_rows);
         for (int sv_attempt = 0, ks_attempt = 0;;) {
-            const uint64_t per_wave = sites_per_wave(rows_cap, KS, C, S->col_words);
-            const int grid = call_sites_grid(hc.n_branching, grids, per_wave);
-            const uint64_t sv_cap = site_values_cap(C, hc.n_branching, grid, S->sv_pool);
-            PF_TRY(need(ctx, who, {{&W.sites_scr, per_wave * grid}, {&O.sv, sv_cap * 8}}));
-            SiteArgs sa = site_args(KS, rows_cap, per_wave, sv_cap);
-            PF_TRY(launch_sites(sa, grid));
+            if (sites_enqueued) {
+                sites_enqueued = false;
+                KS = site_plan.ks;
+            } else {
+                PF_TRY(plan_sites(KS));
+                SiteArgs sa = site_args(KS, site_plan.rows_cap, site_plan.per_wave, site_plan.sv_cap);
+                PF_TRY(launch_sites(sa, site_plan.grid, st));
+            }
+            const uint64_t sv_cap = site_plan.sv_cap;
+            PF_TRY(read_counters());
             if (hc.err & ERR_SITE_LONG) {
                 if (++ks_attempt > 3 || hc.ks_need <= KS) { pf::CtxErr{ctx} = "pf_call_run: the room for a site string does not converge"; return PF_ERR_OVERFLOW; }
                 KS = grown_site_string(hc.ks_need);
@@ -807,34 +947,36 @@
         if (A.attempt > 5) { pf::CtxErr{ctx} = "pf_call_align: pools do not converge"; return PF_ERR_OVERFLOW; }
         bool retry = false;
         PF_TRY(A.size_pools());
-        PF_TRY(A.launch_tiers());
-        PF_TRY(A.read_counters());
-        A.trace.stage("K-PREP .. K-STACK done");
-        PF_TRY(A.launch_pair_tier2());
-        A.note_units();
-        PF_TRY(A.launch_paths_big(&retry));
-        if (!retry) PF_TRY(A.accept_walks(&retry));
-        if (!retry) PF_TRY(A.run_bubble(&retry));
+        int ast = A.launch_tiers();
+        if (ast == PF_OK) ast = A.split ? A.attempt_split(&retry) : A.attempt_joined(&retry);
+        if (A.split && (retry || ast != PF_OK)) A.drain();
+        if (ast != PF_OK) return ast;
         if (!retry) break;
     }
     const CallCounters &hc = A.hc;
-    out->n_branching = hc.n_branching;
-    out->align_jobs = A.n_jobs + hc.n_snp_done + hc.n_pair_done + hc.n_pair2_done + hc.n_stack_done;
-    out->snp_jobs = hc.n_snp_done; out->pair_jobs = hc.n_pair_done + hc.n_pair2_done; out->wave_jobs = A.n_jobs; out->stack_jobs = hc.n_stack_done;
-    PF_TRY(A.number_called());
-    if (hc.n_branching) {
-        PF_TRY(A.run_sites());
-    } else {
-        PF_TRY(need(ctx, A.who, {{&O.sv, 16}}));
-        PF_HIP(hipStreamSynchronize(A.st));
-    }
+    const CallCounters &hb = A.hb;
+    out->n_branching = hb.n_branching;
+    const uint32_t stack_done = hc.n_stack_done + (A.split ? hb.n_stack_done : 0);
+    out->align_jobs = A.n_jobs + hc.n_snp_done + hc.n_pair_done + hc.n_pair2_done + stack_done;
+    out->snp_jobs = hc.n_snp_done; out->pair_jobs = hc.n_pair_done + hc.n_pair2_done; out->wave_jobs = A.n_jobs; out->stack_jobs = stack_done;
+    int fst = A.join_chains();
+    if (fst == PF_OK) fst = A.number_called();
+    if (fst == PF_OK) {
+        if (hb.n_branching) {
+            fst = A.run_sites();
+        } else {
+            fst = need(ctx, A.who, {{&O.sv, 16}});
+            if (fst == PF_OK && hipStreamSynchronize(A.st) != hipSuccess) { pf::CtxErr{ctx} = "pf_call_align: hipStreamSynchronize"; fst = PF_ERR_HIP; }
+        }
+    }
+    if (fst != PF_OK) { if (A.split) A.drain(); return fst; }
     out->site_strings = hc.site_strings;
     A.trace.stage("K-SITES done");
     out->n_called = A.n_called;
     O.nb = A.nb;
     O.cur = *out;
     for (int x = 0; x < 4; ++x) O.used[x] = A.heads[x];
-    O.used[4] = hc.n_branching ? hc.sv_head : 0;
+    O.used[4] = hb.n_branching ? hc.sv_head : 0;
     return PF_OK;
 }
 
@@ -890,7 +1032,8 @@
         PF_TRY(ensure_batch_buffers(ctx, who, W, O, nb));
         PF_TRY(ensure_wave_scratch(ctx, who, W, grids, depth_cap(complex_size), true, true));
         PF_TRY(ensure_pools(ctx, who, W, O, nb, batch_pools(nb, grids, LearntPools{}, false)));
-        PF_TRY(need(ctx, who, {{&W.scan_tmp2, reserve_job_index_bytes(nb)}, {&W.sites_scr, sites_per_wave(256, first_site_string(31), 0, 1) * grids.sites},
+        PF_TRY(need(ctx, who, {{&W.scan_tmp2, std::max<uint64_t>(reserve_job_index_bytes(nb), (uint64_t)nb * 4)},
+                                {&W.sites_scr, sites_per_wave(256, first_site_string(31), 0, 1) * grids.sites},
                                {&O.sv, reserve_site_values(nb, grids) * 8}}));
         trace.mark("reserve: a lane's buffers");
         PF_TRY(ensure_lane_streams(ctx, W, lane));
diff --git a/ploidyfrost_amd/csrc/pf_call_kernels.hpp b/ploidyfrost_amd/csrc/pf_call_kernels.hpp
--- a/ploidyfrost_amd/csrc/pf_call_kernels.hpp
+++ b/ploidyfrost_amd/csrc/pf_call_kernels.hpp
@@ -128,7 +128,7 @@
         hipEvent_t read_ev[2] = {nullptr, nullptr};
     } lane[PF_CALL_LANES];
     struct AlignWork {
-        DevBuf counters, btask, bpath, ptext, queues, blist, slist, plist, plist2, klist, klist_b, stack_scr, pair_scr, pair_scr2, has, scan_tmp, scan_tmp2, paths_scr, sites_scr;
+        DevBuf counters, btask, bpath, ptext, queues, blist, slist, plist, plist2, klist, klist_b, stack_scr, stack_scr_b, pair_scr, pair_scr2, has, scan_tmp, scan_tmp2, paths_scr, sites_scr;
         DevBuf mlist, paths_big_scr;
         uint32_t mlist_cap = 0;
         DevBuf walk_off, walk_pool;
@@ -136,7 +136,7 @@
         hipStream_t stream = nullptr;
         bool own_stream = false;
         hipStream_t side_stream = nullptr;
-        hipEvent_t ev_prep = nullptr, ev_paths = nullptr;
+        hipEvent_t ev_prep = nullptr, ev_paths = nullptr, ev_snp = nullptr;
     } work[PF_CALL_LANES];
     struct TextWork {
         DevBuf sizes, offs, totals, tcounters, tscan;
@@ -195,7 +195,7 @@
             for (hipEvent_t &e : o.read_ev) if (e) { (void)hipEventDestroy(e); e = nullptr; }
         }
         for (AlignWork &w : work) {
-            for (DevBuf *b : {&w.counters, &w.btask, &w.bpath, &w.ptext, &w.queues, &w.blist, &w.slist, &w.plist, &w.plist2, &w.klist, &w.klist_b, &w.stack_scr,
+            for (DevBuf *b : {&w.counters, &w.btask, &w.bpath, &w.ptext, &w.queues, &w.blist, &w.slist, &w.plist, &w.plist2, &w.klist, &w.klist_b, &w.stack_scr, &w.stack_scr_b,
                               &w.pair_scr, &w.pair_scr2, &w.has, &w.scan_tmp, &w.scan_tmp2, &w.paths_scr, &w.sites_scr, &w.mlist, &w.paths_big_scr, &w.walk_off, &w.walk_pool})
                 b->release();
             if (w.own_stream && w.stream) (void)hipStreamDestroy(w.stream);
@@ -203,6 +203,7 @@
             if (w.side_stream) { (void)hipStreamDestroy(w.side_stream); w.side_stream = nullptr; }
             if (w.ev_prep) { (void)hipEventDestroy(w.ev_prep); w.ev_prep = nullptr; }
             if (w.ev_paths) { (void)hipEventDestroy(w.ev_paths); w.ev_paths = nullptr; }
+            if (w.ev_snp) { (void)hipEventDestroy(w.ev_snp); w.ev_snp = nullptr; }
         }
         for (DevBuf &b : out) b.release();
         for (DevBuf &b : outp) b.release();
diff --git a/ploidyfrost_amd/csrc/pf_ctx.hpp b/ploidyfrost_amd/csrc/pf_ctx.hpp
--- a/ploidyfrost_amd/csrc/pf_ctx.hpp
+++ b/ploidyfrost_amd/csrc/pf_ctx.hpp
@@ -98,6 +98,7 @@
     pf::CallState *call = nullptr;
     hipStream_t bub_streams[PF_CALL_LANES][12] = {};
     hipEvent_t bub_events[PF_CALL_LANES][13] = {};
+    unsigned int *bub_h_retry[PF_CALL_LANES] = {};
 
     void *cc = nullptr;
     void *gfa = nullptr;
@@ -191,9 +192,12 @@
     WS_DENSITY,
     WS_MASK_TEXT, WS_MASK_OUT, WS_MASK_BITS, WS_MASK_TABLE, WS_MASK_INDEX,
     WS_BUB_LANES,
-    WS_COUNT_ = WS_BUB_LANES + 5 * (PF_CALL_LANES - 1)
-};
-inline int bub_ws(int slot, int lane) {
+    WS_BUB_SECOND = WS_BUB_LANES + 5 * (PF_CALL_LANES - 1),
+    WS_COUNT_ = WS_BUB_SECOND + 3 * PF_CALL_LANES
+};
+inline int bub_ws(int slot, int lane, int call = 0) {
+    if (call != 0 && (slot == WS_BUB_RETRY || slot == WS_BUB_WORK || slot == WS_BUB_IDX2))
+        return WS_BUB_SECOND + 3 * lane + (slot == WS_BUB_RETRY ? 0 : slot == WS_BUB_WORK ? 1 : 2);
     if (lane == 0) return slot;
     const int j = slot == WS_BUB_SMALL ? 0 : slot == WS_BUB_RETRY ? 1 : slot == WS_BUB_SCRATCH ? 2 : slot == WS_BUB_WORK ? 3 : 4;
     return WS_BUB_LANES + 5 * (lane - 1) + j;
diff --git a/ploidyfrost_amd/csrc/pf_device.hip b/ploidyfrost_amd/csrc/pf_device.hip
--- a/ploidyfrost_amd/csrc/pf_device.hip
+++ b/ploidyfrost_amd/csrc/pf_device.hip
@@ -746,6 +746,7 @@
     if (ctx->copy_stream) { hipStreamSynchronize(ctx->copy_stream); hipStreamDestroy(ctx->copy_stream); }
     for (auto &lane : ctx->bub_streams) for (auto &s : lane) if (s) hipStreamDestroy(s);
     for (auto &lane : ctx->bub_events) for (auto &e : lane) if (e) hipEventDestroy(e);
+    for (auto &h : ctx->bub_h_retry) if (h) { (void)hipHostFree(h); h = nullptr; }
     hipStreamDestroy(ctx->own_stream);
     delete ctx;
 }
```
